# ShuhangGu/DASR

Measured on AMD Instinct MI355X. Metric: SR train images/sec (4x, 128->512), higher is better.
Workload: dtype bf16 MFMA operands, fp32 accumulate / fp32 residual stream

## Files before the change

dasr_amd/_lib.py:

```python
import ctypes as C
import os
import struct

HERE = os.path.dirname(os.path.abspath(__file__))
LIB_PATH = os.path.join(HERE, 'libdasr_hip.so')

c_i32, c_i64, c_f32, c_vp = C.c_int32, C.c_int64, C.c_float, C.c_void_p


class Tensor(C.Structure):
    _fields_ = [('p', c_vp), ('n_stride', c_i64), ('cb_stride', c_i64)]


class ConvParams(C.Structure):
    _fields_ = [('inp', Tensor), ('in_f32', c_i32), ('Hin', c_i32), ('Win', c_i32), ('ups', c_i32), ('cin', c_i32),
                ('w', c_vp), ('w_lo_off', c_i64), ('bias', c_vp),
                ('cout', c_i32), ('Hout', c_i32), ('Wout', c_i32), ('N', c_i32),
                ('kh', c_i32), ('stride', c_i32), ('pad', c_i32), ('prec', c_i32), ('mt', c_i32),
                ('act', c_i32), ('slope', c_f32),
                ('mask', Tensor), ('mask_f32', c_i32),
                ('alpha', c_f32), ('res1', Tensor), ('beta1', c_f32), ('res2', Tensor), ('beta2', c_f32),
                ('out_f32', Tensor), ('out_bf16', Tensor), ('gamma', c_f32), ('xcd_remap', c_i32),
                ('pad_x', c_i32), ('out_stride', c_i32), ('out_oy', c_i32), ('out_ox', c_i32), ('out_W', c_i32), ('slope_ptr', c_vp),
                ('in_stride', c_i32), ('in_oy', c_i32), ('in_ox', c_i32), ('in_W', c_i32), ('in_scale', c_f32), ('out16_f16', c_i32), ('in_wrap', c_i32), ('out16_lo', c_i32), ('res1_lo', c_i32), ('prelu_part', c_vp)]


class WgradPart(C.Structure):
    _fields_ = [('g', Tensor), ('g_f32', c_i32), ('inp', Tensor), ('in_f32', c_i32), ('ups', c_i32), ('n_ctiles', c_i32),
                ('g_planes', c_i32), ('in_planes', c_i32),
                ('Hin', c_i32), ('Win', c_i32), ('Hout', c_i32), ('Wout', c_i32), ('N', c_i32),
                ('kh', c_i32), ('stride', c_i32), ('pad', c_i32), ('want_bias', c_i32),
                ('ws_off', c_i64), ('ws_bias_off', c_i64), ('tap0', c_i32), ('g_scale', c_f32)]


class WgradReducePart(C.Structure):
    _fields_ = [('ws_off', c_i64), ('ws_bias_off', c_i64), ('nsplit', c_i32), ('ntaps', c_i32), ('oc0', c_i32), ('c0', c_i32),
                ('cout', c_i32), ('cin', c_i32), ('n_ctiles', c_i32), ('dst_w_off', c_i64), ('dst_b_off', c_i64),
                ('flip_io', c_i32), ('split_stride', c_i64), ('tap_stride', c_i64), ('bias_stride', c_i64),
                ('tap0', c_i32), ('ntaps_total', c_i32), ('bias_nsplit', c_i32), ('reserved_', c_i32)]


class ResblockParams(C.Structure):
    _fields_ = [('x16', Tensor), ('x32', Tensor), ('w0', c_vp), ('b0', c_vp), ('w1', c_vp), ('b1', c_vp),
                ('y32', Tensor), ('y16', Tensor), ('h', Tensor), ('N', c_i32), ('H', c_i32), ('W', c_i32), ('res_scale', c_f32), ('slope', c_f32)]


class PackSeg(C.Structure):
    _fields_ = [('src_off', c_i64), ('src_cout', c_i32), ('src_cin', c_i32), ('cin_start', c_i32), ('cin_len', c_i32),
                ('src_c0', c_i32), ('transpose', c_i32)]


class PackDesc(C.Structure):
    _fields_ = [('dst_off', c_i64), ('lo_off', c_i64), ('cout', c_i32), ('cin_pad', c_i32), ('ntaps', c_i32), ('mt', c_i32),
                ('nseg', c_i32), ('src_ntaps', c_i32), ('fmt', c_i32), ('tapmap', C.c_int8 * 32), ('tapmask', C.c_uint16 * 16), ('seg', PackSeg * 5)]


class CropDesc(C.Structure):
    _fields_ = [('src', c_vp), ('C', c_i32), ('H', c_i32), ('W', c_i32), ('vH', c_i32), ('vW', c_i32), ('y0', c_i32), ('x0', c_i32), ('flags', c_i32)]


class CropU8Desc(C.Structure):
    _fields_ = [('src', c_vp), ('H', c_i32), ('W', c_i32), ('y0', c_i32), ('x0', c_i32), ('crop', c_i32), ('flags', c_i32), ('sub_y', c_i32), ('sub_x', c_i32)]


class SrnU8Desc(C.Structure):
    _fields_ = [('src', c_vp), ('H', c_i32), ('W', c_i32), ('y0', c_i32), ('x0', c_i32), ('size', c_i32), ('flags', c_i32), ('dst', c_vp)]


class WindowDesc(C.Structure):
    _fields_ = [('y0', c_i32), ('x0', c_i32)]


class Op(C.Structure):
    _fields_ = [('op', c_i32), ('i', c_i32 * 8), ('f', c_f32 * 4), ('l', c_i64 * 4), ('p', c_vp * 4), ('t', Tensor * 5),
                ('conv', ConvParams), ('flops', C.c_double), ('bytes', C.c_double)]

    def get(self, name):
        arr, k, enc = _slot(self.op, name)
        a = getattr(self, arr)
        if enc == '*':
            return list(a) if arr == 'f' else list((c_f32 * 4).from_buffer(a))
        if enc == 'f':
            return struct.unpack('<f', struct.pack('<I', a[k] & 0xffffffff))[0]
        return a[k]

    def set(self, name, value):
        arr, k, enc = _slot(self.op, name)
        a = getattr(self, arr)
        if enc == '*':
            if arr == 'f':
                a[:] = [float(v) for v in value]
            else:
                (c_f32 * 4).from_buffer(a)[:] = [float(v) for v in value]
        elif enc == 'f':
            a[k] = struct.unpack('<I', struct.pack('<f', value))[0]
        elif value is None:
            a[k] = Tensor(None, 0, 0) if arr == 't' else 0
        else:
            a[k] = value


OP_CONV, OP_WGRAD, OP_WGRAD_REDUCE, OP_PACK, OP_DOWNSUM, OP_AXPBY, OP_FILL, OP_L1LOSS, OP_NCHW2B, OP_B2NCHW = range(1, 11)
(OP_INORM_FWD, OP_INORM_BWD, OP_BCE, OP_DWT_FWD, OP_DWT_BWD, OP_LOWPASS, OP_MAXPOOL, OP_MAXPOOL_BWD, OP_L1DIFF, OP_AFFINE4,
 OP_BILINEAR, OP_LOGLOSS, OP_SIGMOID_BWD, OP_PRELU_GRAD, OP_LOWPASS_VALID, OP_ADD_FLAT, OP_SIGMOID_FWD, OP_EVENT_RECORD, OP_STREAM_WAIT,
 OP_SET_STREAM) = range(11, 31)
OP_CVT_F16, OP_DOWNSUM_F16, OP_PIXSHUF, OP_PIXUNSHUF = 31, 32, 33, 34
OP_LPIPS_S2D, OP_MAXPOOL3, OP_MAXPOOL3_BWD, OP_LPIPS_HEAD, OP_RAGAN = 35, 36, 37, 38, 39
OP_BNORM_FWD, OP_BNORM_BWD, OP_BNORM_RUNNING = 40, 41, 42
OP_DDM_SPREAD = 43
OP_INORM_JVP, OP_INORM_SECOND, OP_GRAD_PENALTY, OP_FILL_SCALED = 44, 45, 46, 47
OP_CONV_CHAIN = 48
OP_RDB_CHAIN = 49
OP_BNORM_JVP, OP_BNORM_SECOND = 50, 51
OP_PRELU_FINAL = 52
OP_RESBLOCK = 53
OP_LPIPS_S2D_ANY = 54

OP_ARGS = {
    OP_WGRAD: dict(parts_dev='p0', nparts='i0', nsplit='i1', kh='i2', stride='i3', f32='i4', ws='p1'),
    OP_WGRAD_REDUCE: dict(parts_dev='p0', nparts='i0', ws='p1', grad_flat='p2', scale='f0', inv_prescale='f1', few_splits='i1'),
    OP_PACK: dict(descs_dev='p0', ndesc='i0', total_pieces='l0', piece_prefix_dev='p1', params_flat='p2', packed='p3'),
    OP_DOWNSUM: dict(src='t0', N='i0', C='i1', H='i2', W='i3', mask='t1', mask_f32='i4', slope='f0', dst_f32='t2', dst_bf16='t3'),
    OP_AXPBY: dict(x='t0', a='f0', z='t1', b='f1', N='i0', C='i1', H='i2', W='i3', out_f32='t2', out_bf16='t3', gamma='f2', mask='t4', slope='f3',
                   slope_ptr='p0'),
    OP_FILL: dict(p='p0', n='l0', value='f0'),
    OP_L1LOSS: dict(sr='t0', hr_nchw='p0', weight_map='p1', N='i0', C='i1', H='i2', W='i3', coef='f0', loss_acc='p2', grad='t1', accumulate='i4',
                    grad_scale='f1'),
    OP_NCHW2B: dict(src='p0', N='i0', C='i1', H='i2', W='i3', dst_f32='t0', dst_bf16='t1'),
    OP_B2NCHW: dict(src='t0', N='i0', C='i1', H='i2', W='i3', dst='p0'),
    OP_INORM_FWD: dict(x='t0', N='i0', C='i1', H='i2', W='i3', eps='f0', slope='f1', y='t1', stats='p0'),
    OP_INORM_BWD: dict(a='t0', ga='t1', N='i0', C='i1', H='i2', W='i3', slope='f0', stats='p0', gx='t2'),
    OP_BCE: dict(x='t0', N='i0', C='i1', H='i2', W='i3', gan_type='i4', target='f0', coef='f1', gcoef='f2', loss_acc='p0', score_acc='p1',
                 score_coef='f3', grad='t1'),
    OP_DWT_FWD: dict(x='t0', N='i0', C='i1', H2='i2', W2='i3', norm='i4', ll='t1', hc='t2'),
    OP_DWT_BWD: dict(gll='t0', ghc='t1', N='i0', C='i1', H2='i2', W2='i3', norm='i4', gx='t2', accumulate='i5'),
    OP_LOWPASS: dict(x='t0', x2='t1', w='p0', k='i4', N='i0', C='i1', H='i2', W='i3', mode='i5', a_h='f0', b_h='f1', out_low='t2', out_high='t3',
                     accumulate='i6'),
    OP_MAXPOOL: dict(x='t0', is_f32='i4', N='i0', C='i1', Ho='i2', Wo='i3', y='t1', Win='i6'),
    OP_MAXPOOL_BWD: dict(x='t0', gy='t1', is_f32='i4', N='i0', C='i1', Ho='i2', Wo='i3', gx='t2', relu_mask='i5', Win='i6'),
    OP_L1DIFF: dict(a='t0', b='t1', is_f32='i4', N='i0', C='i1', H='i2', W='i3', coef='f0', gcoef='f1', loss_acc='p0', ga='t2'),
    OP_AFFINE4: dict(x='t0', N='i0', C='i1', H='i2', W='i3', scale4='f*', shift4='l*', y='t1', y_f32='i4', accumulate='i5'),
    OP_BILINEAR: dict(src='p0', N='i0', h='i1', w='i2', factor='i3', dst='p1'),
    OP_LOGLOSS: dict(x='t0', N='i0', H='i1', W='i2', mode='i3', eps='f0', coef='f1', gcoef='f2', loss_acc='p0', score_acc='p1', score_coef='f3',
                     grad='t1', accumulate='i4'),
    OP_SIGMOID_BWD: dict(y='t0', g='t1', N='i0', C='i1', H='i2', W='i3', gz='t2'),
    OP_PRELU_GRAD: dict(y='t0', gx='t1', N='i0', C='i1', H='i2', W='i3', slope='p0', scratch256='p1', dst='p2', scale='f0', f16='i4', inv_prescale='f1'),
    OP_LOWPASS_VALID: dict(x='t0', w='p0', k='i4', N='i0', C='i1', H='i2', W='i3', mode='i5', out='t1', accumulate='i6'),
    OP_ADD_FLAT: dict(y='p0', x='p1', n='l0'),
    OP_SIGMOID_FWD: dict(x='t0', N='i0', C='i1', H='i2', W='i3', y='t1'),
    OP_EVENT_RECORD: dict(event='p0'),
    OP_STREAM_WAIT: dict(event='p0'),
    OP_SET_STREAM: dict(stream='p0'),
    OP_PIXSHUF: dict(src='t0', N='i0', C4='i1', H='i2', W='i3', dst='t1'),
    OP_PIXUNSHUF: dict(gsrc='t0', mask='t1', slope='f0', N='i0', C4='i1', H='i2', W='i3', gdst='t2'),
    OP_CVT_F16: dict(x='t0', N='i0', C='i1', H='i2', W='i3', scale='f0', y='t1', form='i4'),
    OP_DOWNSUM_F16: dict(src='t0', N='i0', C='i1', H='i2', W='i3', mask='t1', slope='f0', out_scale='f1', dst_f32='t2', dst_f16='t3'),
    OP_BNORM_FWD: dict(x='t0', N='i0', C='i1', H='i2', W='i3', group='i4', eps='f0', slope='f1', gamma='p0', beta='p1', y='t1', stats='p2'),
    OP_BNORM_BWD: dict(x='t0', ga='t1', N='i0', C='i1', H='i2', W='i3', group='i4', slope='f0', gamma='p0', beta='p1', stats='p2', gx='t2', dgamma='p3',
                       dbeta='l0', pscale='f1'),
    OP_BNORM_RUNNING: dict(stats='p0', g='i0', C='i1', count='i2', momentum='f0', running_mean='p1', running_var='p2', num_batches_tracked='p3'),
    OP_INORM_JVP: dict(a='t0', t='t1', N='i0', C='i1', H='i2', W='i3', slope='f0', stats='p0', out='t2'),
    OP_INORM_SECOND: dict(a='t0', t='t1', ga='t2', N='i0', C='i1', H='i2', W='i3', slope='f0', stats='p0', out='t3', accumulate='i4'),
    OP_RESBLOCK: dict(p='p0'),
    OP_PRELU_FINAL: dict(partial='p0', nblocks='i0', stride='l0', count='i1', slopes='p1', dsts='p2', scale='f0'),
    OP_BNORM_JVP: dict(x='t0', t='t1', N='i0', C='i1', H='i2', W='i3', group='i4', slope='f0', gamma='p0', beta='p1', stats='p2', out='t2'),
    OP_BNORM_SECOND: dict(x='t0', t='t1', ga='t2', N='i0', C='i1', H='i2', W='i3', group='i4', slope='f0', gamma='p0', beta='p1', stats='p2', out='t3',
                          accumulate='i5', dgamma='p3', pscale='f1'),
    OP_GRAD_PENALTY: dict(g='t0', N='i0', C='i1', H='i2', W='i3', weight='f0', part256='p0', out3='p1', loss_acc='p2', stage='i4',
                          world='i5'),
    OP_FILL_SCALED: dict(x='t0', N='i0', C='i1', H='i2', W='i3', scalar='p0', factor='f0'),
    OP_CONV_CHAIN: dict(dev_layers='p0', host_layers='p1', dev_dep_chunk='p2', nlayers='i0', dev_flags='p3', dev_err='l0'),
    OP_RDB_CHAIN: dict(dev_layers='p0', host_layers='p1', nlayers='i0', dev_flags='p3', dev_err='l0'),
    OP_DDM_SPREAD: dict(d='t0', N='i0', n_h='i1', n_w='i2', H='i3', W='i4', jump='i5', rf='i6', start='f0', out='t1'),
    OP_RAGAN: dict(a='t0', b='t1', N='i0', H='i1', W='i2', stage='i3', n_glob='i4', form='i5', ta='f0', tb='f1', coef='f2', gcoef='f3', eps='l2f',
                   sums='p0', part='p1', loss_acc='p2', score_a='p3', score_b='l0', score_coef='l1f', ga='t2', gb='t3'),
    OP_LPIPS_S2D: dict(x='t0', N='i0', H='i1', W='i2', scale4='f*', shift4='l*', y='t1', mode='i3'),
    OP_MAXPOOL3: dict(x='t0', N='i0', C='i1', H='i2', W='i3', y='t1'),
# ... 184 lines not shown
```

dasr_amd/csrc/conv.hip:

```cpp
#include "common.h"

namespace {

template <int PREC, bool IN_F32, int MT, int KH, int STRIDE, int NT_, int KS = 1>
struct Cfg {
    static constexpr int NT = NT_;
    static constexpr int RPT = STRIDE == 1 ? 1 : 2;
    static constexpr int CPT = STRIDE == 1 ? 32 : 16;
    static constexpr int TH = 4 * NT * RPT;
    static constexpr int TW = CPT;
    static constexpr int IH = (TH - 1) * STRIDE + KH;
    static constexpr int IW = (TW - 1) * STRIDE + KH;
    static constexpr int NTAPS = KH * KH;
    static constexpr int PIXB = KS == 1 ? 48 : 80;
    static constexpr int ACT_BYTES = IH * IW * PIXB;
    static constexpr int W_BYTES = KS * NTAPS * MT * 1024;
    static constexpr int NARR = PREC >= 3 ? 2 : 1;
    static constexpr int LDS_BYTES = NARR * (ACT_BYTES + W_BYTES);
    static constexpr int PPP16 = IN_F32 ? 4 : 2;
    static constexpr int PPP = PPP16 * KS;
    static constexpr int NPIECE = IH * IW * PPP;
    static constexpr int AR = (NPIECE + 255) / 256;
    static constexpr int WPIECE = KS * NTAPS * MT * 64;
    static constexpr int WR = (WPIECE + 255) / 256;
};

constexpr unsigned OOB = 0x80000000u;
constexpr int RSRC_FLAGS = 0x00020000;
constexpr int RSRC_RANGE = 0x7fffffff;

#ifdef DASR_TRACE
__device__ unsigned long long* g_trace = nullptr;
#define TRACE_STAMP(k)                                                                         \
    do {                                                                                       \
        if (g_trace && threadIdx.x == 0) g_trace[(size_t)blockIdx.x * 16 + (k)] = __builtin_readcyclecounter(); \
    } while (0)
#else
#define TRACE_STAMP(k) do {} while (0)
#endif

__device__ __forceinline__ __amdgpu_buffer_rsrc_t make_rsrc(const void* p) {
    return __builtin_amdgcn_make_buffer_rsrc((void*)p, 0, RSRC_RANGE, RSRC_FLAGS);
}

template <int NG>
struct MaskPre {
    u32x4 v[NG][2];
};

template <int MT, int NT>
__device__ __forceinline__ void mask_prefetch(const dasr_conv_params& p, MaskPre<NT * MT>& m, int tid, int mg, int n, int oy0, int ox0) {
    const int lane = tid & 63, wave = tid >> 6, nn = lane & 31, kh2 = lane >> 5;
    const int ostr = p.out_stride > 1 ? p.out_stride : 1, owid = p.out_W > 0 ? p.out_W : p.Wout;
    const __amdgpu_buffer_rsrc_t rmask = make_rsrc((const char*)p.mask.p + (size_t)n * p.mask.n_stride * 2);
    const unsigned mask_cb = (unsigned)p.mask.cb_stride;
#pragma unroll
    for (int gi = 0; gi < NT * MT; ++gi) {
        const int nt = gi / MT, mi = gi - nt * MT;
        const int oy = oy0 + wave * NT + nt, ox = ox0 + nn;
        const unsigned oob = ((oy < p.Hout) & (ox < p.Wout)) ? 0u : OOB;
        const unsigned pixel = (unsigned)((oy * ostr + p.out_oy) * owid + ox * ostr + p.out_ox) * 16u;
#pragma unroll
        for (int pr = 0; pr < 2; ++pr) {
            const int oc = (mg * MT + mi) * 32 + 16 * pr;
            const unsigned mo = (((unsigned)(oc >> 4) * mask_cb + pixel + 8u * kh2) * 2u) | oob;
            m.v[gi][pr] = __builtin_amdgcn_raw_buffer_load_b128(rmask, mo, 0, 0);
        }
    }
}

template <bool SC1>
__device__ __forceinline__ void st128(u32x4 v, __amdgpu_buffer_rsrc_t r, unsigned off) {
    if constexpr (SC1) __builtin_amdgcn_raw_buffer_store_b128(v, r, off, 0, 16);
    else __builtin_amdgcn_raw_buffer_store_b128(v, r, off, 0, 0);
}

template <bool IN_F32, int MT, int NT, int STRIDE, int EPI, int F16OUT = -1, bool PRE = false, bool FSC1 = false, bool BIAS_STAGED = false, bool CONST_SLOPE = false,
          bool PACC = false>
__device__ __forceinline__ void conv_epilogue(const dasr_conv_params& p, f32x16 (&acc)[MT][NT], char* smem, float bias_reg, int tid, int mg, int n,
                                              int oy0, int ox0, const MaskPre<NT * MT>* pre = nullptr) {
    const int lane = tid & 63, wave = tid >> 6, nn = lane & 31, kh2 = lane >> 5;
    (void)lane;
    constexpr bool G = EPI == 0;
    const bool has_bias = G ? p.bias != nullptr : bool(EPI & 1);
    const bool act_lrelu = G ? p.act == 1 : bool(EPI & 2);
    const bool act_sigmoid = G ? p.act == 2 : false;
    const bool has_mask = G ? p.mask.p != nullptr : bool(EPI & 4);
    const bool has_r1 = G ? p.res1.p != nullptr : bool(EPI & 8);
    const bool has_r2 = G ? p.res2.p != nullptr : bool(EPI & 16);
    const bool has_f32 = G ? p.out_f32.p != nullptr : bool(EPI & 32);
    const bool has_bf16 = G ? p.out_bf16.p != nullptr : bool(EPI & 64);
    const bool scaled = G ? true : bool(EPI & 128);
    const bool f16out = F16OUT < 0 ? p.out16_f16 != 0 : F16OUT != 0;
    const bool chan_tail = G ? true : false;
    const int ostr = p.out_stride > 1 ? p.out_stride : 1, owid = p.out_W > 0 ? p.out_W : p.Wout;
    constexpr int MSZ = IN_F32 ? 4 : 2;
    const float slope = (!CONST_SLOPE && p.slope_ptr) ? *p.slope_ptr : p.slope;
    constexpr bool PACC_OK = PACC && EPI == 68 && MT == 2 && !IN_F32 && !FSC1 && !PRE;
    static_assert(!PACC || PACC_OK, "the slope-gradient partials exist for the 64-channel mask-only epilogue of the LDS-DMA kernel");
    constexpr bool pacc_on = PACC_OK;
    float pacc = 0.f;
    const __amdgpu_buffer_rsrc_t rmask = make_rsrc((const char*)p.mask.p + (size_t)n * p.mask.n_stride * MSZ);
    const __amdgpu_buffer_rsrc_t rr1 = make_rsrc((const char*)p.res1.p + (size_t)n * p.res1.n_stride * ((G && p.res1_lo) ? 2 : 4));
    const __amdgpu_buffer_rsrc_t rr2 = make_rsrc((const float*)p.res2.p + (size_t)n * p.res2.n_stride);
    const __amdgpu_buffer_rsrc_t rof = make_rsrc((float*)p.out_f32.p + (size_t)n * p.out_f32.n_stride);
    const __amdgpu_buffer_rsrc_t rob = make_rsrc((bf16_t*)p.out_bf16.p + (size_t)n * p.out_bf16.n_stride);
    const unsigned mask_cb = (unsigned)p.mask.cb_stride, r1_cb = (unsigned)p.res1.cb_stride, r2_cb = (unsigned)p.res2.cb_stride;
    const unsigned of_cb = (unsigned)p.out_f32.cb_stride, ob_cb = (unsigned)p.out_bf16.cb_stride;
    constexpr bool SC1 = FSC1 || (MT == 1 && !IN_F32 && F16OUT == 0);
    const unsigned lo_pl = (G || F16OUT != 0) ? (unsigned)p.out16_lo : 0u;
    f32x4 bia[MT][4];
    if (has_bias) {
        float* bl = (float*)smem;
        if constexpr (!BIAS_STAGED) {
            if (tid < 32 * MT) bl[tid] = bias_reg;
            __syncthreads();
        }
#pragma unroll
        for (int mi = 0; mi < MT; ++mi)
#pragma unroll
            for (int g = 0; g < 4; ++g) bia[mi][g] = *(const f32x4*)(bl + mi * 32 + 8 * g + 4 * kh2);
    }
    TRACE_STAMP(5);
    constexpr int NG = NT * MT;
    constexpr bool WIDE16 = !G && !IN_F32;
    constexpr bool WIDE32 = !G && STRIDE == 1;
    constexpr bool PIPE_EPI = !G && !(MT == 2 && (EPI & 16) && (EPI & 8)) && (EPI & (4 | 8 | 16));
    u32x4 mk[2][4], r1v[2][4], r2v[2][4];
    auto group_addr = [&](int gi, unsigned (&eo)[4], unsigned (&cbv)[4]) {
        const int nt = gi / MT, mi = gi - nt * MT;
        int r, c;
        if constexpr (STRIDE == 1) {
            r = wave * NT + nt;
            c = nn;
        } else {
            r = (wave * NT + nt) * 2 + (nn >> 4);
            c = nn & 15;
        }
        const int oy = oy0 + r, ox = ox0 + c;
        const bool pv = (oy < p.Hout) & (ox < p.Wout);
        const unsigned pixel = (unsigned)((oy * ostr + p.out_oy) * owid + ox * ostr + p.out_ox) * 16u;
#pragma unroll
        for (int g = 0; g < 4; ++g) {
            const int oc = (mg * MT + mi) * 32 + 8 * g + 4 * kh2;
            const bool cv = chan_tail ? (pv & (oc < ((p.cout + 15) & ~15))) : pv;
            cbv[g] = (unsigned)(oc >> 4);
            eo[g] = cv ? pixel + (unsigned)(oc & 15) : OOB;
        }
    };
    auto group_addr32 = [&](int gi, unsigned (&e32)[2]) {
        const int nt = gi / MT;
        const int oy = oy0 + wave * NT + nt;
        const unsigned q4 = 4u * (2u * (unsigned)(nn >> 4) + (unsigned)kh2);
#pragma unroll
        for (int st = 0; st < 2; ++st) {
            const int ox = ox0 + (nn & 15) + 16 * st;
            const bool pv = (oy < p.Hout) & (ox < p.Wout);
            e32[st] = pv ? (unsigned)((oy * ostr + p.out_oy) * owid + ox * ostr + p.out_ox) * 16u + q4 : OOB;
        }
    };
    auto issue_loads = [&](int gi, int slot) {
        unsigned eo[4], cbv[4];
        group_addr(gi, eo, cbv);
        unsigned e32[2];
        if constexpr (WIDE32) group_addr32(gi, e32);
        if (has_mask && !PRE) {
            if constexpr (WIDE16) {
#pragma unroll
                for (int pr = 0; pr < 2; ++pr) {
                    const unsigned mo = eo[2 * pr] != OOB ? (cbv[2 * pr] * mask_cb + eo[2 * pr] + 4u * kh2) * 2u : OOB;
                    mk[slot][2 * pr] = __builtin_amdgcn_raw_buffer_load_b128(rmask, mo, 0, 0);
                }
            } else {
#pragma unroll
                for (int g = 0; g < 4; ++g) {
                    const unsigned mo = eo[g] != OOB ? (cbv[g] * mask_cb + eo[g]) * MSZ : OOB;
                    if constexpr (IN_F32) {
                        mk[slot][g] = __builtin_amdgcn_raw_buffer_load_b128(rmask, mo, 0, 0);
                    } else {
                        const u32x2 t2 = __builtin_amdgcn_raw_buffer_load_b64(rmask, mo, 0, 0);
                        mk[slot][g] = u32x4{t2[0], t2[1], 0u, 0u};
                    }
                }
            }
        }
        if (G && has_r1 && p.res1_lo) {
#pragma unroll
            for (int g = 0; g < 4; ++g) {
                const u32x2 hi = __builtin_amdgcn_raw_buffer_load_b64(rr1, eo[g] != OOB ? (cbv[g] * r1_cb + eo[g]) * 2u : OOB, 0, 0);
                const u32x2 lo = __builtin_amdgcn_raw_buffer_load_b64(rr1, eo[g] != OOB ? ((cbv[g] + (unsigned)p.res1_lo) * r1_cb + eo[g]) * 2u : OOB, 0, 0);
                r1v[slot][g] = u32x4{hi[0], hi[1], lo[0], lo[1]};
            }
        } else if (has_r1) {
#pragma unroll
            for (int g = 0; g < 4; ++g) {
                if constexpr (WIDE32) r1v[slot][g] = __builtin_amdgcn_raw_buffer_load_b128(rr1, e32[g & 1] != OOB ? (cbv[g] * r1_cb + e32[g & 1]) * 4u : OOB, 0, 0);
                else r1v[slot][g] = __builtin_amdgcn_raw_buffer_load_b128(rr1, eo[g] != OOB ? (cbv[g] * r1_cb + eo[g]) * 4u : OOB, 0, 0);
            }
        }
        if (has_r2) {
#pragma unroll
            for (int g = 0; g < 4; ++g) {
                if constexpr (WIDE32) r2v[slot][g] = __builtin_amdgcn_raw_buffer_load_b128(rr2, e32[g & 1] != OOB ? (cbv[g] * r2_cb + e32[g & 1]) * 4u : OOB, 0, 0);
                else r2v[slot][g] = __builtin_amdgcn_raw_buffer_load_b128(rr2, eo[g] != OOB ? (cbv[g] * r2_cb + eo[g]) * 4u : OOB, 0, 0);
            }
        }
    };
    auto rows_swap = [&](u32x4& a, u32x4& b) {
#pragma unroll
        for (int j = 0; j < 4; ++j) {
            const auto r = __builtin_amdgcn_permlane16_swap(a[j], b[j], false, false);
            a[j] = r[0];
            b[j] = r[1];
        }
    };
    if constexpr (PIPE_EPI) issue_loads(0, 0);
#pragma unroll
    for (int gi = 0; gi < NG; ++gi) {
        const int nt = gi / MT, mi = gi - nt * MT;
        const int slot = PIPE_EPI ? (gi & 1) : 0;
        if constexpr (PIPE_EPI) {
            if (gi + 1 < NG) issue_loads(gi + 1, (gi + 1) & 1);
        } else {
            issue_loads(gi, 0);
        }
        {
            unsigned eo[4], cbv[4];
            group_addr(gi, eo, cbv);
            float v[4][4];
#pragma unroll
            for (int g = 0; g < 4; ++g)
#pragma unroll
                for (int j = 0; j < 4; ++j) v[g][j] = acc[mi][nt][4 * g + j];
            if (has_bias) {
#pragma unroll
                for (int g = 0; g < 4; ++g)
#pragma unroll
                    for (int j = 0; j < 4; ++j) v[g][j] += bia[mi][g][j];
            }
            if (act_lrelu && !G && !CONST_SLOPE && p.slope_ptr) {
#pragma unroll
                for (int g = 0; g < 4; ++g)
#pragma unroll
                    for (int j = 0; j < 4; ++j) v[g][j] = v[g][j] > 0.f ? v[g][j] : slope * v[g][j];
            } else if (act_lrelu && !G) {
#pragma unroll
                for (int g = 0; g < 4; ++g)
#pragma unroll
                    for (int j = 0; j < 4; ++j) v[g][j] = fmaxf(v[g][j], slope * v[g][j]);
            } else if (act_lrelu) {
#pragma unroll
                for (int g = 0; g < 4; ++g)
#pragma unroll
                    for (int j = 0; j < 4; ++j) v[g][j] = fmaxf(v[g][j], 0.f) + slope * fminf(v[g][j], 0.f);
            } else if (act_sigmoid) {
#pragma unroll
                for (int g = 0; g < 4; ++g)
#pragma unroll
                    for (int j = 0; j < 4; ++j) v[g][j] = __frcp_rn(1.f + __expf(-v[g][j]));
            }
            if (has_mask) {
                if constexpr (WIDE16) {
#pragma unroll
                    for (int pr = 0; pr < 2; ++pr) {
                        u32x4 w = mk[slot][2 * pr];
                        if constexpr (PRE) w = pre->v[gi][pr];
                        const auto r0 = __builtin_amdgcn_permlane32_swap(w[0], w[2], false, false);
                        const auto r1 = __builtin_amdgcn_permlane32_swap(w[1], w[3], false, false);
                        mk[slot][2 * pr] = u32x4{r0[0], r1[0], 0u, 0u};
                        mk[slot][2 * pr + 1] = u32x4{r0[1], r1[1], 0u, 0u};
                    }
                }
#pragma unroll
                for (int g = 0; g < 4; ++g)
#pragma unroll
                    for (int j = 0; j < 4; ++j) {
                        if constexpr (IN_F32) {
                            v[g][j] *= __uint_as_float(mk[slot][g][j]) > 0.f ? 1.f : slope;
                        } else {
                            const unsigned wd = mk[slot][g][j >> 1];
                            const short hbits = (j & 1) ? (short)(wd >> 16) : (short)(wd & 0xffffu);
                            if constexpr (PACC_OK) {
                                if (pacc_on) {
                                    const unsigned short hb = (unsigned short)hbits;
                                    const float hv = f16out ? (float)__builtin_bit_cast(f16_t, hb) : (float)__builtin_bit_cast(bf16_t, hb);
                                    pacc += hbits > 0 ? 0.f : v[g][j] * hv;
                                }
                            }
                            v[g][j] = hbits > 0 ? v[g][j] : slope * v[g][j];
                        }
                    }
            }
            if (scaled && p.alpha != 1.f) {
#pragma unroll
                for (int g = 0; g < 4; ++g)
#pragma unroll
                    for (int j = 0; j < 4; ++j) v[g][j] *= p.alpha;
            }
            if (G && has_r1 && p.res1_lo) {
#pragma unroll
                for (int g = 0; g < 4; ++g) {
                    const u32x4 w = r1v[slot][g];
#pragma unroll
                    for (int j = 0; j < 4; ++j) {
                        const unsigned short hb = (unsigned short)((j & 1) ? (w[j >> 1] >> 16) : (w[j >> 1] & 0xffffu));
                        const unsigned short lb = (unsigned short)((j & 1) ? (w[2 + (j >> 1)] >> 16) : (w[2 + (j >> 1)] & 0xffffu));
                        const float r = f16out ? (float)__builtin_bit_cast(f16_t, hb) + (float)__builtin_bit_cast(f16_t, lb)
                                               : (float)__builtin_bit_cast(bf16_t, hb) + (float)__builtin_bit_cast(bf16_t, lb);
                        v[g][j] += p.beta1 * r;
                    }
                }
            } else if (has_r1) {
                if constexpr (WIDE32) {
                    rows_swap(r1v[slot][0], r1v[slot][1]);
                    rows_swap(r1v[slot][2], r1v[slot][3]);
                }
#pragma unroll
                for (int g = 0; g < 4; ++g)
#pragma unroll
                    for (int j = 0; j < 4; ++j) v[g][j] += p.beta1 * __uint_as_float(r1v[slot][g][j]);
            }
            if (has_r2) {
                if constexpr (WIDE32) {
                    rows_swap(r2v[slot][0], r2v[slot][1]);
                    rows_swap(r2v[slot][2], r2v[slot][3]);
                }
#pragma unroll
                for (int g = 0; g < 4; ++g)
#pragma unroll
                    for (int j = 0; j < 4; ++j) v[g][j] += p.beta2 * __uint_as_float(r2v[slot][g][j]);
            }
            if (chan_tail && (mg * MT + mi) * 32 + 32 > p.cout) {
#pragma unroll
                for (int g = 0; g < 4; ++g)
#pragma unroll
                    for (int j = 0; j < 4; ++j)
                        if ((mg * MT + mi) * 32 + 8 * g + 4 * kh2 + j >= p.cout) v[g][j] = 0.f;
            }
            if (has_f32 && WIDE32) {
                unsigned e32[2];
                group_addr32(gi, e32);
#pragma unroll
                for (int pr = 0; pr < 2; ++pr) {
                    u32x4 oa = {__float_as_uint(v[2 * pr][0]), __float_as_uint(v[2 * pr][1]), __float_as_uint(v[2 * pr][2]), __float_as_uint(v[2 * pr][3])};
                    u32x4 ob = {__float_as_uint(v[2 * pr + 1][0]), __float_as_uint(v[2 * pr + 1][1]), __float_as_uint(v[2 * pr + 1][2]), __float_as_uint(v[2 * pr + 1][3])};
                    rows_swap(oa, ob);
                    st128<SC1>(oa, rof, e32[0] != OOB ? (cbv[2 * pr] * of_cb + e32[0]) * 4u : OOB);
                    st128<SC1>(ob, rof, e32[1] != OOB ? (cbv[2 * pr] * of_cb + e32[1]) * 4u : OOB);
                }
            } else if (has_f32) {
#pragma unroll
                for (int g = 0; g < 4; ++g) {
                    const u32x4 o = {__float_as_uint(v[g][0]), __float_as_uint(v[g][1]), __float_as_uint(v[g][2]), __float_as_uint(v[g][3])};
                    st128<SC1>(o, rof, eo[g] != OOB ? (cbv[g] * of_cb + eo[g]) * 4u : OOB);
                }
            }
            if (has_bf16 && WIDE16) {
                const bool gm = scaled && p.gamma != 1.f;
#pragma unroll
                for (int pr = 0; pr < 2; ++pr) {
                    bf16x4 oa, ob;
#pragma unroll
                    for (int j = 0; j < 4; ++j) {
                        const float va = gm ? v[2 * pr][j] * p.gamma : v[2 * pr][j], vb = gm ? v[2 * pr + 1][j] * p.gamma : v[2 * pr + 1][j];
                        oa[j] = f16out ? __builtin_bit_cast(bf16_t, (f16_t)va) : (bf16_t)va;
                        ob[j] = f16out ? __builtin_bit_cast(bf16_t, (f16_t)vb) : (bf16_t)vb;
                    }
                    const u32x2 a = __builtin_bit_cast(u32x2, oa), b = __builtin_bit_cast(u32x2, ob);
                    const auto r0 = __builtin_amdgcn_permlane32_swap(a[0], b[0], false, false);
                    const auto r1 = __builtin_amdgcn_permlane32_swap(a[1], b[1], false, false);
                    const u32x4 o = {r0[0], r1[0], r0[1], r1[1]};
                    st128<SC1>(o, rob, eo[2 * pr] != OOB ? (cbv[2 * pr] * ob_cb + eo[2 * pr] + 4u * kh2) * 2u : OOB);
                    if (lo_pl) {
                        bf16x4 la, lb;
#pragma unroll
                        for (int j = 0; j < 4; ++j) {
                            const float va = gm ? v[2 * pr][j] * p.gamma : v[2 * pr][j], vb = gm ? v[2 * pr + 1][j] * p.gamma : v[2 * pr + 1][j];
                            const float ha = f16out ? (float)(f16_t)va : (float)(bf16_t)va, hb = f16out ? (float)(f16_t)vb : (float)(bf16_t)vb;
                            la[j] = f16out ? __builtin_bit_cast(bf16_t, (f16_t)(va - ha)) : (bf16_t)(va - ha);
                            lb[j] = f16out ? __builtin_bit_cast(bf16_t, (f16_t)(vb - hb)) : (bf16_t)(vb - hb);
                        }
                        const u32x2 a2 = __builtin_bit_cast(u32x2, la), b2 = __builtin_bit_cast(u32x2, lb);
                        const auto q0 = __builtin_amdgcn_permlane32_swap(a2[0], b2[0], false, false);
                        const auto q1 = __builtin_amdgcn_permlane32_swap(a2[1], b2[1], false, false);
                        const u32x4 o2 = {q0[0], q1[0], q0[1], q1[1]};
                        st128<SC1>(o2, rob, eo[2 * pr] != OOB ? ((cbv[2 * pr] + lo_pl) * ob_cb + eo[2 * pr] + 4u * kh2) * 2u : OOB);
                    }
                }
            } else if (has_bf16) {
                const bool gm = scaled && p.gamma != 1.f;
#pragma unroll
                for (int g = 0; g < 4; ++g) {
                    bf16x4 ob;
#pragma unroll
                    for (int j = 0; j < 4; ++j) {
                        const float vv = gm ? v[g][j] * p.gamma : v[g][j];
                        ob[j] = f16out ? __builtin_bit_cast(bf16_t, (f16_t)vv) : (bf16_t)vv;
                    }
#ifdef DASR_TRACE
                    if (p.xcd_remap & 2) {
                        const unsigned lin = ((((unsigned)blockIdx.x * 4 + wave) * NT + nt) * 4 + g) * 512u + (unsigned)lane * 8u;
                        __builtin_amdgcn_raw_buffer_store_b64(__builtin_bit_cast(u32x2, ob), make_rsrc(p.out_bf16.p), lin, 0, 0);
                        continue;
                    }
#endif
                    __builtin_amdgcn_raw_buffer_store_b64(__builtin_bit_cast(u32x2, ob), rob, eo[g] != OOB ? (cbv[g] * ob_cb + eo[g]) * 2u : OOB, 0, 0);
                    if (lo_pl) {
                        bf16x4 lb;
#pragma unroll
                        for (int j = 0; j < 4; ++j) {
                            const float vv = gm ? v[g][j] * p.gamma : v[g][j];
                            const float hh = f16out ? (float)(f16_t)vv : (float)(bf16_t)vv;
                            lb[j] = f16out ? __builtin_bit_cast(bf16_t, (f16_t)(vv - hh)) : (bf16_t)(vv - hh);
                        }
                        __builtin_amdgcn_raw_buffer_store_b64(__builtin_bit_cast(u32x2, lb), rob, eo[g] != OOB ? ((cbv[g] + lo_pl) * ob_cb + eo[g]) * 2u : OOB, 0, 0);
                    }
                }
            }
        }
    }
    if constexpr (PACC_OK) {
        if (pacc_on) {
            const float t = wave_sum(pacc);
            __syncthreads();
            if (lane == 0) ((float*)smem)[wave] = t;
            __syncthreads();
            if (tid == 0) {
                float tot = 0.f;
                for (int w = 0; w < (int)(blockDim.x >> 6); ++w) tot += ((const float*)smem)[w];
                p.prelu_part[blockIdx.x] = tot * slope;
            }
        }
    }
}

template <int PREC, bool IN_F32, int MT, int KH, int STRIDE, int NT, int KS, bool DBUF, int MODE, int EPI>
__global__ __launch_bounds__(256, 2) void conv_kernel(const dasr_conv_params p) {
    using C = Cfg<PREC, IN_F32, MT, KH, STRIDE, NT, KS>;
    extern __shared__ __attribute__((aligned(16))) char smem[];
    constexpr int ACT_LO = C::ACT_BYTES, W_HI = C::NARR * C::ACT_BYTES, W_LO = W_HI + C::W_BYTES;
    constexpr int DUMMY = C::LDS_BYTES;

    const int tid = threadIdx.x, lane = tid & 63, wave = tid >> 6;
#ifdef DASR_TRACE
    if (g_trace && threadIdx.x == 0) g_trace[(size_t)blockIdx.x * 16 + 15] = __builtin_amdgcn_s_memrealtime();
#endif
    TRACE_STAMP(0);
    const int cout_tiles = (p.cout + 31) >> 5;
    const int MG = (cout_tiles + MT - 1) / MT;
    const int tiles_x = (p.Wout + C::TW - 1) / C::TW, tiles_y = (p.Hout + C::TH - 1) / C::TH;
    int bid = blockIdx.x;
    {
        const int total = gridDim.x;
        if ((p.xcd_remap & 1) && (total & 7) == 0) bid = (bid & 7) * (total >> 3) + (bid >> 3);
    }
    const int mg = bid % MG;
    bid /= MG;
    const int tx = bid % tiles_x;
    bid /= tiles_x;
    const int ty = bid % tiles_y;
    const int n = bid / tiles_y;
    const int oy0 = ty * C::TH, ox0 = tx * C::TW;
    const int iy0 = oy0 * STRIDE - p.pad, ix0 = ox0 * STRIDE - (p.pad_x >= 0 ? p.pad_x : p.pad);
    const int HL = p.ups ? 2 * p.Hin : p.Hin, WL = p.ups ? 2 * p.Win : p.Win;
    const int nchunks = p.cin / (16 * KS);
    constexpr int ESZ = IN_F32 ? 4 : 2;
    static_assert(PREC != 2 || IN_F32, "prec 2 (f16 operands) converts an f32 input while staging");
    const float in_sc = ((PREC == 2 || PREC == 4) && p.in_scale != 0.f) ? p.in_scale : 1.f;
    float bias_reg = 0.f;
    {
        const int oc = mg * MT * 32 + tid;
        const unsigned bo = ((p.bias != nullptr) & (tid < 32 * MT) & (oc < p.cout)) ? (unsigned)oc * 4u : OOB;
        bias_reg = __uint_as_float(__builtin_amdgcn_raw_buffer_load_b32(make_rsrc(p.bias), bo, 0, 0));
    }

    unsigned goff[C::AR];
    int loff[C::AR];
#pragma unroll
    for (int r = 0; r < C::AR; ++r) {
        const int q = tid + r * 256;
        const int pix = q / C::PPP, piece = q - pix * C::PPP;
        const int iy = pix / C::IW, ix = pix - iy * C::IW;
        const int gy = iy0 + iy, gx = ix0 + ix;
        const bool ok = (q < C::NPIECE) & (gy >= 0) & (gy < HL) & (gx >= 0) & (gx < WL);
        const int sy = p.ups ? (gy >> 1) : gy, sx = p.ups ? (gx >> 1) : gx;
        const int pl = piece / C::PPP16, pp = piece - pl * C::PPP16;
        const int spix = p.in_stride > 1 ? (sy * p.in_stride + p.in_oy) * p.in_W + sx * p.in_stride + p.in_ox : sy * p.Win + sx;
        goff[r] = ok ? (unsigned)((pl * (int)p.in.cb_stride + spix * 16 + pp * (IN_F32 ? 4 : 8)) * ESZ) : OOB;
        loff[r] = q < C::NPIECE ? pix * C::PIXB + piece * (IN_F32 ? 8 : 16) : DUMMY;
    }
    const __amdgpu_buffer_rsrc_t rin = make_rsrc((const char*)p.in.p + (size_t)n * p.in.n_stride * ESZ);
    const unsigned in_chunk_bytes = (unsigned)(p.in.cb_stride * KS * ESZ);
    const __amdgpu_buffer_rsrc_t rw = make_rsrc((const bf16_t*)p.w + (size_t)mg * nchunks * KS * C::NTAPS * MT * 512);
    const unsigned w_chunk_bytes = KS * C::NTAPS * MT * 1024;
    const unsigned w_lo_bytes = (unsigned)(p.w_lo_off * 2);
    unsigned woff[C::WR];
    int wloff[C::WR];
#pragma unroll
    for (int r = 0; r < C::WR; ++r) {
        const int q = tid + r * 256;
        woff[r] = q < C::WPIECE ? (unsigned)q * 16u : OOB;
        wloff[r] = q < C::WPIECE ? q * 16 : DUMMY - W_HI;
    }

    u32x4 areg[C::AR];
    u32x4 wreg[C::WR * C::NARR];
    auto load_chunk = [&](int ck) {
        const unsigned so = (unsigned)ck * in_chunk_bytes;
#pragma unroll
        for (int r = 0; r < C::AR; ++r) areg[r] = __builtin_amdgcn_raw_buffer_load_b128(rin, goff[r], so, 0);
        const unsigned wo = (unsigned)ck * w_chunk_bytes;
#pragma unroll
        for (int r = 0; r < C::WR; ++r) {
            wreg[r] = __builtin_amdgcn_raw_buffer_load_b128(rw, woff[r], wo, 0);
            if constexpr (PREC >= 3) wreg[C::WR + r] = __builtin_amdgcn_raw_buffer_load_b128(rw, woff[r], wo + w_lo_bytes, 0);
        }
    };
    auto store_chunk = [&](char* buf) {
#pragma unroll
        for (int r = 0; r < C::AR; ++r) {
            if constexpr (!IN_F32) {
                *(u32x4*)(buf + loff[r]) = areg[r];
            } else {
                bf16x4 hi, lo;
#pragma unroll
                for (int j = 0; j < 4; ++j) {
                    bf16_t h, l;
                    if constexpr (PREC == 2) {
                        h = __builtin_bit_cast(bf16_t, (f16_t)(__uint_as_float(areg[r][j]) * in_sc));
                        l = h;
                    } else if constexpr (PREC == 4) {
                        split_f16(__uint_as_float(areg[r][j]) * in_sc, h, l);
                    } else {
                        split_bf16(__uint_as_float(areg[r][j]), h, l);
                    }
                    hi[j] = h;
                    lo[j] = l;
                }
                *(bf16x4*)(buf + loff[r]) = hi;
// ... 169 lines not shown

template <int MT, int NW = 4>
struct GCfg {
    static constexpr int NT = 4, NTH = NW * 64, TH = 4 * NW, TW = 32, IH = TH + 2, IW = 34, NPIX = IH * IW;
    static constexpr int AR = (NPIX * 2 + NTH - 1) / NTH;
    static constexpr int ACT_BYTES = AR * NTH * 16;
    static constexpr int WPIECE = 9 * MT * 64;
    static constexpr int WR = (WPIECE + NTH - 1) / NTH;
    static constexpr int W_BYTES = WPIECE * 16;
    static constexpr int BUF_BYTES = ACT_BYTES + W_BYTES;
    static constexpr int LDS_BYTES = 2 * BUF_BYTES;
};

template <int MT, int NW>
__device__ __forceinline__ void glds_dma_piece(int i, int ck, char* buf, __amdgpu_buffer_rsrc_t rin, __amdgpu_buffer_rsrc_t rw, const unsigned* goff,
                                               unsigned in_chunk_bytes, int wave, int tid, int ckp) {
    using C = GCfg<MT, NW>;
    typedef __attribute__((address_space(3))) void* lds_ptr;
    if (i < C::AR) {
        __builtin_amdgcn_raw_ptr_buffer_load_lds(rin, (lds_ptr)(buf + (i * C::NTH + wave * 64) * 16), 16, goff[i], (unsigned)ckp * in_chunk_bytes, 0, 0);
    } else {
        const int r = i - C::AR;
        if (r * C::NTH + wave * 64 < C::WPIECE)
            __builtin_amdgcn_raw_ptr_buffer_load_lds(rw, (lds_ptr)(buf + C::ACT_BYTES + (r * C::NTH + wave * 64) * 16), 16, (unsigned)(tid + r * C::NTH) * 16u,
                                                     (unsigned)ck * (9u * MT * 1024u), 0, 0);
    }
}

template <int MT, int EPI, int NW, int ABL = 0, bool F16 = false, int RING = 0>
__global__ __launch_bounds__(NW * 64, NW == 4 ? 2 : 1) void conv_glds_kernel(const dasr_conv_params p) {
    using C = GCfg<MT, NW>;
    constexpr int NT = C::NT;
    extern __shared__ __attribute__((aligned(16))) char smem[];
    const int tid = threadIdx.x, lane = tid & 63, wave = __builtin_amdgcn_readfirstlane(tid >> 6);
#ifdef DASR_TRACE
    if (g_trace && threadIdx.x == 0) g_trace[(size_t)blockIdx.x * 16 + 15] = __builtin_amdgcn_s_memrealtime();
#endif
    TRACE_STAMP(0);
    int a_cout = p.cout, a_Wout = p.Wout, a_Hout = p.Hout, a_remap = p.xcd_remap, a_ups = p.ups, a_cin = p.cin, a_Hin = p.Hin, a_Win = p.Win;
    const void* a_bias = p.bias;
    const void* a_in = p.in.p;
    const void* a_w = p.w;
    long long a_nstr = p.in.n_stride, a_cbstr = p.in.cb_stride;
    int a_wrap = p.in_wrap;
    asm volatile("" : "+s"(a_cout), "+s"(a_Wout), "+s"(a_Hout), "+s"(a_remap), "+s"(a_cin), "+s"(a_Hin), "+s"(a_Win), "+s"(a_bias), "+s"(a_in), "+s"(a_w),
                 "+s"(a_nstr), "+s"(a_cbstr), "+s"(a_wrap), "+s"(a_ups)
                 : "s"(p.slope), "s"(p.out_stride), "s"(p.out_oy), "s"(p.out_ox), "s"(p.out_W), "s"(p.alpha), "s"(p.gamma), "s"(p.out16_lo), "s"(p.N));
    a_remap |= a_ups << 8;
    const int cout_tiles = (a_cout + 31) >> 5;
    const int MG = (cout_tiles + MT - 1) / MT;
    const int tiles_x = (a_Wout + C::TW - 1) / C::TW, tiles_y = (a_Hout + C::TH - 1) / C::TH;
    int bid = blockIdx.x;
    {
        const int total = (int)((unsigned)a_remap >> 12);
        const int remapped = (bid & 7) * (total >> 3) + (bid >> 3);
        bid = ((a_remap & 1) && (total & 7) == 0) ? remapped : bid;
    }
    const int mg = bid % MG;
    bid /= MG;
    const int tx = bid % tiles_x;
    bid /= tiles_x;
    const int ty = bid % tiles_y;
    const int n = bid / tiles_y;
    const int oy0 = ty * C::TH, ox0 = tx * C::TW;
    const int iy0 = oy0 - 1, ix0 = ox0 - 1;
    const int nchunks = a_cin >> 4;
    const int in_wrap = a_wrap > 0 ? a_wrap : 0x7fffffff;
    constexpr int rot = 0;
    float bias_reg = 0.f;
    {
        const int oc = mg * MT * 32 + tid;
        const unsigned bo = ((a_bias != nullptr) & (tid < 32 * MT) & (oc < a_cout)) ? (unsigned)oc * 4u : OOB;
        bias_reg = __uint_as_float(__builtin_amdgcn_raw_buffer_load_b32(make_rsrc(a_bias), bo, 0, 0));
    }
    unsigned goff[C::AR];
#pragma unroll
    for (int r = 0; r < C::AR; ++r) {
        const int q = tid + r * C::NTH;
        const int pp = q >> 1, h = (q & 1) ^ ((pp >> 3) & 1);
        const int iy = pp / C::IW, ix = pp - iy * C::IW;
        const int gy = iy0 + iy, gx = ix0 + ix;
        const int us = (a_remap >> 8) & 1;
        const bool ok = (pp < C::NPIX) & (gy >= 0) & (gy < (a_Hin << us)) & (gx >= 0) & (gx < (a_Win << us));
        goff[r] = ok ? (unsigned)((((gy >> us) * a_Win + (gx >> us)) * 16 + 8 * h) * 2) : OOB;
    }
    const __amdgpu_buffer_rsrc_t rin = make_rsrc((const bf16_t*)a_in + (size_t)n * a_nstr);
    const unsigned in_chunk_bytes = (unsigned)(a_cbstr * 2);
    const __amdgpu_buffer_rsrc_t rw = make_rsrc((const bf16_t*)a_w + (size_t)mg * nchunks * 9 * MT * 512);
    constexpr int NP = C::AR + C::WR;
#pragma unroll
    for (int i = 0; i < NP; ++i) glds_dma_piece<MT, NW>(i, rot, smem, rin, rw, goff, in_chunk_bytes, wave, tid, rot);
    TRACE_STAMP(1);
    const int nn = lane & 31, kh2 = lane >> 5;
    int baddr[6][3];
#pragma unroll
    for (int rr = 0; rr < 6; ++rr)
#pragma unroll
        for (int kx = 0; kx < 3; ++kx) {
            const int pp = (wave * NT + rr) * C::IW + nn + kx;
            baddr[rr][kx] = ((pp << 1) + (kh2 ^ ((pp >> 3) & 1))) << 4;
        }
    const int aoff = lane * 16;

    f32x16 acc[MT][NT];
    constexpr bool R1_PRE = MT == 2 && EPI != 0 && (EPI & 8);
    if constexpr (R1_PRE) {
        const __amdgpu_buffer_rsrc_t rr1 = make_rsrc((const float*)p.res1.p + (size_t)n * p.res1.n_stride);
        const unsigned r1_cb = (unsigned)p.res1.cb_stride;
        const int nn_ = lane & 31, kh_ = lane >> 5;
#pragma unroll
        for (int nt = 0; nt < NT; ++nt) {
            const int oy = oy0 + wave * NT + nt, ox = ox0 + nn_;
            const bool pv = (oy < a_Hout) & (ox < a_Wout);
            const unsigned pixel = (unsigned)((oy + p.out_oy) * (p.out_W > 0 ? p.out_W : a_Wout) + ox + p.out_ox) * 16u;
#pragma unroll
            for (int mi = 0; mi < MT; ++mi)
#pragma unroll
                for (int g = 0; g < 4; ++g) {
                    const int oc = (mg * MT + mi) * 32 + 8 * g + 4 * kh_;
                    const u32x4 t = __builtin_amdgcn_raw_buffer_load_b128(rr1, pv ? ((unsigned)(oc >> 4) * r1_cb + pixel + (unsigned)(oc & 15)) * 4u : OOB, 0, 0);
#pragma unroll
                    for (int j = 0; j < 4; ++j) acc[mi][nt][4 * g + j] = __uint_as_float(t[j]);
                }
        }
    } else {
#pragma unroll
        for (int mi = 0; mi < MT; ++mi)
#pragma unroll
            for (int nt = 0; nt < NT; ++nt)
#pragma unroll
                for (int j = 0; j < 16; ++j) acc[mi][nt][j] = 0.f;
    }

    __builtin_amdgcn_s_waitcnt(0x0F70);
    __syncthreads();
    if constexpr (R1_PRE) {
        const float c1 = p.beta1 / p.alpha;
#pragma unroll
        for (int mi = 0; mi < MT; ++mi)
#pragma unroll
            for (int nt = 0; nt < NT; ++nt) acc[mi][nt] *= c1;
    }
    TRACE_STAMP(2);

    constexpr bool PRE = EPI == 68 && MT == 1;
    MaskPre<NT * MT> mpre;
    bf16x8 fb[2][6], fa[2][MT];
    for (int ck = 0; ck < nchunks; ++ck) {
        const char* buf = smem + (ck & 1) * C::BUF_BYTES;
        const char* wbuf = buf + C::ACT_BYTES;
        char* nbuf = smem + ((ck + 1) & 1) * C::BUF_BYTES;
        const bool more = ck + 1 < nchunks;
        if constexpr (PRE) {
            if (!more) mask_prefetch<MT, NT>(p, mpre, tid, mg, n, oy0, ox0);
        }
        const int ckn = ck + 1 + rot < nchunks ? ck + 1 + rot : ck + 1 + rot - nchunks;
        const int ckp = ckn >= in_wrap ? ckn - in_wrap : ckn;
        if (ck == 2) TRACE_STAMP(8);
#pragma unroll
        for (int rr = 0; rr < 6; ++rr) fb[0][rr] = *(const bf16x8*)(buf + baddr[rr][0]);
#pragma unroll
        for (int mi = 0; mi < MT; ++mi) fa[0][mi] = *(const bf16x8*)(wbuf + aoff + (0 * MT + mi) * 1024);
#pragma unroll
        for (int s = 0; s < 9; ++s) {
            const int kx = s / 3, ky = s - kx * 3;
            if (s + 1 < 9) {
                const int kx1 = (s + 1) / 3, ky1 = (s + 1) - kx1 * 3;
#pragma unroll
                for (int mi = 0; mi < MT; ++mi) fa[(s + 1) & 1][mi] = *(const bf16x8*)(wbuf + aoff + ((ky1 * 3 + kx1) * MT + mi) * 1024);
                if (ky == 1 && kx < 2) {
#pragma unroll
                    for (int rr = 0; rr < 6; ++rr) fb[(kx + 1) & 1][rr] = *(const bf16x8*)(buf + baddr[rr][kx + 1]);
                }
            }
            if (more && s < 4) {
#pragma unroll
                for (int i = s * NP / 4; i < (s + 1) * NP / 4; ++i) glds_dma_piece<MT, NW>(i, ckn, nbuf, rin, rw, goff, in_chunk_bytes, wave, tid, ckp);
            }
            __builtin_amdgcn_sched_barrier(0);
#pragma unroll
            for (int mi = 0; mi < MT; ++mi)
#pragma unroll
                for (int nt = 0; nt < NT; ++nt)
                    acc[mi][nt] = mfma16<F16>(fa[s & 1][mi], fb[kx & 1][nt + ky], acc[mi][nt]);
            __builtin_amdgcn_sched_barrier(0);
        }
        if (ck == 2) TRACE_STAMP(9);
        __builtin_amdgcn_s_waitcnt(0x0F70);
        if (ck == 2) TRACE_STAMP(10);
        __syncthreads();
        if (ck == 2) TRACE_STAMP(11);
    }
    TRACE_STAMP(4);
    if constexpr (EPI == 68 && MT == 2 && !PRE) {
        if (p.prelu_part) conv_epilogue<false, MT, NT, 1, EPI, F16 ? 1 : 0, false, false, false, false, true>(p, acc, smem, bias_reg, tid, mg, n, oy0, ox0, &mpre);
        else conv_epilogue<false, MT, NT, 1, EPI, F16 ? 1 : 0, PRE>(p, acc, smem, bias_reg, tid, mg, n, oy0, ox0, &mpre);
    } else {
        conv_epilogue<false, MT, NT, 1, R1_PRE ? (EPI & ~8) : EPI, F16 ? 1 : 0, PRE>(p, acc, smem, bias_reg, tid, mg, n, oy0, ox0, &mpre);
    }
    TRACE_STAMP(6);
#ifdef DASR_TRACE
    __builtin_amdgcn_s_waitcnt(0);
#endif
    TRACE_STAMP(7);
#ifdef DASR_TRACE
    if (g_trace && threadIdx.x == 0) g_trace[(size_t)blockIdx.x * 16 + 14] = __builtin_amdgcn_s_memrealtime();
#endif
}

#ifdef DASR_TRACE
#define CH_T() (g_trace && threadIdx.x == 0 ? (unsigned long long)__builtin_readcyclecounter() : 0ull)
#define CH_ACC(type, phase, val)                                                                           \
    do {                                                                                                   \
        if (g_trace && threadIdx.x == 0) g_trace[(size_t)(1 << 20) + (size_t)blockIdx.x * 64 + (type) * 8 + (phase)] += (val); \
    } while (0)
#else
#define CH_T() 0ull
#define CH_ACC(type, phase, val) do {} while (0)
#endif

#ifdef DASR_TRACE
#define CH_WHERE(ticket, xcc)                                                                  \
    do {                                                                                       \
        if (g_trace && threadIdx.x == 0) {                                                     \
            unsigned hw;                                                                       \
            asm volatile("s_getreg_b32 %0, hwreg(HW_REG_HW_ID)" : "=s"(hw));                   \
            g_trace[(size_t)(1 << 20) + (size_t)blockIdx.x * 64 + 56] = hw;                    \
            g_trace[(size_t)(1 << 20) + (size_t)blockIdx.x * 64 + 57] = (unsigned)(ticket);    \
            g_trace[(size_t)(1 << 20) + (size_t)blockIdx.x * 64 + 58] = (unsigned)(xcc);       \
        }                                                                                      \
    } while (0)
#else
#define CH_WHERE(ticket, xcc) do {} while (0)
#endif

struct ChainSync {
    __amdgpu_buffer_rsrc_t rflags;
    int* err;
    unsigned f0;
    int base, ty, tx, tiles_y, tiles_x;

    __device__ __forceinline__ void wait(int layer, int tid) const {
        if (layer > 0) {
            if (tid < 9 && tid != 4) {
                const int y = ty + tid / 3 - 1, x = tx + tid % 3 - 1;
                if ((y >= 0) & (y < tiles_y) & (x >= 0) & (x < tiles_x)) {
                    const unsigned off = (unsigned)(base + y * tiles_x + x) * 4u, target = f0 + (unsigned)layer;
                    int spins = 0;
                    while ((int)(__builtin_amdgcn_raw_buffer_load_b32(rflags, off, 0, 17) - target) < 0) {
                        __builtin_amdgcn_s_sleep(2);
                        ++spins;
                        if (spins > (1 << 21) || ((spins & 1023) == 0 && __builtin_amdgcn_raw_buffer_load_b32(make_rsrc(err), 0, 0, 17) != 0)) {
                            atomicOr(err, 2);
                            break;
                        }
                    }
                }
            }
            __syncthreads();
        }
    }
    __device__ __forceinline__ void publish(int layer, int tid) const {
        __builtin_amdgcn_s_waitcnt(0x0F70);
        __syncthreads();
        if (tid == 0) __builtin_amdgcn_raw_buffer_store_b32(f0 + (unsigned)layer + 1u, rflags, (unsigned)(base + ty * tiles_x + tx) * 4u, 0, 16);
    }
};

template <int MT, int EPI, bool F16>
__device__ __forceinline__ void chain_layer(const dasr_conv_params& p, char* smem, const int tid, const int n, const int oy0, const int ox0,
                                            const unsigned (&goff)[GCfg<1, 4>::AR], const int dep_chunk, const ChainSync& cs, const int layer) {
    using C = GCfg<MT, 4>;
    constexpr int NT = C::NT, NW = 4;
    static_assert(GCfg<1, 4>::AR == GCfg<2, 4>::AR, "the activation pieces do not depend on MT");
    const int lane = tid & 63, wave = __builtin_amdgcn_readfirstlane(tid >> 6);
    const int nchunks = p.cin >> 4;
    const int ttype = MT == 2 ? 2 : (dep_chunk <= 1 ? 0 : 1);
    (void)ttype;
    const unsigned long long t_a = CH_T();
    float bias_reg;
    {
        const unsigned bo = ((p.bias != nullptr) & (tid < 32 * MT)) ? (unsigned)tid * 4u : OOB;
        bias_reg = __uint_as_float(__builtin_amdgcn_raw_buffer_load_b32(make_rsrc(p.bias), bo, 0, 0));
    }
    const __amdgpu_buffer_rsrc_t rin = make_rsrc((const bf16_t*)p.in.p + (size_t)n * p.in.n_stride);
    const unsigned in_chunk_bytes = (unsigned)(p.in.cb_stride * 2);
    const __amdgpu_buffer_rsrc_t rw = make_rsrc(p.w);
    constexpr int NP = C::AR + C::WR;
    if (dep_chunk <= 0) cs.wait(layer, tid);
#pragma unroll
    for (int i = 0; i < NP; ++i) glds_dma_piece<MT, NW>(i, 0, smem, rin, rw, goff, in_chunk_bytes, wave, tid, 0);
    const unsigned long long t_b = CH_T();
    const int nn = lane & 31, kh2 = lane >> 5;
    int baddr[6][3];
#pragma unroll
    for (int rr = 0; rr < 6; ++rr)
#pragma unroll
        for (int kx = 0; kx < 3; ++kx) {
            const int pp = (wave * NT + rr) * C::IW + nn + kx;
            baddr[rr][kx] = ((pp << 1) + (kh2 ^ ((pp >> 3) & 1))) << 4;
        }
    const int aoff = lane * 16;
    f32x16 acc[MT][NT];
    constexpr bool R1_PRE = MT == 2 && (EPI & 8);
    if constexpr (R1_PRE) {
        const __amdgpu_buffer_rsrc_t rr1 = make_rsrc((const float*)p.res1.p + (size_t)n * p.res1.n_stride);
        const unsigned r1_cb = (unsigned)p.res1.cb_stride;
#pragma unroll
        for (int nt = 0; nt < NT; ++nt) {
            const int oy = oy0 + wave * NT + nt, ox = ox0 + nn;
            const bool pv = (oy < p.Hout) & (ox < p.Wout);
            const unsigned pixel = (unsigned)(oy * p.Wout + ox) * 16u;
#pragma unroll
            for (int mi = 0; mi < MT; ++mi)
#pragma unroll
                for (int g = 0; g < 4; ++g) {
                    const int oc = mi * 32 + 8 * g + 4 * kh2;
                    const u32x4 t = __builtin_amdgcn_raw_buffer_load_b128(rr1, pv ? ((unsigned)(oc >> 4) * r1_cb + pixel + (unsigned)(oc & 15)) * 4u : OOB, 0, 0);
#pragma unroll
                    for (int j = 0; j < 4; ++j) acc[mi][nt][4 * g + j] = __uint_as_float(t[j]);
                }
        }
    } else {
#pragma unroll
        for (int mi = 0; mi < MT; ++mi)
#pragma unroll
            for (int nt = 0; nt < NT; ++nt)
#pragma unroll
                for (int j = 0; j < 16; ++j) acc[mi][nt][j] = 0.f;
    }
    __builtin_amdgcn_s_waitcnt(0x0F70);
    __syncthreads();
    if constexpr (R1_PRE) {
        const float c1 = p.beta1 / p.alpha;
#pragma unroll
        for (int mi = 0; mi < MT; ++mi)
#pragma unroll
            for (int nt = 0; nt < NT; ++nt) acc[mi][nt] *= c1;
    }
    constexpr bool PRE = EPI == 68 && MT == 1;
    MaskPre<NT * MT> mpre;
    bf16x8 fb[2][6];
    const unsigned long long t_c = CH_T();
    unsigned long long t_poll = 0;
    (void)t_poll;
    for (int ck = 0; ck < nchunks; ++ck) {
        const char* buf = smem + (ck & 1) * C::BUF_BYTES;
        const char* wbuf = buf + C::ACT_BYTES;
        char* nbuf = smem + ((ck + 1) & 1) * C::BUF_BYTES;
        const bool more = ck + 1 < nchunks;
        if (ck + 1 == dep_chunk) {
            const unsigned long long t0 = CH_T();
            cs.wait(layer, tid);
            t_poll += CH_T() - t0;
        }
        if constexpr (PRE) {
            if (!more) mask_prefetch<MT, NT>(p, mpre, tid, 0, n, oy0, ox0);
        }
        bf16x8 fa[3][MT];
#pragma unroll
        for (int rr = 0; rr < 6; ++rr) fb[0][rr] = *(const bf16x8*)(buf + baddr[rr][0]);
#pragma unroll
        for (int mi = 0; mi < MT; ++mi) fa[0][mi] = *(const bf16x8*)(wbuf + aoff + (0 * MT + mi) * 1024);
#pragma unroll
        for (int s = 0; s < 9; ++s) {
            const int kx = s / 3, ky = s - kx * 3;
            if (s + 1 < 9) {
                const int kx1 = (s + 1) / 3, ky1 = (s + 1) - kx1 * 3;
#pragma unroll
                for (int mi = 0; mi < MT; ++mi) fa[(s + 1) & 1][mi] = *(const bf16x8*)(wbuf + aoff + ((ky1 * 3 + kx1) * MT + mi) * 1024);
                if (ky == 1 && kx < 2) {
#pragma unroll
                    for (int rr = 0; rr < 6; ++rr) fb[(kx + 1) & 1][rr] = *(const bf16x8*)(buf + baddr[rr][kx + 1]);
                }
            }
            if (more && s < 4) {
#pragma unroll
                for (int i = s * NP / 4; i < (s + 1) * NP / 4; ++i) glds_dma_piece<MT, NW>(i, ck + 1, nbuf, rin, rw, goff, in_chunk_bytes, wave, tid, ck + 1);
            }
            __builtin_amdgcn_sched_barrier(0);
#pragma unroll
            for (int mi = 0; mi < MT; ++mi)
#pragma unroll
                for (int nt = 0; nt < NT; ++nt) acc[mi][nt] = mfma16<F16>(fa[s & 1][mi], fb[kx & 1][nt + ky], acc[mi][nt]);
            __builtin_amdgcn_sched_barrier(0);
        }
        __builtin_amdgcn_s_waitcnt(0x0F70);
        __syncthreads();
    }
    const unsigned long long t_d = CH_T();
    conv_epilogue<false, MT, NT, 1, R1_PRE ? (EPI & ~8) : EPI, F16 ? 1 : 0, PRE, true>(p, acc, smem, bias_reg, tid, 0, n, oy0, ox0, &mpre);
    const unsigned long long t_e = CH_T();
    cs.publish(layer, tid);
    const unsigned long long t_f = CH_T();
    CH_ACC(ttype, 0, t_b - t_a);
    CH_ACC(ttype, 1, t_c - t_b);
    CH_ACC(ttype, 2, t_d - t_c);
    CH_ACC(ttype, 3, t_poll);
    CH_ACC(ttype, 4, t_e - t_d);
    CH_ACC(ttype, 5, t_f - t_e);
    CH_ACC(ttype, 6, 1ull);
    CH_ACC(ttype, 7, (unsigned long long)nchunks);
    (void)t_a; (void)t_b; (void)t_c; (void)t_d; (void)t_e; (void)t_f;
}

template <bool F16, bool BWD>
__global__ __launch_bounds__(256, 2) void conv_chain_kernel(const dasr_conv_params* __restrict__ layers, const int* __restrict__ dep_chunk, int nlayers,
                                                           int tiles_y, int tiles_x, unsigned* flags, unsigned* tickets, int* err) {
    using C = GCfg<1, 4>;
    extern __shared__ __attribute__((aligned(16))) char smem[];
    const int tid = threadIdx.x;
    const int T = tiles_y * tiles_x;
    unsigned xcc;
    asm volatile("s_getreg_b32 %0, hwreg(HW_REG_XCC_ID)" : "=s"(xcc));
    const int xcd = (int)(xcc & 7u);
    const int quota = (int)(gridDim.x >> 3);
    int* tk = (int*)smem;
    if (tid == 0) tk[0] = (int)(atomicAdd(tickets + xcd, 1u) % (unsigned)quota);
    __syncthreads();
    const int j = __builtin_amdgcn_readfirstlane(tk[0]);
    __syncthreads();
    const int img = j / T, tile = j - img * T;
    const int n = xcd + 8 * img;
    const int ty = tile / tiles_x, tx = tile - ty * tiles_x;
    CH_WHERE(j, xcc);
    ChainSync cs;
    cs.rflags = make_rsrc(flags);
    cs.err = err;
    cs.base = n * T;
    cs.ty = ty, cs.tx = tx, cs.tiles_y = tiles_y, cs.tiles_x = tiles_x;
    cs.f0 = __builtin_amdgcn_readfirstlane(__builtin_amdgcn_raw_buffer_load_b32(cs.rflags, (unsigned)(cs.base + tile) * 4u, 0, 17));
    const int oy0 = ty * C::TH, ox0 = tx * C::TW;
    const int iy0 = oy0 - 1, ix0 = ox0 - 1;
    const int Hin = layers[0].Hin, Win = layers[0].Win;
    unsigned goff[C::AR];
#pragma unroll
    for (int r = 0; r < C::AR; ++r) {
        const int q = tid + r * C::NTH;
        const int pp = q >> 1, h = (q & 1) ^ ((pp >> 3) & 1);
        const int iy = pp / C::IW, ix = pp - iy * C::IW;
        const int gy = iy0 + iy, gx = ix0 + ix;
        const bool ok = (pp < C::NPIX) & (gy >= 0) & (gy < Hin) & (gx >= 0) & (gx < Win);
        goff[r] = ok ? (unsigned)(((gy * Win + gx) * 16 + 8 * h) * 2) : OOB;
    }
    for (int L = 0; L < nlayers; ++L) {
        const dasr_conv_params& p = layers[L];
        const int dep = dep_chunk[L];
        if constexpr (BWD) {
            if (p.mt == 1) chain_layer<1, 68, F16>(p, smem, tid, n, oy0, ox0, goff, dep, cs, L);
            else if (p.res2.p != nullptr) chain_layer<2, 248, F16>(p, smem, tid, n, oy0, ox0, goff, dep, cs, L);
            else chain_layer<2, 232, F16>(p, smem, tid, n, oy0, ox0, goff, dep, cs, L);
        } else {
            if (p.mt == 1) chain_layer<1, 67, F16>(p, smem, tid, n, oy0, ox0, goff, dep, cs, L);
            else if (p.res2.p != nullptr) chain_layer<2, 249, F16>(p, smem, tid, n, oy0, ox0, goff, dep, cs, L);
            else chain_layer<2, 233, F16>(p, smem, tid, n, oy0, ox0, goff, dep, cs, L);
        }
    }
}

template <int MT, int EPI = 0, int NW = 4, int ABL = 0, bool F16 = false, int RING = 0>
int launch_glds(const dasr_conv_params& p, hipStream_t s) {
    static_assert(ABL == 0 && RING == 0, "one dense-block conv kernel");
    using C = GCfg<MT, NW>;
    static bool attr_set = false;
    auto kfn = conv_glds_kernel<MT, EPI, NW, ABL, F16, RING>;
    if ((p.cin & 15) || p.kh != 3 || p.stride != 1 || p.pad != 1 || p.in_f32 || p.prec != (F16 ? 2 : 1) || (p.pad_x >= 0 && p.pad_x != 1) || p.in_stride > 1)
        return DASR_EINVAL;
    if (p.out_bf16.p && (p.out16_f16 != 0) != F16) return DASR_EINVAL;
    if (p.prelu_part && !(EPI == 68 && MT == 2)) return DASR_EINVAL;
    if (!attr_set) {
        HIP_TRY(hipFuncSetAttribute((const void*)kfn, hipFuncAttributeMaxDynamicSharedMemorySize, C::LDS_BYTES));
        attr_set = true;
    }
    const int cout_tiles = (p.cout + 31) >> 5;
    const int MG = (cout_tiles + MT - 1) / MT;
    const int tiles_x = (p.Wout + C::TW - 1) / C::TW, tiles_y = (p.Hout + C::TH - 1) / C::TH;
    const long long grid = (long long)MG * tiles_x * tiles_y * p.N;
    if (grid <= 0 || grid >= (1LL << 20)) return DASR_EINVAL;
    dasr_conv_params q = p;
    q.xcd_remap = (p.xcd_remap & 0xfff) | (int)((unsigned)grid << 12);
    DASR_LAUNCH_TAG(__PRETTY_FUNCTION__, kfn, dim3((unsigned)grid), dim3(C::NTH), C::LDS_BYTES, s, q);
    return (int)hipGetLastError();
}

template <int PREC, bool IN_F32, int MT, int KH, int STRIDE, int NT, int KS = 1, bool DBUF = false, int MODE = 0, int EPI = 0>
int launch(const dasr_conv_params& p, hipStream_t s) {
    static_assert(KS == 1 && !DBUF && MODE == 0, "one staging form of the register-staged kernel");
    using C = Cfg<PREC, IN_F32, MT, KH, STRIDE, NT, KS>;
    static bool attr_set = false;
    auto kfn = conv_kernel<PREC, IN_F32, MT, KH, STRIDE, NT, KS, DBUF, MODE, EPI>;
    if (p.cin % (16 * KS)) return DASR_EINVAL;
    if (p.prelu_part) return DASR_EINVAL;
    if (!attr_set) {
        HIP_TRY(hipFuncSetAttribute((const void*)kfn, hipFuncAttributeMaxDynamicSharedMemorySize, C::LDS_BYTES + 16));
        attr_set = true;
    }
    const int cout_tiles = (p.cout + 31) >> 5;
    const int MG = (cout_tiles + MT - 1) / MT;
    const int tiles_x = (p.Wout + C::TW - 1) / C::TW, tiles_y = (p.Hout + C::TH - 1) / C::TH;
    const long long grid = (long long)MG * tiles_x * tiles_y * p.N;
    if (grid <= 0 || grid > 0x7fffffffLL) return DASR_EINVAL;
    DASR_LAUNCH_TAG(__PRETTY_FUNCTION__, kfn, dim3((unsigned)grid), dim3(256), C::LDS_BYTES + 16, s, p);
    return (int)hipGetLastError();
}

__global__ void conv_naive_kernel(const dasr_conv_params p, const float* w) {
    const long long total = (long long)p.N * p.cout * p.Hout * p.Wout;
    const long long i = (long long)blockIdx.x * blockDim.x + threadIdx.x;
    if (i >= total) return;
    const int ox = i % p.Wout;
    long long t = i / p.Wout;
    const int oy = t % p.Hout;
    t /= p.Hout;
    const int oc = t % p.cout;
    const int n = t / p.cout;
    const int HL = p.ups ? 2 * p.Hin : p.Hin, WL = p.ups ? 2 * p.Win : p.Win;
    float acc = 0.f;
    for (int c = 0; c < p.cin; ++c)
        for (int ky = 0; ky < p.kh; ++ky)
            for (int kx = 0; kx < p.kh; ++kx) {
                const int gy = oy * p.stride - p.pad + ky, gx = ox * p.stride - (p.pad_x >= 0 ? p.pad_x : p.pad) + kx;
                if (gy < 0 || gy >= HL || gx < 0 || gx >= WL) continue;
                const int sy = p.ups ? gy >> 1 : gy, sx = p.ups ? gx >> 1 : gx;
                const size_t spix = p.in_stride > 1 ? ((size_t)sy * p.in_stride + p.in_oy) * p.in_W + (size_t)sx * p.in_stride + p.in_ox : (size_t)sy * p.Win + sx;
                const size_t o = (size_t)n * p.in.n_stride + (size_t)(c >> 4) * p.in.cb_stride + spix * 16 + (c & 15);
                const float x = p.in_f32 ? ((const float*)p.in.p)[o] : (float)((const bf16_t*)p.in.p)[o];
                acc += x * w[(((size_t)oc * p.cin + c) * p.kh + ky) * p.kh + kx];
            }
    if (p.bias) acc += p.bias[oc];
    const float nslope = p.slope_ptr ? *p.slope_ptr : p.slope;
    if (p.act == 1) acc = acc > 0.f ? acc : acc * nslope;
    if (p.act == 2) acc = 1.f / (1.f + expf(-acc));
    const size_t po = ((size_t)oy * p.Wout + ox) * 16 + (oc & 15);
    if (p.mask.p) {
        const size_t mo = (size_t)n * p.mask.n_stride + (size_t)(oc >> 4) * p.mask.cb_stride + po;
        const float m = p.mask_f32 ? ((const float*)p.mask.p)[mo] : (float)((const bf16_t*)p.mask.p)[mo];
        acc = m > 0.f ? acc : acc * nslope;
    }
    acc *= p.alpha;
    if (p.res1.p) acc += p.beta1 * ((const float*)p.res1.p)[(size_t)n * p.res1.n_stride + (size_t)(oc >> 4) * p.res1.cb_stride + po];
    if (p.res2.p) acc += p.beta2 * ((const float*)p.res2.p)[(size_t)n * p.res2.n_stride + (size_t)(oc >> 4) * p.res2.cb_stride + po];
    if (p.out_f32.p) ((float*)p.out_f32.p)[(size_t)n * p.out_f32.n_stride + (size_t)(oc >> 4) * p.out_f32.cb_stride + po] = acc;
    if (p.out_bf16.p)
        ((bf16_t*)p.out_bf16.p)[(size_t)n * p.out_bf16.n_stride + (size_t)(oc >> 4) * p.out_bf16.cb_stride + po] = (bf16_t)(acc * p.gamma);
}

int classify_epi(const dasr_conv_params& p) {
    if ((p.cout & 31) || p.act == 2 || p.out_stride > 1 || p.res1_lo || (p.out16_lo && !p.out16_f16)) return 0;
    if (p.act == 1 && !p.slope_ptr && !(p.slope >= 0.f && p.slope <= 1.f)) return 0;
    int e = (p.bias ? 1 : 0) | (p.act == 1 ? 2 : 0) | (p.mask.p ? 4 : 0) | (p.res1.p ? 8 : 0) | (p.res2.p ? 16 : 0) | (p.out_f32.p ? 32 : 0) |
            (p.out_bf16.p ? 64 : 0);
    if (p.res1.p || p.alpha != 1.f || p.gamma != 1.f) e |= 128;
    return e;
}

int g_tune_rdb64 = 13;

#include "rdb_is.h"

}

#ifdef DASR_TRACE
extern "C" int dasr_debug_set_trace(void* buf) {
    return (int)hipMemcpyToSymbol(HIP_SYMBOL(g_trace), &buf, sizeof(buf));
}
#endif

extern "C" int dasr_set_tuning(int32_t key, int32_t value) {
    if (key == 2 && (value == 12 || value == 13)) { g_tune_rdb64 = value; return 0; }
    if ((key == 1 && value == 12) || (key == 3 && value == 0) || (key == 4 && value == 1) || (key == 5 && value == 1) || (key == 6 && value == 0)) return 0;
    return DASR_EINVAL;
}

extern "C" int dasr_conv_chain(const dasr_conv_params* dev_layers, const dasr_conv_params* host_layers, const int32_t* dev_dep_chunk, int32_t nlayers,
                               uint32_t* dev_flags, int32_t* dev_err, void* stream) {
    using C = GCfg<2, 4>;
    if (!dev_layers || !host_layers || !dev_dep_chunk || nlayers <= 0 || !dev_flags || !dev_err) return DASR_EINVAL;
    const dasr_conv_params& p0 = host_layers[0];
    const bool f16 = p0.prec == 2;
    const bool bwd = classify_epi(p0) == 68 || classify_epi(p0) == 232 || classify_epi(p0) == 248;
    for (int i = 0; i < nlayers; ++i) {
        const dasr_conv_params& p = host_layers[i];
        if (p.kh != 3 || p.stride != 1 || p.pad != 1 || p.in_f32 || p.prec != p0.prec || (p.cin & 15) || p.cin <= 0 || p.ups || p.in_wrap || p.out16_lo || p.res1_lo) return DASR_EINVAL;
        if (p.Hin != p0.Hin || p.Win != p0.Win || p.Hout != p0.Hin || p.Wout != p0.Win || p.N != p0.N || p.out_stride > 1 || p.in_stride > 1 || p.out_W || p.out_oy || p.out_ox) return DASR_EINVAL;
        if (!(p.mt == 1 || p.mt == 2) || p.cout != 32 * p.mt || !p.w || !p.in.p || p.slope_ptr || p.mask_f32 || p.prelu_part) return DASR_EINVAL;
        if ((p.out16_f16 != 0) != f16 || (p.prec != 1 && p.prec != 2)) return DASR_EINVAL;
        const int epi = classify_epi(p);
        const bool ok = bwd ? (p.mt == 1 ? epi == 68 : (epi == 232 || epi == 248)) : (p.mt == 1 ? epi == 67 : (epi == 233 || epi == 249));
        if (!ok) return DASR_EINVAL;
    }
    const int tiles_x = (p0.Wout + C::TW - 1) / C::TW, tiles_y = (p0.Hout + C::TH - 1) / C::TH;
    const long long ntiles = (long long)tiles_x * tiles_y * p0.N;
    const long long grid = 512;
    if ((p0.N & 7) || ntiles != grid) return DASR_EINVAL;
    {
        static int n_cu = -1;
        if (n_cu < 0) {
            int dev = 0;
            hipDeviceProp_t prop;
            HIP_TRY(hipGetDevice(&dev));
            HIP_TRY(hipGetDeviceProperties(&prop, dev));
            n_cu = prop.multiProcessorCount;
        }
        if (n_cu != 256) return DASR_EINVAL;
    }
    hipStream_t s = as_stream(stream);
    static bool attr_set[4] = {false, false, false, false};
    const int v = (f16 ? 1 : 0) | (bwd ? 2 : 0);
#define DASR_CHAIN_LAUNCH(F16_, BWD_, NAME)                                                                                                              \
    {                                                                                                                                                    \
        auto kfn = conv_chain_kernel<F16_, BWD_>;                                                                                                        \
        if (!attr_set[v]) {                                                                                                                              \
            HIP_TRY(hipFuncSetAttribute((const void*)kfn, hipFuncAttributeMaxDynamicSharedMemorySize, C::LDS_BYTES));                                    \
            attr_set[v] = true;                                                                                                                          \
        }                                                                                                                                                \
        DASR_LAUNCH_TAG(NAME, kfn, dim3((unsigned)grid), dim3(256), C::LDS_BYTES, s, dev_layers, (const int*)dev_dep_chunk, (int)nlayers, tiles_y, tiles_x, \
                        dev_flags, dev_flags + grid, dev_err);                                                                                           \
    }
    if (v == 0) DASR_CHAIN_LAUNCH(false, false, "conv_chain_kernel<false, false>")
    else if (v == 1) DASR_CHAIN_LAUNCH(true, false, "conv_chain_kernel<true, false>")
    else if (v == 2) DASR_CHAIN_LAUNCH(false, true, "conv_chain_kernel<false, true>")
    else DASR_CHAIN_LAUNCH(true, true, "conv_chain_kernel<true, true>")
#undef DASR_CHAIN_LAUNCH
    return (int)hipGetLastError();
}

extern "C" int dasr_rdb_chain(const dasr_conv_params* dev_layers, const dasr_conv_params* host_layers, int32_t nlayers, uint32_t* dev_flags, int32_t* dev_err, void* stream) {
    if (!dev_layers || !host_layers || nlayers <= 0 || nlayers % 5 || !dev_flags || !dev_err) return DASR_EINVAL;
    const dasr_conv_params& p0 = host_layers[0];
    if (p0.prec != 1) return DASR_EINVAL;
    const int e0 = classify_epi(p0);
    const bool bwd = e0 == 68;
    if (!bwd && e0 != 67) return DASR_EINVAL;
    for (int i = 0; i < nlayers; ++i) {
        const dasr_conv_params& p = host_layers[i];
        const dasr_conv_params& pb = host_layers[i - i % 5];
        const int k = i % 5;
        if (p.kh != 3 || p.stride != 1 || p.pad != 1 || p.in_f32 || p.prec != 1 || p.ups || p.in_wrap || p.out16_lo || p.res1_lo || p.out16_f16) return DASR_EINVAL;
        if (p.Hin != p0.Hin || p.Win != p0.Win || p.Hout != p0.Hin || p.Wout != p0.Win || p.N != p0.N || p.out_stride > 1 || p.in_stride > 1 || p.out_W || p.out_oy || p.out_ox) return DASR_EINVAL;
        if (p.cin != 64 + 32 * k || p.mt != (k == 4 ? 2 : 1) || p.cout != 32 * p.mt || !p.w || !p.in.p || p.slope_ptr || p.mask_f32 || p.prelu_part) return DASR_EINVAL;
        if (p.in.p != pb.in.p || p.in.n_stride != pb.in.n_stride || p.in.cb_stride != pb.in.cb_stride) return DASR_EINVAL;
        const int epi = classify_epi(p);
        const bool ok = k < 4 ? epi == (bwd ? 68 : 67) : ((epi & ~(16 | 64)) == (bwd ? 168 : 169) && p.res1.p && p.alpha != 0.f);
        if (!ok) return DASR_EINVAL;
    }
    if (p0.N & 7) return DASR_EINVAL;
    const int tiles_x = (p0.Wout + ISC::TW - 1) / ISC::TW;
    auto geometry = [&](int th, int& q_out, int& tpw_out) -> bool {
        const int T = tiles_x * ((p0.Hout + th - 1) / th);
        if (T <= 0 || T > 32) return false;
        const long long per_xcd = (long long)T * p0.N / 8;
        for (int c = 32 - 32 % T; c >= T; c -= T)
            if (per_xcd % c == 0 && per_xcd / c <= ISC::MAX_TPW) {
                q_out = c, tpw_out = (int)(per_xcd / c);
                return true;
            }
        return false;
    };
    int th = 0, q = 0, tpw = 0, best = 1 << 30;
    for (int cand = 16; cand >= 4; cand >>= 1) {
        int qc = 0, tc = 0;
        if (!geometry(cand, qc, tc)) continue;
        const int cost = tc * (cand == 16 ? 43 : cand == 8 ? 30 : 24);
        if (cost < best) best = cost, th = cand, q = qc, tpw = tc;
    }
    if (!th) return DASR_EINVAL;
    const int grid = 8 * q;
    const int tiles_y = (p0.Hout + th - 1) / th;
    {
        static int n_cu = -1;
        if (n_cu < 0) {
            int dev = 0;
            hipDeviceProp_t prop;
            HIP_TRY(hipGetDevice(&dev));
            HIP_TRY(hipGetDeviceProperties(&prop, dev));
            n_cu = prop.multiProcessorCount;
        }
        if (n_cu != 256) return DASR_EINVAL;
    }
    unsigned* tickets = dev_flags + (long long)tiles_x * ((p0.Hout + 3) / 4) * p0.N;
    const int nrdb = nlayers / 5;
    hipStream_t st = as_stream(stream);
#define IS_GO(NTv, NWv)                                                                                                                                              \
    return bwd ? launch_rdb_is<false, true, NTv, NWv>(dev_layers, nrdb, tiles_y, tiles_x, tpw, dev_flags, tickets, dev_err, st, "rdb_is_kernel<false, true, " #NTv ", " #NWv ">", grid) \
               : launch_rdb_is<false, false, NTv, NWv>(dev_layers, nrdb, tiles_y, tiles_x, tpw, dev_flags, tickets, dev_err, st, "rdb_is_kernel<false, false, " #NTv ", " #NWv ">", grid)
    if (th == 16) { IS_GO(2, 8); }
    if (th == 8) { IS_GO(1, 8); }
    IS_GO(1, 4);
#undef IS_GO
}

extern "C" int dasr_conv(const dasr_conv_params* pp, void* stream) {
    dasr_conv_params p = *pp;
    p.xcd_remap = 1;
    if (p.pad_x == 0 && p.out_stride == 0 && p.kh != 2 && p.kh != 1) p.pad_x = -1;
    hipStream_t s = as_stream(stream);
    if (p.cin <= 0 || (p.cin & 15) || p.cout <= 0 || !p.w || !p.in.p) return DASR_EINVAL;
    if (!(p.mt == 1 || p.mt == 2) || !(p.prec >= 1 && p.prec <= 4)) return DASR_EINVAL;
    if (p.prec == 4 && (!p.in_f32 || p.mt != 1)) return DASR_EINVAL;
    if (p.prec == 2 && !p.in_f32 && (p.kh != 3 || p.stride != 1)) return DASR_EINVAL;
    int kcode = 0;
    if (p.kh == 4) kcode = p.stride == 2 ? 2 : 1;
    else if (p.kh == 2) kcode = 3;
    else if (p.kh == 5) kcode = 4;
    else if (p.kh == 1) kcode = 5;
    else if (p.kh == 3 && p.stride == 2) kcode = 6;
    const int key = (p.prec == 4 ? 3000 : p.prec == 3 ? 1000 : p.prec == 2 ? 2000 : 0) + (p.in_f32 ? 100 : 0) + p.mt * 10 + kcode;
    if (p.kh == 3 && ((p.stride != 1 && p.stride != 2) || (p.pad != 1 && !(p.pad >= 0 && p.pad <= 2 && p.stride == 1 && p.in_f32)))) return DASR_EINVAL;
    if (p.kh == 5 && (p.stride != 1 || p.pad != 2)) return DASR_EINVAL;
    if (p.kh == 1 && (p.stride != 1 || p.pad != 0)) return DASR_EINVAL;
    if (p.kh == 4 && ((p.stride != 1 && p.stride != 2) || p.pad < 0 || p.pad > 3)) return DASR_EINVAL;
    if (p.kh == 2 && (p.stride != 1 || p.pad < 0 || p.pad > 1)) return DASR_EINVAL;
    if (p.kh < 1 || p.kh > 5) return DASR_EINVAL;
    if (p.mask.p && (p.mask_f32 != 0) != (p.in_f32 != 0)) return DASR_EINVAL;
    if (p.ups && !p.in_f32 && p.prec != 2) return DASR_EINVAL;
    if (p.in_wrap < 0 || p.out16_lo < 0 || p.res1_lo < 0) return DASR_EINVAL;
    if (p.in_wrap || p.out16_lo || p.res1_lo) {
        if (p.in_f32 || p.kh != 3 || p.stride != 1 || p.pad != 1 || !(p.prec == 1 || p.prec == 2) || p.ups || p.out_stride > 1) return DASR_EINVAL;
        if (p.in_wrap && (p.cin >> 4) * 2 != p.in_wrap * 3) return DASR_EINVAL;
        if (p.out16_lo && !p.out_bf16.p) return DASR_EINVAL;
        if (p.res1_lo < 0 || (p.res1_lo && !p.res1.p)) return DASR_EINVAL;
    }
    switch (key) {
        case 10:
            switch (classify_epi(p)) {
                case 67: return launch_glds<1, 67>(p, s);
                case 68: return launch_glds<1, 68>(p, s);
                default: return launch_glds<1, 0>(p, s);
            }
        case 20:
            if (g_tune_rdb64 == 12 || (long long)p.N * ((p.Hout + 15) / 16) * ((p.Wout + 31) / 32) * ((p.cout + 63) / 64) > 256) {
                switch (classify_epi(p)) {
                    case 233: return launch_glds<2, 233>(p, s);
                    case 249: return launch_glds<2, 249>(p, s);
                    case 232: return launch_glds<2, 232>(p, s);
                    case 248: return launch_glds<2, 248>(p, s);
                    default: return launch_glds<2, 0>(p, s);
                }
            }
            switch (classify_epi(p)) {
                case 233: return launch_glds<2, 233, 8>(p, s);
                case 249: return launch_glds<2, 249, 8>(p, s);
                case 232: return launch_glds<2, 232, 8>(p, s);
                case 248: return launch_glds<2, 248, 8>(p, s);
                default: return launch_glds<2, 0, 8>(p, s);
            }
        case 110: return launch<1, true, 1, 3, 1, 4>(p, s);
        case 120: return launch<1, true, 2, 3, 1, 4>(p, s);
        case 1110: return launch<3, true, 1, 3, 1, 4>(p, s);
        case 1111: return launch<3, true, 1, 4, 1, 2>(p, s);
        case 1112: return launch<3, true, 1, 4, 2, 1>(p, s);
        case 1113: return launch<3, true, 1, 2, 1, 4>(p, s);
        case 1114: return launch<3, true, 1, 5, 1, 2>(p, s);
        case 1115: return launch<3, true, 1, 1, 1, 4>(p, s);
        case 1116: return launch<3, true, 1, 3, 2, 1>(p, s);
        case 2010:
            switch (classify_epi(p)) {
                case 67: return launch_glds<1, 67, 4, 0, true>(p, s);
                case 68: return launch_glds<1, 68, 4, 0, true>(p, s);
                case 64: return launch_glds<1, 64, 4, 0, true>(p, s);
                default: return launch_glds<1, 0, 4, 0, true>(p, s);
            }
        case 2020:
            if (p.res1.p) {
                const bool four = g_tune_rdb64 == 12 || (long long)p.N * ((p.Hout + 15) / 16) * ((p.Wout + 31) / 32) * ((p.cout + 63) / 64) > 256;
                switch (classify_epi(p)) {
                    case 233: return four ? launch_glds<2, 233, 4, 0, true>(p, s) : launch_glds<2, 233, 8, 0, true>(p, s);
                    case 249: return four ? launch_glds<2, 249, 4, 0, true>(p, s) : launch_glds<2, 249, 8, 0, true>(p, s);
                    case 232: return four ? launch_glds<2, 232, 4, 0, true>(p, s) : launch_glds<2, 232, 8, 0, true>(p, s);
                    case 248: return four ? launch_glds<2, 248, 4, 0, true>(p, s) : launch_glds<2, 248, 8, 0, true>(p, s);
                    default: return launch_glds<2, 0, 4, 0, true>(p, s);
                }
            }
            switch (classify_epi(p)) {
                case 67: return launch_glds<2, 67, 4, 0, true>(p, s);
                case 68: return launch_glds<2, 68, 4, 0, true>(p, s);
                case 64: return launch_glds<2, 64, 4, 0, true>(p, s);
                default: return launch_glds<2, 0, 4, 0, true>(p, s);
            }
        case 3110: return launch<4, true, 1, 3, 1, 4>(p, s);
        case 3111: return launch<4, true, 1, 4, 1, 2>(p, s);
        case 3112: return launch<4, true, 1, 4, 2, 1>(p, s);
        case 3113: return launch<4, true, 1, 2, 1, 4>(p, s);
        case 3114: return launch<4, true, 1, 5, 1, 2>(p, s);
        case 3115: return launch<4, true, 1, 1, 1, 4>(p, s);
        case 3116: return launch<4, true, 1, 3, 2, 1>(p, s);
        case 2110: return launch<2, true, 1, 3, 1, 4>(p, s);
        case 2120: return launch<2, true, 2, 3, 1, 4>(p, s);
        case 2111: return launch<2, true, 1, 4, 1, 2>(p, s);
        case 2112: return launch<2, true, 1, 4, 2, 1>(p, s);
        case 2113: return launch<2, true, 1, 2, 1, 4>(p, s);
        case 2123: return launch<2, true, 2, 2, 1, 4>(p, s);
        case 2114: return launch<2, true, 1, 5, 1, 2>(p, s);
        case 2115: return launch<2, true, 1, 1, 1, 4>(p, s);
        case 2116: return launch<2, true, 1, 3, 2, 1>(p, s);
        default: return DASR_EINVAL;
    }
}

extern "C" int dasr_conv_naive(const dasr_conv_params* pp, const float* w_ref, void* stream) {
    const dasr_conv_params& p = *pp;
    const long long total = (long long)p.N * p.cout * p.Hout * p.Wout;
    if (total <= 0) return DASR_EINVAL;
    DASR_LAUNCH(conv_naive_kernel, dim3((unsigned)((total + 255) / 256)), dim3(256), 0, as_stream(stream), p, w_ref);
    return (int)hipGetLastError();
}
```

dasr_amd/csrc/rdb_is.h:

```cpp
struct ISC {
    static constexpr int TW = 32, IW = 34;
    static constexpr int WGRAN = 18432, NSLOT = 4;
    static constexpr int LDS_BYTES = 163840;
    static constexpr int X_OFF = LDS_BYTES - 8192;
    static constexpr int BIAS_OFF = X_OFF;
    static constexpr int POLL_OFF = X_OFF + 2560;
    static constexpr int MAX_TPW = 8;
    static constexpr int F0_OFF = POLL_OFF + MAX_TPW * 64;
    static constexpr int DEC_OFF = F0_OFF + 64;
    static constexpr int TRC_OFF = DEC_OFF + 64;
    static constexpr int NSTEP = 34;
    static constexpr int PUB_DELAY = 1;
};
template <int NT_, int NW_ = 8>
struct ISCfg : ISC {
    static constexpr int NW = NW_, NTH = 64 * NW_;
    static constexpr int NT = NT_, TH = NW * NT, IH = TH + 2, NPIX = IH * IW;
    static constexpr int APIECE = NPIX * 2;
    static constexpr int AR = (APIECE + NTH - 1) / NTH;
    static constexpr int ACT_SLOT = (APIECE * 16 + 1023) / 1024 * 1024;
    static constexpr int W_OFF = NSLOT * ACT_SLOT;
    static constexpr int NWG = 4;
    static constexpr int WDIST = 3;
    static_assert(W_OFF + NWG * WGRAN <= X_OFF && WDIST < NWG && WDIST >= 2 && WDIST <= 5, "LDS budget / ring depth");
// ... 315 lines not shown
            const bool has_next = rn < nrdb;
            const int L0n = has_next ? 5 * rn : L0;
            const void* wp0 = layers[L0].w;
            const void* wp1 = layers[L0 + 1].w;
            const void* wp2 = layers[L0 + 2].w;
            const void* wp3 = layers[L0 + 3].w;
            const void* wp4 = layers[L0 + 4].w;
            const void* wpn0 = layers[L0n].w;
            const void* wpn1 = layers[L0n + 1].w;
            const void* wpn2 = layers[L0n + 2].w;
            auto wptr = [&](int u, bool next) -> const void* {
                return next ? (u == 0 ? wpn0 : u == 1 ? wpn1 : wpn2) : (u == 0 ? wp0 : u == 1 ? wp1 : u == 2 ? wp2 : u == 3 ? wp3 : wp4);
            };

            {
                const unsigned long long t0 = IS_T();
                is_wait_vm(__builtin_amdgcn_readfirstlane(issued - mark_x));
                __builtin_amdgcn_s_barrier();
                IS_ACC(4, IS_T() - t0);
            }
            const dasr_conv_params& p5 = layers[L0 + 4];
            const bool r1pre = p5.out_bf16.p != nullptr;
            if (r1pre) {
                const __amdgpu_buffer_rsrc_t rr1 = make_rsrc((const float*)p5.res1.p + (size_t)cur.n * p5.res1.n_stride);
                const unsigned r1_cb = (unsigned)p5.res1.cb_stride;
#pragma unroll
                for (int nt = 0; nt < NT; ++nt) {
                    const int oy = cur.oy0 + wave * NT + nt, ox = cur.ox0 + nn;
                    const bool pv = (oy < p5.Hout) & (ox < p5.Wout);
                    const unsigned pixel = (unsigned)(oy * p5.Wout + ox) * 16u;
#pragma unroll
                    for (int mi = 0; mi < 2; ++mi)
#pragma unroll
                        for (int gq = 0; gq < 4; ++gq) {
                            const int oc = mi * 32 + 8 * gq + 4 * kh2;
                            const u32x4 t = __builtin_amdgcn_raw_buffer_load_b128(rr1, pv ? ((unsigned)(oc >> 4) * r1_cb + pixel + (unsigned)(oc & 15)) * 4u : OOB, 0, 0);
#pragma unroll
                            for (int e = 0; e < 4; ++e) A5[mi][nt][4 * gq + e] = __uint_as_float(t[e]);
                        }
                }
            } else {
#pragma unroll
                for (int mi = 0; mi < 2; ++mi)
#pragma unroll
                    for (int nt = 0; nt < NT; ++nt)
#pragma unroll
                        for (int e = 0; e < 16; ++e) A5[mi][nt][e] = 0.f;
            }
#pragma unroll
            for (int nt = 0; nt < NT; ++nt)
#pragma unroll
                for (int e = 0; e < 16; ++e) A0[0][nt][e] = 0.f, A1[0][nt][e] = 0.f, A2[0][nt][e] = 0.f, A3[0][nt][e] = 0.f;

            bool arr_issued = false;
            int mark_act = 0;
            bool next_x_issued = false, next_rdy = false;
            const unsigned f0n = (unsigned)__builtin_amdgcn_readfirstlane(xi[sn]);

            auto request_group = [&](int c0) {
                issued += is_dma_act<C>(rin, smem + (c0 & 3) * C::ACT_SLOT, cur.goff, (unsigned)c0 * icb, wave, tid);
                issued += is_dma_act<C>(rin, smem + ((c0 + 1) & 3) * C::ACT_SLOT, cur.goff, (unsigned)(c0 + 1) * icb, wave, tid);
                arr_issued = true;
                mark_act = issued;
            };
            auto request_next_x = [&](const ISGeo<C>& nxt) {
                const dasr_conv_params& pn = layers[L0n];
                const __amdgpu_buffer_rsrc_t rinn = make_rsrc((const bf16_t*)pn.in.p + (size_t)nxt.n * pn.in.n_stride);
                const unsigned icbn = (unsigned)(pn.in.cb_stride * 2);
#pragma unroll
                for (int c = 0; c < 4; ++c) issued += is_dma_act<C>(rinn, smem + c * C::ACT_SLOT, nxt.goff, (unsigned)c * icbn, wave, tid);
                mark_x = issued;
                next_x_issued = true;
            };

            auto do_step = [&](auto tc) {
                constexpr int TT = decltype(tc)::value;
                constexpr ISStep d = IS_PROG[TT];
                constexpr int GK = is_group_of_step(TT);
                constexpr bool MUST = GK >= 1 && GK <= 4 && TT + 1 == IS_WIN1[GK];
                const char* abuf = smem + (d.c & 3) * C::ACT_SLOT;
                const char* wbuf = smem + C::W_OFF + (g % C::NWG) * C::WGRAN;
                char* wnext = smem + C::W_OFF + ((g + C::WDIST) % C::NWG) * C::WGRAN;
                if constexpr (GK != 0 && TT == IS_WIN0[GK > 0 ? GK : 1]) arr_issued = false;
                bool act_now = false, poll_now = false;
                unsigned target = 0;
                int pslot = 0;
                auto decided = [&]() -> bool {
                    const unsigned* dw = (const unsigned*)(smem + C::DEC_OFF) + ((g - 1) & 1) * 2;
                    return __builtin_amdgcn_readfirstlane(dw[0]) == target && __builtin_amdgcn_readfirstlane(dw[1]) == (unsigned)pslot;
                };
                bool need = false;
                if constexpr (GK >= 1 && GK <= 4) {
                    target = cur.f0 + (unsigned)(L0 + GK), pslot = cur.slot;
                    if (!arr_issued) {
                        if (decided()) act_now = true;
                        else need = true, poll_now = !pub_on && !poll_pend;
                    }
                } else if constexpr (GK == 5) {
                    if (has_next && rn > 0 && !next_rdy) {
                        target = f0n + (unsigned)L0n, pslot = sn;
                        if (decided()) next_rdy = true;
                        else need = true, poll_now = !poll_pend;
                    }
                }
                constexpr int EU_AFTER = is_epi_after(TT);
                auto prefetch_w = [&]() {
                    if (g + C::WDIST < total_steps) {
                        constexpr int T3 = (TT + C::WDIST) % C::NSTEP;
                        constexpr ISStep e = IS_PROG[T3];
                        constexpr bool NX = TT + C::WDIST >= C::NSTEP;
                        if constexpr (e.kind == 5) {
                            issued += is_dma_w<C::NTH>(make_rsrc(wptr(4, NX)), wnext, (unsigned)e.c * 18432u, 1152, wave, tid);
                        } else {
                            issued += is_dma_w<C::NTH>(make_rsrc(wptr(e.u0, NX)), wnext, (unsigned)e.c * 9216u, 576, wave, tid);
                            if constexpr (e.kind == 2) issued += is_dma_w<C::NTH>(make_rsrc(wptr(e.u1, NX)), wnext + 9216, (unsigned)e.c * 9216u, 576, wave, tid);
                        }
                    }
                };
                auto mid = [&](int s) {
                    if (s == 0) {
                        if (poll_now && wave == 0) {
                            if constexpr (GK == 5) {
                                const ISGeo<C> nq = geo_of(sn);
                                if (lane < 9) is_dma_poll(rflags, smem + C::POLL_OFF + sn * 64, nq.nbo);
                            } else {
                                if (lane < 9) is_dma_poll(rflags, smem + C::POLL_OFF + cur.slot * 64, cur.nbo);
                            }
                            ++issued;
                            poll_mark = issued;
                            poll_pend = true;
                        }
                        if constexpr (EU_AFTER < 0) prefetch_w();
                    }
                    if (s == 2) {
                        if constexpr (GK >= 1 && GK <= 4) {
                            if (act_now) request_group(4 + 2 * (GK - 1));
                        }
                    }
                };
                const unsigned long long t0 = IS_T();
                if constexpr (d.kind == 1) {
                    if constexpr (d.u0 == 0) is_body<NT, 1, 1024, 0, F16>(A0[0], A0[0], abuf, wbuf, baddr, aoff, mid);
                    else if constexpr (d.u0 == 1) is_body<NT, 1, 1024, 0, F16>(A1[0], A1[0], abuf, wbuf, baddr, aoff, mid);
                    else if constexpr (d.u0 == 2) is_body<NT, 1, 1024, 0, F16>(A2[0], A2[0], abuf, wbuf, baddr, aoff, mid);
                    else is_body<NT, 1, 1024, 0, F16>(A3[0], A3[0], abuf, wbuf, baddr, aoff, mid);
                } else if constexpr (d.kind == 2) {
                    if constexpr (d.u0 == 1) is_body<NT, 2, 1024, 9216, F16>(A1[0], A2[0], abuf, wbuf, baddr, aoff, mid);
                    else is_body<NT, 2, 1024, 9216, F16>(A2[0], A3[0], abuf, wbuf, baddr, aoff, mid);
                    static_assert(d.kind != 2 || (d.u0 == 1 && d.u1 == 2) || (d.u0 == 2 && d.u1 == 3), "pairs of the program");
                } else {
                    is_body<NT, 2, 2048, 1024, F16>(A5[0], A5[1], abuf, wbuf, baddr, aoff, mid);
                }
                MaskPre<NT> mpre;
                if constexpr (BWD && EU_AFTER >= 0 && EU_AFTER < 4) mask_prefetch<1, NT>(layers[L0 + EU_AFTER], mpre, tid, 0, cur.n, cur.oy0, cur.ox0);
                const unsigned long long t1 = IS_T();
                int nwait = issued - mk[C::WDIST - 2];
                bool do_pub = false;
                if (pub_on && g >= pub_due) do_pub = true, nwait = min(nwait, issued - pub_mark);
                if constexpr (MUST) {
                    if (arr_issued) nwait = min(nwait, issued - mark_act);
                }
                is_wait_vm(__builtin_amdgcn_readfirstlane(nwait));
                const unsigned long long t1b = IS_T();
                if (poll_pend && wave == 0) {
                    unsigned ib;
                    asm volatile("s_getreg_b32 %0, hwreg(HW_REG_IB_STS)" : "=s"(ib));
                    const int out = (int)((ib & 15u) | (((ib >> 22) & 3u) << 4));
                    if (out <= issued - poll_mark) {
                        poll_pend = false;
                        if (need) {
                            const unsigned v = ((const unsigned*)(smem + C::POLL_OFF))[pslot * 16 + (lane < 9 ? lane : 0)];
                            const bool rdy = __builtin_amdgcn_ballot_w64((int)(v - target) < 0) == 0ull;
                            if (lane < 2) ((unsigned*)(smem + C::DEC_OFF))[(g & 1) * 2 + lane] = lane == 0 ? (rdy ? target : target - 1u) : (unsigned)pslot;
                            __builtin_amdgcn_s_waitcnt(0xC07F);
                        }
                    }
                }
                __builtin_amdgcn_s_barrier();
                if (do_pub) flag_store();
#pragma unroll
                for (int k = 7; k > 0; --k) mk[k] = mk[k - 1];
                mk[0] = issued;
                const unsigned long long t2 = IS_T();
                IS_ACC(d.kind == 1 ? 0 : 1, t1 - t0);
                IS_ACC(2, t2 - t1);
                IS_ACC(d.kind == 1 ? 12 : 13, t1b - t1);
                IS_ACC(d.kind == 1 ? 14 : 15, t2 - t1b);
                IS_ACC(d.kind == 1 ? 8 : 9, 1ull);
                if constexpr (MUST) {
                    if (!arr_issued) {
                        block_until(cur, target);
                        request_group(4 + 2 * (GK - 1));
                        const unsigned long long t3 = IS_T();
                        __builtin_amdgcn_s_waitcnt(0x0F70);
                        __builtin_amdgcn_s_barrier();
                        IS_ACC(3, IS_T() - t3);
                    }
                }
                constexpr int EU = is_epi_after(TT);
                if constexpr (EU == 0) {
                    const unsigned long long t3 = IS_T();
                    const float c1 = r1pre ? p5.beta1 / p5.alpha : 1.f;
#pragma unroll
                    for (int mi = 0; mi < 2; ++mi)
#pragma unroll
                        for (int nt = 0; nt < NT; ++nt) {
                            A5[mi][nt] *= c1;
                            asm volatile("" : "+v"(A5[mi][nt]));
                        }
                    IS_ACC(7, IS_T() - t3);
                }
                if constexpr (EU >= 0) {
                    const unsigned long long t4 = IS_T();
                    const dasr_conv_params& p = layers[L0 + EU];
                    char* bl = smem + C::BIAS_OFF + par * 1280 + EU * 256;
                    if constexpr (EU == 4) {
                        if (has_next) {
                            if (rn > 0 && !next_rdy) {
                                const unsigned* dw = (const unsigned*)(smem + C::DEC_OFF) + (g & 1) * 2;
                                next_rdy = __builtin_amdgcn_readfirstlane(dw[0]) == f0n + (unsigned)L0n && __builtin_amdgcn_readfirstlane(dw[1]) == (unsigned)sn;
                            }
                        }
                        const bool two = p.res2.p != nullptr, sh = p.out_bf16.p != nullptr;
                        constexpr int E0 = BWD ? 160 : 161;
                        if (two && sh) conv_epilogue<false, 2, NT, 1, E0 + 80, F16 ? 1 : 0, false, true, true, true>(p, A5, bl, 0.f, tid, 0, cur.n, cur.oy0, cur.ox0);
                        else if (sh) conv_epilogue<false, 2, NT, 1, E0 + 64, F16 ? 1 : 0, false, true, true, true>(p, A5, bl, 0.f, tid, 0, cur.n, cur.oy0, cur.ox0);
                        else if (two) conv_epilogue<false, 2, NT, 1, E0 + 8 + 16, F16 ? 1 : 0, false, true, true, true>(p, A5, bl, 0.f, tid, 0, cur.n, cur.oy0, cur.ox0);
                        else conv_epilogue<false, 2, NT, 1, E0 + 8, F16 ? 1 : 0, false, true, true, true>(p, A5, bl, 0.f, tid, 0, cur.n, cur.oy0, cur.ox0);
                    } else {
                        auto epi14 = [&](f32x16 (&A)[1][NT]) {
                            if constexpr (BWD) conv_epilogue<false, 1, NT, 1, 68, F16 ? 1 : 0, true, true, true, true>(p, A, bl, 0.f, tid, 0, cur.n, cur.oy0, cur.ox0, &mpre);
                            else conv_epilogue<false, 1, NT, 1, 67, F16 ? 1 : 0, false, true, true, true>(p, A, bl, 0.f, tid, 0, cur.n, cur.oy0, cur.ox0);
                        };
                        if constexpr (EU == 0) epi14(A0);
                        else if constexpr (EU == 1) epi14(A1);
                        else if constexpr (EU == 2) epi14(A2);
                        else epi14(A3);
                    }
                    flush_pub();
                    pub_on = true, pub_mark = issued, pub_due = g + C::PUB_DELAY;
                    pub_off = cur.selfo, pub_val = cur.f0 + (unsigned)(L0 + EU + 1);
                    prefetch_w();
                    if constexpr (EU == 4) {
                        if (has_next && (rn == 0 || next_rdy)) request_next_x(geo_of(sn));
                        if constexpr (!BWD) {
                            if (has_next) {
#pragma unroll
                                for (int l = 0; l < 5; l += NW) {
                                    if (l + wave < 5) {
                                        const dasr_conv_params& pb = layers[L0n + l + wave];
                                        is_dma_bias(make_rsrc(pb.bias), smem + C::BIAS_OFF + (par ^ 1) * 1280 + (l + wave) * 256, (pb.bias != nullptr && lane < 32 * pb.mt) ? (unsigned)lane * 4u : OOB);
                                        ++issued;
                                    }
                                }
                            }
                        }
                    }
                    mk[0] = issued;
                    IS_ACC(EU == 4 ? 6 : 5, IS_T() - t4);
                }
                ++g;
            };
            auto run = [&](auto self, auto tc) -> void {
                constexpr int TT = decltype(tc)::value;
                if constexpr (TT < C::NSTEP) {
                    do_step(tc);
                    self(self, ISInt<TT + 1>{});
                }
            };
            run(run, ISInt<0>{});
            IS_ACC(10, 1ull);
            {
                const ISGeo<C> nxt = geo_of(sn);
                if (has_next && !next_x_issued) {
                    block_until(nxt, nxt.f0 + (unsigned)L0n);
                    request_next_x(nxt);
                }
                cur = nxt;
            }
        }
    }
    flush_pub();
    __builtin_amdgcn_s_waitcnt(0x0F70);
#ifdef DASR_TRACE
    if (g_trace && tid < 16) g_trace[(size_t)(1 << 20) + (size_t)blockIdx.x * 64 + tid] = ((unsigned long long*)(smem + C::TRC_OFF))[tid];
#endif
}

template <bool F16, bool BWD, int NT, int NW>
int launch_rdb_is(const dasr_conv_params* dev_layers, int nrdb, int tiles_y, int tiles_x, int tpw, unsigned* flags, unsigned* tickets, int* err, hipStream_t s, const char* name, int grid) {
    static bool attr_set = false;
    auto kfn = rdb_is_kernel<F16, BWD, NT, NW>;
    if (!attr_set) {
        HIP_TRY(hipFuncSetAttribute((const void*)kfn, hipFuncAttributeMaxDynamicSharedMemorySize, ISC::LDS_BYTES));
        attr_set = true;
    }
    DASR_LAUNCH_TAG(name, kfn, dim3((unsigned)grid), dim3(64 * NW), ISC::LDS_BYTES, s, dev_layers, nrdb, tiles_y, tiles_x, tpw, flags, tickets, err);
    return (int)hipGetLastError();
}
```

dasr_amd/dist.py:

```python
import os

import torch
import torch.distributed as dist


RANK_CONSISTENT_ENV = ('DASR_HR_PREC', 'DASR_RDB_PREC', 'DASR_VGG_PREC', 'DASR_VGG_BWD_PREC', 'DASR_VGG_NOGRAD_PREC', 'DASR_D_PREC', 'DASR_DSN_BWD16', 'DASR_DSN_FWD16', 'DASR_DSN_PRELU_FUSED',
                       'DASR_STREAMS', 'DASR_ENQ', 'DASR_CHAIN', 'DASR_CHAIN_FORM', 'DASR_CHAIN_SPLIT', 'DASR_TUNE', 'DASR_HIP_LIB', 'DASR_RCCL_NATIVE', 'DASR_DP_BACKEND', 'DASR_ALLOW_NONFINITE')


SHARED_DEVICE = False


def env_fingerprint():
    import hashlib
    items = [(k, os.environ.get(k, '')) for k in RANK_CONSISTENT_ENV]
    return hashlib.sha1(repr(items).encode()).hexdigest(), items


class DataParallelGroup:
    def __init__(self, backend=None, force=False):
        self.world = int(os.environ.get('WORLD_SIZE', '1'))
        self.rank = int(os.environ.get('RANK', '0'))
        self.local_rank = int(os.environ.get('LOCAL_RANK', '0'))
        self.backend = backend or os.environ.get('DASR_DP_BACKEND') or ('nccl' if torch.cuda.is_available() else 'gloo')
        self.force = bool(force)
        ndev = torch.cuda.device_count() if torch.cuda.is_available() else 0
        if self.backend == 'nccl' and ndev and self.local_rank >= ndev:
            raise RuntimeError('LOCAL_RANK %d but only %d visible device(s): one process per GPU (RCCL cannot share a device between ranks; '
                               'DASR_DP_BACKEND=gloo does, for tests)' % (self.local_rank, ndev))
        self.device_index = self.local_rank % ndev if ndev else 0
        self.shared_device = False
        if (self.world > 1 or force) and not dist.is_initialized():
            os.environ.setdefault('MASTER_ADDR', '127.0.0.1')
            os.environ.setdefault('MASTER_PORT', '29500')
            if self.backend == 'nccl':
                torch.cuda.set_device(self.device_index)
            dist.init_process_group(self.backend, rank=self.rank, world_size=self.world)
        self.comm_stream = torch.cuda.Stream() if (self.backend == 'nccl' and torch.cuda.is_available()) else None
        self.pending = []
        self.native = None
        if self.world > 1:
            self.check_env_agreement()
            self._detect_shared_device(ndev)
        if self.backend == 'nccl' and self.active and os.environ.get('DASR_RCCL_NATIVE', '0') == '1':
            self._init_native()

    def check_env_agreement(self):
        digest, items = env_fingerprint()
        got = [None] * self.world
        dist.all_gather_object(got, (self.rank, digest, items))
        if len(set(g[1] for g in got)) > 1:
            ref = dict(got[0][2])
            diff = sorted(set(k for g in got for k, v in g[2] if ref.get(k) != v))
            raise RuntimeError('data-parallel ranks disagree on %s: %s' % (', '.join(diff), '; '.join('rank %d: %s' % (g[0], {k: v for k, v in g[2] if k in diff}) for g in got)))

    def _detect_shared_device(self, ndev):
        global SHARED_DEVICE
        if not ndev:
            return
        import socket
        got = [None] * self.world
        dist.all_gather_object(got, (socket.gethostname(), self.device_index))
        self.shared_device = len(set(got)) < len(got)
        if self.shared_device:
            SHARED_DEVICE = True

    def _init_native(self):
        import ctypes as C
        from . import _lib
        L = _lib.lib()
        ident = [None]
        if self.rank == 0:
            buf = C.create_string_buffer(128)
            _lib.check(L.dasr_rccl_unique_id(buf), 'dasr_rccl_unique_id')
            ident = [buf.raw]
        if self.world > 1:
            dist.broadcast_object_list(ident, src=0)
        comm = C.c_void_p()
        _lib.check(L.dasr_rccl_init(ident[0], self.rank, self.world, C.byref(comm)), 'dasr_rccl_init')
        self.native = comm

    @property
    def active(self):
        return self.world > 1 or self.force

    def all_reduce_here(self, flat_slice):
        if self.active and flat_slice.numel():
            if self.native is not None:
                from . import _lib
                _lib.check(_lib.lib().dasr_allreduce(self.native, flat_slice.data_ptr(), flat_slice.numel(), torch.cuda.current_stream().cuda_stream),
                           'dasr_allreduce')
            else:
                dist.all_reduce(flat_slice, op=dist.ReduceOp.SUM)

    @property
    def grad_scale(self):
        return 1.0 / self.world

    def reduce_async(self, flat_slice):
        if not self.active or flat_slice.numel() == 0:
            return
        if self.comm_stream is not None:
            ev = torch.cuda.Event()
            ev.record(torch.cuda.current_stream())
            with torch.cuda.stream(self.comm_stream):
                self.comm_stream.wait_event(ev)
                self.all_reduce_here(flat_slice)
            self.pending.append(flat_slice)
        else:
            dist.all_reduce(flat_slice, op=dist.ReduceOp.SUM)

    def wait(self):
        if self.comm_stream is not None and self.pending:
            torch.cuda.current_stream().wait_stream(self.comm_stream)
            self.pending = []

    def allreduce_mean(self, flat):
        self.reduce_async(flat)
        self.wait()

    def barrier(self):
        if self.active:
            dist.barrier()

    def sync_error_words(self, words):
        if not self.active or not words:
            return
        dev = 'cuda' if self.backend == 'nccl' else 'cpu'
        t = torch.stack([w.reshape(-1)[0].to(dev) for w in words]).to(torch.int32)
        dist.all_reduce(t, op=dist.ReduceOp.MAX)
        for i, w in enumerate(words):
            w.reshape(-1)[0:1].copy_(t[i:i + 1])

    def max_over_ranks(self, value):
        if not self.active:
            return value
        dev = 'cuda' if self.backend == 'nccl' else 'cpu'
        t = torch.tensor([value], dtype=torch.float64, device=dev)
        dist.all_reduce(t, op=dist.ReduceOp.MAX)
        return float(t.item())

    def broadcast_params(self, flat):
        if self.active:
            dist.broadcast(flat, src=0)


def shard_minibatch(batch, rank, world):
    out = {}
    for k, v in batch.items():
        if torch.is_tensor(v):
            n = v.shape[0]
            assert n % world == 0, 'global batch %d not divisible by world size %d' % (n, world)
            per = n // world
            out[k] = v[rank * per:(rank + 1) * per]
        else:
            out[k] = v
    return out
```

dasr_amd/engine.py:

```python
import ctypes as C
from collections import OrderedDict

import torch

from . import _lib
from ._lib import Tensor, ConvParams, WgradPart, WgradReducePart, PackDesc, Op, make_op

SLOPE = 0.2

BUCKETS = {1: 'G forward: trunk fea_conv .. LR_conv (DSN: whole generator)', 2: 'G HR tail forward', 3: 'G HR tail backward (data + weight gradients)',
           4: 'G trunk data gradient (DSN: generator backward)', 5: 'G trunk weight gradients (deferred phase + reduce)', 6: 'perceptual net forward, gradient images',
           7: 'perceptual net forward, target images (one pass)', 8: 'perceptual net data gradient', 9: 'discriminator forward',
           10: 'discriminator backward (data + weight gradients)', 11: 'G other backward (LR_conv, fea_conv)', 0: 'losses / filters / layout / optimiser'}


def _stream():
    return C.c_void_p(torch.cuda.current_stream().cuda_stream)


def ceil_div(a, b):
    return (a + b - 1) // b


class BTensor:
# ... 116 lines not shown
        return r

    def finalize(self):
        dev = self.params.device
        self.buf = torch.zeros(self.size, dtype=torch.bfloat16, device=dev)
        arr = (PackDesc * len(self.descs))(*self.descs)
        self.desc_dev = torch.frombuffer(bytearray(bytes(arr)), dtype=torch.uint8).to(dev)
        self.prefix_dev = torch.tensor(self.prefix, dtype=torch.int64, device=dev)

    def ptr(self, ref):
        return self.buf.data_ptr() + 2 * ref.off

    def op(self):
        return make_op(_lib.OP_PACK, descs_dev=self.desc_dev.data_ptr(), ndesc=len(self.descs), total_pieces=self.prefix[-1],
                       piece_prefix_dev=self.prefix_dev.data_ptr(), params_flat=self.params.flat.data_ptr(), packed=self.buf.data_ptr())

    def run(self):
        ops = (Op * 1)(self.op())
        _lib.check(_lib.lib().dasr_run_ops(C.cast(ops, C.c_void_p), 1, _stream()), 'pack')


_GEN = 0
_CONV_FIELDS = frozenset(n for n, _ in ConvParams._fields_)


def patch(op, **args):
    global _GEN
    for name, value in args.items():
        if op.op == _lib.OP_CONV and name != 'tag':
            if name not in _CONV_FIELDS:
                raise TypeError('dasr_conv_params has no field %r' % name)
            setattr(op.conv, name, value)
        else:
            op.set(name, value)
    _GEN += 1


def set_reduce_scale(lists, scale):
    scale = C.c_float(scale).value
    changed = False
    for ol in lists:
        for o in ol.ops:
            if o.op == _lib.OP_WGRAD_REDUCE:
                name = 'scale'
            elif (o.op == _lib.OP_BNORM_BWD and o.get('dgamma')) or o.op == _lib.OP_BNORM_SECOND:
                name = 'pscale'
            else:
                continue
            if o.get(name) != scale:
                patch(o, **{name: scale})
                changed = True
    return changed


class OpList:
    def __init__(self):
        self.ops = []
        self.keep = []
        self._arr, self._gen = None, -1

    def add(self, o):
        self.ops.append(o)
        self._arr = None

    def extend(self, other):
        self.ops.extend(other.ops)
        self.keep.extend(other.keep)
        self._arr = None

    def slice(self, lo=0, hi=None):
        ol = OpList()
        ol.ops = self.ops[lo:hi]
        return ol

    def pop(self, idx):
        self._arr = None
        return self.ops.pop(idx)

    def tag(self, bucket, start=0, end=None):
        for o in self.ops[start:end]:
            if o.get('tag') == 0:
                patch(o, tag=bucket)
        return self

    def set(self, idx, name, value):
        self.ops[idx].set(name, value)
        if self._arr is not None:
            self._arr[idx].set(name, value)

    def _image(self):
        if self._arr is None or self._gen != _GEN:
            self._arr, self._gen = (Op * len(self.ops))(*self.ops), _GEN
        return self._arr

    def safe_cuts(self, chunk):
        key = ('cuts', chunk, len(self.ops))
        if getattr(self, '_cuts_key', None) != key:
            cuts, redirected, last = [0], False, 0
            for i, o in enumerate(self.ops):
                if o.op == _lib.OP_SET_STREAM:
                    redirected = bool(o.get('stream'))
                if i + 1 - last >= chunk and not redirected:
                    cuts.append(i + 1)
                    last = i + 1
            if cuts[-1] != len(self.ops):
                cuts.append(len(self.ops))
            self._cuts, self._cuts_key = cuts, key
        return self._cuts

    def run(self, lo=0, hi=None):
        if not self.ops:
            return
        hi = len(self.ops) if hi is None else min(hi, len(self.ops))
        if hi <= lo:
            return
        L = _lib.lib()
        rc = L.dasr_run_ops(C.c_void_p(C.addressof(self._image()) + lo * C.sizeof(Op)), hi - lo, _stream())
        if rc != 0:
            k = L.dasr_last_failed_op() + lo
            raise _lib.DasrHipError('dasr_run_ops: op #%d (kind %d) failed with code %d' % (k, self.ops[k].op if 0 <= k < len(self.ops) else -1, rc))


def run_interleaved(lists, streams, chunk=None):
    chunk = chunk or 48
    cuts = [l.safe_cuts(chunk) for l in lists]
    for k in range(max(len(c) for c in cuts) - 1):
        for l, st, c in zip(lists, streams, cuts):
            if k + 1 < len(c):
                with torch.cuda.stream(st):
                    l.run(c[k], c[k + 1])


def run_parallel(lists, streams):
    import os
    lists = [l for l in lists]
    if len(lists) == 1 or os.environ.get('DASR_ENQ', 'mt') == 'chunk' or torch.cuda.is_current_stream_capturing():
        return run_interleaved(lists, streams)
    n = len(lists)
    ptrs = (C.c_void_p * n)(*[C.addressof(l._image()) for l in lists])
    cnts = (C.c_int32 * n)(*[len(l.ops) for l in lists])
    sts = (C.c_void_p * n)(*[st.cuda_stream for st in streams])
    L = _lib.lib()
    rc = L.dasr_run_ops_mt(ptrs, cnts, sts, n)
    if rc != 0:
        k = L.dasr_last_failed_op()
        li, oi = (k >> 24) & 0x7f, k & 0xffffff
        kind = lists[li].ops[oi].op if (0 <= li < n and 0 <= oi < len(lists[li].ops)) else -1
        raise _lib.DasrHipError('dasr_run_ops_mt: list %d op #%d (kind %d) failed with code %d' % (li, oi, kind, rc))


def conv_op(pack, ref, inp, in_f32, cin, Hin, Win, Hout, Wout, N, bias=None, kh=3, stride=1, pad=1, ups=0, act=0, slope=SLOPE,
            mask=None, mask_f32=0, alpha=1.0, res1=None, beta1=0.0, res2=None, beta2=0.0, out_f32=None, out_bf16=None, gamma=1.0,
            pad_x=-1, out_stride=1, out_oy=0, out_ox=0, out_W=0, slope_ptr=None, in_stride=1, in_oy=0, in_ox=0, in_W=0, flops=None, in_scale=0.0, out16_f16=0,
            in_wrap=0, out16_lo=0, res1_lo=0):
    assert cin == ref.cin_pad, (cin, ref.cin_pad)
    o = Op()
    o.op = _lib.OP_CONV
    o.flops = float(flops) if flops is not None else 2.0 * N * Hout * Wout * kh * kh * (cin // 3 if in_wrap else cin) * ref.cout
    p = o.conv
    p.inp, p.in_f32, p.Hin, p.Win, p.ups, p.cin = inp, int(in_f32), Hin, Win, ups, cin
    p.w, p.w_lo_off, p.bias = pack.ptr(ref), ref.lo_off, bias
    p.cout, p.Hout, p.Wout, p.N = ref.cout, Hout, Wout, N
    p.kh, p.stride, p.pad, p.prec, p.mt = kh, stride, pad, ref.prec, ref.mt
    p.act, p.slope = act, slope
    p.mask, p.mask_f32 = (mask if mask is not None else NULL_T), mask_f32
    p.alpha = alpha
    p.res1, p.beta1 = (res1 if res1 is not None else NULL_T), beta1
    p.res2, p.beta2 = (res2 if res2 is not None else NULL_T), beta2
    p.out_f32 = out_f32 if out_f32 is not None else NULL_T
    p.out_bf16 = out_bf16 if out_bf16 is not None else NULL_T
    p.gamma = gamma
    p.pad_x, p.out_stride, p.out_oy, p.out_ox, p.out_W = pad_x, out_stride, out_oy, out_ox, out_W
    p.slope_ptr = slope_ptr
    p.in_stride, p.in_oy, p.in_ox, p.in_W = in_stride, in_oy, in_ox, in_W
    p.in_scale = in_scale if (ref.prec in (2, 4) and in_f32) else 0.0
    p.out16_f16 = int(out16_f16)
    p.res1_lo = int(res1_lo)
    p.in_wrap, p.out16_lo = int(in_wrap), int(out16_lo)
    return o


class ConvChain:

    def __init__(self, ops, dep_chunks, n_images, n_tiles, device, flags=None, err=None, form='layer'):
        assert len(ops) == len(dep_chunks) and ops
        assert form in ('layer', 'is')
        self.form = form
        n = len(ops)
        self.host = (_lib.ConvParams * n)(*[o.conv for o in ops])
        raw = torch.frombuffer(bytearray(bytes(self.host)), dtype=torch.uint8)
        self.dev = raw.to(device)
        self.dep = torch.tensor([int(d) for d in dep_chunks], dtype=torch.int32, device=device)
        self.flags = flags if flags is not None else torch.zeros(n_images * n_tiles + 8, dtype=torch.int32, device=device)
        self.err = err if err is not None else torch.zeros(1, dtype=torch.int32, device=device)
        self.n = n
        self.flops = sum(o.flops for o in ops)

    def op(self):
        chain = dict(dev_layers=self.dev.data_ptr(), host_layers=C.cast(self.host, C.c_void_p).value, dev_flags=self.flags.data_ptr(),
                     dev_err=self.err.data_ptr(), nlayers=self.n)
        if self.form == 'is':
            return make_op(_lib.OP_RDB_CHAIN, flops=self.flops, **chain)
        return make_op(_lib.OP_CONV_CHAIN, flops=self.flops, dev_dep_chunk=self.dep.data_ptr(), **chain)

    def check(self):
        e = int(self.err.item())
        if e:
            raise RuntimeError('conv chain: device error word %d (bit 1: a neighbour wait gave up)' % e)


class _WgradEmit:

    def __init__(self):
        self.parts = []
        self.f16, self.g_scale = False, 0.0
        self.flops = 0.0
        self.ppu = 0

    def emit(self, ops, workspace, device, grad_ptr, **finalize_kw):
        self.finalize(workspace, device, **finalize_kw)
        pair = self.ops(grad_ptr)
        for o in pair:
            ops.add(o)
        ops.keep.append(self)
        return pair


class WgradGroup(_WgradEmit):

    def __init__(self, kh, stride):
        super().__init__()
        self.kh, self.stride = kh, stride

    def add_conv(self, g, g_f32, g_planes_total, inp, in_f32, in_planes_total, cout, cin, Hin, Win, Hout, Wout, N,
                 dst_w_off, dst_b_off, pad=None, ups=0, f16=False, g_scale=0.0, split=None, more_pairs=()):
        assert not f16 or (g_f32 and in_f32)
        assert split is None or f16
        self.f16 = bool(f16) or self.f16
        if f16 and g_scale:
            self.g_scale = float(g_scale)
        ntaps = self.kh * self.kh
        tpp = ntaps if ntaps <= 16 else 10
        self.tpp = tpp
        self.flops += 2.0 * N * Hout * Wout * ntaps * cin * cout
        pad = (self.kh - 1) // 2 if pad is None else pad
        cin_pad = ceil_div(cin, 16) * 16
        variants = ([(g, inp)] if split is None else [(g, inp), (g, split[1]), (split[0], inp)]) + list(more_pairs)
        for oc0 in range(0, cout, 32):
            for c0 in range(0, cin_pad, 64):
                for tap0 in range(0, ntaps, tpp):
                    rp = WgradReducePart()
                    first = dst_b_off is not None and c0 == 0 and tap0 == 0
                    wps = []
                    for vi, (gv, xv) in enumerate(variants):
                        wp = WgradPart()
                        wp.g, wp.g_f32 = gv(oc0), int(g_f32)
                        wp.inp, wp.in_f32 = xv(c0), int(in_f32)
                        wp.ups = ups
                        wp.n_ctiles = min(2, ceil_div(cin_pad - c0, 32))
                        wp.g_planes = min(2, g_planes_total - oc0 // 16)
                        wp.in_planes = min(4, in_planes_total - c0 // 16)
                        wp.Hin, wp.Win, wp.Hout, wp.Wout, wp.N = Hin, Win, Hout, Wout, N
                        wp.kh, wp.stride, wp.pad, wp.tap0 = self.kh, self.stride, pad, tap0
                        wp.want_bias = 1 if (first and vi == 0) else 0
                        wp.g_scale = float(g_scale) if f16 else 0.0
                        wps.append(wp)
                    rp.ntaps, rp.oc0, rp.c0, rp.cout, rp.cin, rp.n_ctiles = min(tpp, ntaps - tap0), oc0, c0, cout, cin, wps[0].n_ctiles
                    rp.tap0, rp.ntaps_total = tap0, ntaps
                    rp.dst_w_off = dst_w_off
                    rp.dst_b_off = dst_b_off if first else -1
                    for wp in wps:
                        self.parts.append((wp, rp if wp is wps[0] else None, len(wps) if wp is wps[0] else 0))

    def finalize(self, workspace, device, target_wgs=768):
        wp0 = self.parts[0][0]
        ph = 2 if self.stride == 2 else (8 if self.kh in (3, 1) else 4)
        ntiles = wp0.N * ceil_div(wp0.Hout, ph) * ceil_div(wp0.Wout, 16)
        nparts = len(self.parts)
        self.nsplit = max(1, min(ntiles, target_wgs // nparts))
        if self.nsplit >= 16:
            self.nsplit -= self.nsplit % 8
        off = 0
        reds = []
        for wp, rp, nvar in self.parts:
            wp.ws_off = off
            if rp is not None:
                rp.ws_off = off
                rp.nsplit = self.nsplit * nvar
                rp.bias_nsplit = self.nsplit if nvar > 1 else 0
                rp.split_stride, rp.tap_stride, rp.bias_stride = self.tpp * 2048, 2048, 32
                reds.append(rp)
            off += self.nsplit * self.tpp * 2048
        for wp, rp, nvar in self.parts:
            wp.ws_bias_off = off
            if rp is not None:
                rp.ws_bias_off = off
            off += self.nsplit * 32
        self.ws_floats = off
        self.workspace = workspace
        workspace.reserve(off)
        wa = (WgradPart * nparts)(*[p[0] for p in self.parts])
        ra = (WgradReducePart * len(reds))(*reds)
        self.n_red = len(reds)
        self.w_dev = torch.frombuffer(bytearray(bytes(wa)), dtype=torch.uint8).to(device)
        self.r_dev = torch.frombuffer(bytearray(bytes(ra)), dtype=torch.uint8).to(device)

    def ops(self, grad_ptr, scale=1.0):
        f32s = set((p[0].g_f32, p[0].in_f32) for p in self.parts)
        assert f32s in ({(0, 0)}, {(1, 1)}), 'a wgrad group must be all-bf16 or all-f32'
        a = make_op(_lib.OP_WGRAD, flops=float(self.flops), parts_dev=self.w_dev.data_ptr(), nparts=len(self.parts), nsplit=self.nsplit,
                    kh=self.kh, stride=self.stride, f32=self.parts[0][0].g_f32 | (2 if self.f16 else 0))
        gs = self.g_scale
        b = make_op(_lib.OP_WGRAD_REDUCE, parts_dev=self.r_dev.data_ptr(), nparts=self.n_red, grad_flat=grad_ptr, scale=scale,
                    few_splits=1 if (self.tpp <= 16 and all(rp is None or rp.nsplit <= 4 for _, rp, _ in self.parts)) else 0,
                    inv_prescale=1.0 / gs if gs else 0.0)
        self.workspace.register(a, b)
        return [a, b]


class WgradGroup3(_WgradEmit):

    kh, stride = 3, 1

    def add_block(self, g_view, g_planes, in_view, in_planes, n_ctiles, Hin, Win, Hout, Wout, N, tiles, want_bias, f32=False, ups=0):
        assert 1 <= len(tiles) <= 3 and g_planes <= 6
        wp = WgradPart()
        wp.g, wp.g_f32, wp.inp, wp.in_f32 = g_view, int(f32), in_view, int(f32)
        wp.ups, wp.n_ctiles, wp.g_planes, wp.in_planes = ups, n_ctiles, g_planes, in_planes
        wp.Hin, wp.Win, wp.Hout, wp.Wout, wp.N = Hin, Win, Hout, Wout, N
        wp.kh, wp.stride, wp.pad, wp.want_bias = 3, 1, 1, int(bool(want_bias))
        self.parts.append((wp, [(i, t) for i, t in enumerate(tiles) if t is not None]))
# ... 128 lines not shown
```

dasr_amd/rrdbnet.py:

```python
import os
from collections import OrderedDict

import torch

from . import _lib
from .engine import (BTensor, ParamStore, PackRegistry, OpList, WgradGroup, WgradGroup3, Workspace, conv_op, ceil_div, SLOPE, ConvChain, GradScale,
                     set_reduce_scale)
from ._lib import Op, Tensor, make_op

GC = 32
_SUBPIXEL_ROWS = {0: ((0,), (1, 2)), 1: ((0, 1), (2,))}


def rrdbnet_param_spec(in_nc, out_nc, nf, nb, upsample_mode='upconv'):
    spec = [('model.0.weight', (nf, in_nc, 3, 3)), ('model.0.bias', (nf,))]
    for i in range(nb):
        for r in (1, 2, 3):
            for j in range(1, 6):
                cin = nf + (j - 1) * GC
                cout = GC if j < 5 else nf
                p = 'model.1.sub.%d.RDB%d.conv%d.0.' % (i, r, j)
                spec += [(p + 'weight', (cout, cin, 3, 3)), (p + 'bias', (cout,))]
    spec += [('model.1.sub.%d.weight' % nb, (nf, nf, 3, 3)), ('model.1.sub.%d.bias' % nb, (nf,))]
    ups = ((3, nf), (6, nf)) if upsample_mode == 'upconv' else ((2, 4 * nf), (5, 4 * nf))
    for idx, co in ups + ((8, nf), (10, out_nc)):
        spec += [('model.%d.weight' % idx, (co, nf, 3, 3)), ('model.%d.bias' % idx, (co,))]
    return spec


class RRDBNetHIP:
    act_slope = SLOPE

    def __init__(self, in_nc=3, out_nc=3, nf=64, nb=23, upscale=4, device='cuda', rdb_prec=None, stream_prec=3, upsample_mode='upconv'):
        assert upscale == 4 and nf % 32 == 0 and in_nc <= 16 and out_nc <= 16
        if upsample_mode not in ('upconv', 'pixelshuffle'):
            raise NotImplementedError('upsample mode [{:s}] is not found'.format(str(upsample_mode)))
        self.in_nc, self.out_nc, self.nf, self.nb, self.upsample_mode = in_nc, out_nc, nf, nb, upsample_mode
        self.device = torch.device(device)
        self.params = ParamStore(rrdbnet_param_spec(in_nc, out_nc, nf, nb, upsample_mode), self.device)
        if rdb_prec is None:
            rdb_prec = int(os.environ.get('DASR_RDB_PREC', '1'))
        if rdb_prec not in (1, 2):
            raise ValueError('rdb_prec / DASR_RDB_PREC must be 1 (bf16) or 2 (f16 storage)')
        self.rdb_prec, self.stream_prec = rdb_prec, stream_prec
        self.rdb_f16 = rdb_prec == 2
        self.chain = os.environ.get('DASR_CHAIN', '1') == '1' and not self.rdb_f16
        self.chain_form = os.environ.get('DASR_CHAIN_FORM', 'auto')
        assert self.chain_form in ('auto', 'is', 'layer')
        self.chain_err = torch.zeros(1, dtype=torch.int32, device=self.device)
        self.hr_prec = int(os.environ.get('DASR_HR_PREC', '2')) if stream_prec == 3 else stream_prec
        if self.hr_prec not in (2, 3):
            raise ValueError('DASR_HR_PREC must be 2 (f16 storage) or 3 (split-bf16 on f32 tensors)')
        self.hr_f16s = self.hr_prec == 2
        self.ps = upsample_mode == 'pixelshuffle'
        if self.ps and not self.hr_f16s:
            raise NotImplementedError('the PixelShuffle upsampler is built on the f16-storage HR tail (unset DASR_HR_PREC)')
        self.pack = PackRegistry(self.params)
        self._register_packs()
        self.pack.finalize()
        self.plans = {}

    def _seg_fwd(self, key, cout, cin):
        return (self.params.off(key), cout, cin, 0, cin, 0, 0)

    def _register_packs(self):
        self._register_stream_packs()
        self._register_trunk_packs()

    def _register_stream_packs(self):
        nf, P, sp = self.nf, self.params, self.stream_prec
        hp = self.hr_prec
        hmt = 1
        self.pk = {}
        self.pk['fea'] = self.pack.add(nf, 16, 9, 1, sp, [(P.off('model.0.weight'), nf, self.in_nc, 0, self.in_nc, 0, 0)])
        lr = 'model.1.sub.%d.weight' % self.nb
        for name, key, cout in (('lr', lr, nf), ('up1', 'model.3.weight', nf), ('up2', 'model.6.weight', nf),
                                ('hr0', 'model.8.weight', nf), ('hr1', 'model.10.weight', self.out_nc)):
            if self.ps and name in ('up1', 'up2'):
                continue
            pr = sp if name == 'lr' else hp
            if self.hr_f16s and name != 'lr':
                continue
            self.pk[name] = self.pack.add(cout, nf, 9, hmt if (pr == 2 and cout % 64 == 0) else 1, pr, [self._seg_fwd(key, cout, nf)])
            cin_b = ceil_div(cout, 16) * 16
            self.pk[name + '_b'] = self.pack.add(nf, cin_b, 9, hmt if pr == 2 else 1, pr, [(P.off(key), cout, nf, 0, cout, 0, 1)])
        if self.hr_f16s:
            mtH = 2 if nf % 64 == 0 else 1
            ups = (('up1', 'model.2.weight', 4 * nf), ('up2', 'model.5.weight', 4 * nf)) if self.ps else (('up1', 'model.3.weight', nf), ('up2', 'model.6.weight', nf))
            for name, key, co in ups + (('hr0', 'model.8.weight', nf),):
                self.pk[name] = self.pack.add(co, nf, 9, mtH, 2, [self._seg_fwd(key, co, nf)])
                self.pk[name + '_b'] = self.pack.add(nf, co, 9, mtH, 2, [(P.off(key), co, nf, 0, co, 0, 1)])
            self.pk['hr1'] = self.pack.add(self.out_nc, nf, 9, 1, 2, [self._seg_fwd('model.10.weight', self.out_nc, nf)])
            self.pk['hr1_b'] = self.pack.add(nf, 16, 9, mtH, 2, [(P.off('model.10.weight'), self.out_nc, nf, 0, self.out_nc, 0, 1)])
        self.subpixel = not self.hr_f16s
        rows = _SUBPIXEL_ROWS
        for name, key in (() if self.hr_f16s else (('up1', 'model.3.weight'), ('up2', 'model.6.weight'))):
            for py in (0, 1):
                for px in (0, 1):
                    fw = [sum(1 << (ky * 3 + kx) for ky in rows[py][a] for kx in rows[px][b]) for a in (0, 1) for b in (0, 1)]
                    bw = [sum(1 << (ky * 3 + kx) for ky in rows[py][1 - a] for kx in rows[px][1 - b]) for a in (0, 1) for b in (0, 1)]
                    self.pk[(name, py, px)] = self.pack.add(nf, nf, 4, hmt, hp, [self._seg_fwd(key, nf, nf)], tapmap=[0, 0, 0, 0], src_ntaps=9, tapmasks=fw)
                    self.pk[(name + '_b', py, px)] = self.pack.add(nf, nf, 4, hmt, hp, [(P.off(key), nf, nf, 0, nf, 0, 1)], tapmap=[0, 0, 0, 0], src_ntaps=9,
                                                                   tapmasks=bw)

    def _register_trunk_packs(self):
        nf, P = self.nf, self.params
        mt_nf = 2 if (nf >= 64 and self.rdb_prec in (1, 2)) else 1
        for i in range(self.nb):
            for r in (1, 2, 3):
                pre = 'model.1.sub.%d.RDB%d.conv' % (i, r)
                for j in range(1, 6):
                    cin = nf + (j - 1) * GC
                    cout = GC if j < 5 else nf
                    self.pk[(i, r, j)] = self.pack.add(cout, cin, 9, mt_nf if j == 5 else 1, self.rdb_prec,
                                                       [self._seg_fwd('%s%d.0.weight' % (pre, j), cout, cin)])
                for k in range(4, -1, -1):
                    segs = []
                    for j in range(5, k, -1):
                        cout_j = GC if j < 5 else nf
                        cin_j = nf + (j - 1) * GC
                        start = 0 if j == 5 else nf + (4 - j) * GC
                        src_c0 = 0 if k == 0 else nf + (k - 1) * GC
                        segs.append((P.off('%s%d.0.weight' % (pre, j)), cout_j, cin_j, start, cout_j, src_c0, 1))
                    cin_b = nf + (4 - k) * GC
                    cout_b = nf if k == 0 else GC
                    self.pk[(i, r, 'b', k)] = self.pack.add(cout_b, cin_b, 9, mt_nf if k == 0 else 1, self.rdb_prec, segs)

    def repack(self):
        self.pack.run()

    def chain_ok(self, N, h, w):
        return self.chain_split(N, h, w) > 0

    def chain_split(self, N, h, w):
        return self.chain_choice(N, h, w)[1]

    @staticmethod
    def is_geometry(N, T):
        if N % 8 or T <= 0 or T > 32:
            return None
        per_xcd = N * T // 8
        for q in range(32 - 32 % T, T - 1, -T):
            if per_xcd % q == 0 and per_xcd // q <= 8:
                return q, per_xcd // q
        return None

    @staticmethod
    def is_launch(N, h, w):
        best, cost = None, None
        for th, c in ((16, 43), (8, 30), (4, 24)):
            g = RRDBNetHIP.is_geometry(N, ceil_div(h, th) * ceil_div(w, 32))
            if g is not None and (cost is None or g[1] * c < cost):
                best, cost = (th,) + g, g[1] * c
        return best

    def chain_choice(self, N, h, w):
        T = ceil_div(h, 16) * ceil_div(w, 32)
        ntiles = N * T
        if not self.chain:
            return None, 0, 'chained launches are off (DASR_CHAIN=0 or f16 dense blocks)'
        if getattr(self, 'debug_taps', ()):
            return None, 0, 'debug taps between the layers'
        from . import dist as _dist
        if _dist.SHARED_DEVICE:
            return None, 0, 'another rank of this job shares the device'
        if not hasattr(self, '_cus'):
            self._cus = torch.cuda.get_device_properties(self.device).multi_processor_count if self.device.type == 'cuda' else 0
        if self._cus != 256:
            return None, 0, 'the device does not expose 256 CUs (partitioned, or no GPU)'
        why = []
        if self.chain_form in ('auto', 'layer'):
            k = ntiles // 512
            kmax = int(os.environ.get('DASR_CHAIN_SPLIT', '4'))
            if k >= 1 and k <= kmax and ntiles == 512 * k and N % k == 0 and (N // k) % 8 == 0:
                return 'layer', k, ''
            why.append('layer form: %d tiles are not 512 k (k <= %d) with N / k a multiple of 8' % (ntiles, kmax))
        if self.chain_form in ('auto', 'is'):
            if RRDBNetHIP.is_launch(N, h, w) is not None and self.nf == 64:
                return 'is', 1, ''
            why.append('input-stationary form: needs nf 64, N %% 8 == 0 and q <= 32 workgroups per XCD with q a multiple of the %d tiles per image, q dividing the %s tiles per XCD, '
                       'at most 8 tiles per workgroup' % (T, ('%d' % (ntiles // 8)) if N % 8 == 0 else 'N x tiles / 8'))
        return None, 0, '; '.join(why)

    def plan(self, N, h, w, replica=0, store=None, n0=0):
        key = (N, h, w, replica, id(store) if store is not None else 0, n0)
        if key not in self.plans:
            self.plans[key] = self._make_plan(N, h, w, replica, store=store, n0=n0)
        return self.plans[key]

    def _make_plan(self, *args, **kw):
        return _Plan(self, *args, **kw)

    defer_wgrad = True

    def trunk_store(self, N, h, w):
        key = (N, h, w)
        st = self.__dict__.setdefault('_stores', {})
        if key not in st:
            st[key] = TrunkStore(self, N, h, w)
        return st[key]

    def state_dict(self):
        return self.params.state_dict()

    def load_state_dict(self, sd, strict=True):
        self.params.load_state_dict(sd, strict)
        self.repack()

    INFER_CACHE = 2

    def forward(self, x):
        N, _, h, w = x.shape
        key = (N, h, w)
        cache = self.__dict__.setdefault('infer_plans', OrderedDict())
        p = cache.pop(key, None)
        if p is None:
            while len(cache) >= self.INFER_CACHE:
                cache.popitem(last=False)
            p = self._make_plan(N, h, w, inference=True)
        cache[key] = p
        p.set_input(x)
        p.fwd.run()
        return p.read_output()


def _sub_batch_conv(o, n0, n, N):
    import ctypes as C
    q = Op()
    C.memmove(C.addressof(q), C.addressof(o), C.sizeof(Op))
    c = q.conv
    assert c.N == N and not c.res1_lo and not c.in_wrap and not c.out16_lo
    for name, esz in (('inp', 4 if c.in_f32 else 2), ('mask', 4 if c.mask_f32 else 2), ('res1', 4), ('res2', 4), ('out_f32', 4), ('out_bf16', 2)):
        t = getattr(c, name)
        if t.p:
            t.p = t.p + n0 * t.n_stride * esz
    c.N = n
    q.flops = o.flops * n / N
    return q


def rdb_wgrad_parts(grp, nf, pre, P, Gs, S, h, w, N):
    gt = []
    for j in (5, 4, 3, 2, 1):
        cout_j = nf if j == 5 else GC
        for oc0 in range(0, cout_j, 32):
            gt.append(dict(j=j, oc0=oc0, cout=cout_j, cin=nf + (j - 1) * GC))
    n = 0
    for c0 in range(0, nf + 4 * GC, 64):
        need = [t for t in gt if t['cin'] > c0]
        blk_ch = min(64, nf + 4 * GC - c0)
        for k0 in range(0, len(need), 3):
            sub = need[k0:k0 + 3]
            tiles = []
            for t in sub:
                wkey = '%s%d.0.' % (pre, t['j'])
                tiles.append(dict(dst_w_off=P.off(wkey + 'weight'), dst_b_off=P.off(wkey + 'bias') if c0 == 0 else None,
                                  cout=t['cout'], cin=t['cin'], oc0=t['oc0'], c0=c0,
                                  n_ctiles=min(2, ceil_div(min(t['cin'] - c0, 64), 32))))
            grp.add_block(Gs.view(32 * k0), 2 * len(sub), S.view(c0), blk_ch // 16, ceil_div(blk_ch, 32),
                          h, w, h, w, N, tiles, want_bias=(c0 == 0))
            n += 1
    return n, 2.0 * N * h * w * 9 * sum((nf + (j - 1) * GC) * (GC if j < 5 else nf) for j in range(1, 6))


class TrunkStore(GradScale):

    def __init__(self, net, N, h, w):
        self.net, self.N, self.h, self.w = net, N, h, w
        dev, nf, nb = net.device, net.nf, net.nb
        sc = nf + 4 * GC
        mk = lambda: torch.zeros((N, ceil_div(sc, 16), h, w, 16), dtype=torch.float16 if net.rdb_f16 else torch.bfloat16, device=dev)
        super().__init__(net.rdb_f16, headroom=0.04)
        self.slab_t = [mk() for _ in range(3 * nb)]
        self.gslab_t = [mk() for _ in range(3 * nb)]
        self.sc = sc
        self.ws = Workspace(dev)
        self._build_phase()
        self.ws.finalize()

    def slab(self, ridx, n0=0, N=None):
        N = self.N if N is None else N
        return BTensor.wrap(self.slab_t[ridx][n0:n0 + N], self.sc, False)

    def gslab(self, ridx, n0=0, N=None):
        N = self.N if N is None else N
        return BTensor.wrap(self.gslab_t[ridx][n0:n0 + N], self.sc, False)

    def _build_phase(self):
        net, N, h, w = self.net, self.N, self.h, self.w
        nf, nb, P = net.nf, net.nb, net.params
        target = 256
        gmax = 4
        self.phase = OpList()
        self.groups = []
        hi_rrdb = nb
        ppr = None
        while hi_rrdb > 0:
            if ppr is None:
                tmp = WgradGroup3()
                ppu, _ = rdb_wgrad_parts(tmp, nf, 'model.1.sub.0.RDB1.conv', P, self.gslab(0), self.slab(0), h, w, N)
                ppr = 3 * ppu
            G = 1
            while G * 2 <= hi_rrdb and G * 2 <= gmax and G * 2 * ppr <= target:
                G *= 2
            lo_rrdb = hi_rrdb - G
            grp = WgradGroup3()
            for i in range(hi_rrdb - 1, lo_rrdb - 1, -1):
                for r in (3, 2, 1):
                    ridx = 3 * i + (r - 1)
                    _, fl = rdb_wgrad_parts(grp, nf, 'model.1.sub.%d.RDB%d.conv' % (i, r), P, self.gslab(ridx), self.slab(ridx), h, w, N)
                    grp.flops += fl
            if net.rdb_f16:
                grp.f16, grp.g_scale = True, self.gscale
            first = len(self.phase.ops)
            reduce_op = grp.emit(self.phase, self.ws, net.device, P.grad.data_ptr(), target_wgs=target, ppu=ppu)[1]
            if net.rdb_f16:
                self.register_reduce(reduce_op)
            lo = P.off('model.1.sub.%d.RDB1.conv1.0.weight' % lo_rrdb)
            hi = P.off('model.1.sub.%d.RDB1.conv1.0.weight' % hi_rrdb) if hi_rrdb < nb else P.off('model.1.sub.%d.weight' % nb)
            self.groups.append((first, len(self.phase.ops), lo, hi))
            hi_rrdb = lo_rrdb
        self.phase.tag(5)

    def set_grad_scale(self, scale):
        return set_reduce_scale([self.phase], scale)


class _Plan:

    def __init__(self, net, N, h, w, replica=0, inference=False, store=None, n0=0):
        self.net, self.N, self.h, self.w = net, N, h, w
        dev, nf, nb = net.device, net.nf, net.nb
        self.inference = inference
        self.replica = replica
        self.defer = not inference
        self.shared_store = store is not None
        self.store = store if store is not None else (TrunkStore(net, N, h, w) if self.defer else None)
        self.n0 = n0
        self.grad = net.params.grad if (replica == 0 or inference) else torch.zeros_like(net.params.grad)
        import math
        self.gscale = float(2.0 ** max(0, int(math.floor(math.log2(max(1, N * 3 * 16 * h * w)))) - 3))
        P, pack, pk = net.params, net.pack, net.pk
        H2, W2, H4, W4 = 2 * h, 2 * w, 4 * h, 4 * w
        sc = nf + 4 * GC
        B = lambda C_, H, W, f32: BTensor(N, C_, H, W, f32, dev)
        self.x_nchw = torch.zeros((N, net.in_nc, h, w), dtype=torch.float32, device=dev)
        self.sr_nchw = torch.zeros((N, net.out_nc, H4, W4), dtype=torch.float32, device=dev)
        self.x_in = B(16, h, w, True)
        self.fea = B(nf, h, w, True)
        if inference:
            ab = [BTensor(N, sc, h, w, False, dev, f16=net.rdb_f16) for _ in range(2)]
            self.slabs = [ab[i & 1] for i in range(3 * nb)]
        else:
            self.slabs = [self.store.slab(r, n0, N) for r in range(3 * nb)]
        self.stream = [B(nf, h, w, True) for _ in range(4)]
        self.t0 = B(nf, h, w, True)
        hs = net.hr_f16s
        Bh = (lambda C_, H, W: BTensor(N, C_, H, W, False, dev, f16=True)) if hs else (lambda C_, H, W: B(C_, H, W, True))
        self.t0h = Bh(nf, h, w) if hs else None
        self.u1 = Bh(nf, H2, W2)
        self.u2 = Bh(nf, H4, W4)
        if net.ps:
            self.ps1, self.ps2 = Bh(4 * nf, h, w), Bh(4 * nf, H2, W2)
            if not inference:
                self.g_ps1, self.g_ps2 = Bh(4 * nf, h, w), Bh(4 * nf, H2, W2)
        self.h0 = Bh(nf, H4, W4)
        self.sr = B(16, H4, W4, True)
        if inference:
            self._build_forward()
            return
        self.g_sr = B(16, H4, W4, True)
        self.g_sr16 = Bh(16, H4, W4) if hs else None
        self.g4a = Bh(nf, H4, W4)
        self.g4b = Bh(nf, H4, W4)
        self.g2a = Bh(nf, H2, W2)
        self.g2b = Bh(nf, H2, W2)
        self.g_t0 = B(nf, h, w, True)
        self.gstream = [B(nf, h, w, True) for _ in range(4)]
        self.n_gslab = 3 * nb
        self.gslab = [self.store.gslab(3 * nb - 1 - k, n0, N) for k in range(3 * nb)]
        self.g_fea = B(nf, h, w, True)
        self.ws = Workspace(dev)
        self._build_forward()
        self._build_backward()
        self.ws.finalize()

    def take_f16_loss_gradient(self):
        if self.g_sr16 is None or getattr(self, '_loss16_taken', False) or hasattr(self, 'whole_step'):
            return None
        o = self.bwd.ops[0]
        assert o.op == _lib.OP_CVT_F16 and o.get('y').p == self.g_sr16.view().p
        self.bwd.pop(0)
        self.tail_end -= 1
        self._marks = [(idx - 1, lo, hi) for idx, lo, hi in self._marks]
        self._segments = None
        self._loss16_taken = True
        return self.g_sr16.view(), self.gscale

    def check_chain(self):
        if getattr(self, 'chain', None) is not None:
            try:
                self.chain.check()
            except RuntimeError as e:
                raise RuntimeError(str(e) + '.  The chained trunk launches (dasr_conv_chain) need the GPU to themselves -- another process sharing the '
                                   'device breaks their workgroup placement; DASR_CHAIN=0 restores one launch per conv.')

    def set_input(self, x):
        self.x_nchw.copy_(x)

    def read_output(self):
        if self._out_ops is not None:
            self._out_ops.run()
        return self.sr_nchw

    def _add_output_op(self, fwd, o):
        if self.inference:
            fwd.add(o)
            self._out_ops = None
        else:
            self._out_ops = OpList()
            self._out_ops.add(o)

    def _build_forward(self):
        net, N, h, w = self.net, self.N, self.h, self.w
        nf, nb, P, pack, pk = net.nf, net.nb, net.params, net.pack, net.pk
        H2, W2, H4, W4 = 2 * h, 2 * w, 4 * h, 4 * w
        ops = OpList()
        ops.add(make_op(_lib.OP_NCHW2B, src=self.x_nchw.data_ptr(), N=N, C=net.in_nc, H=h, W=w, dst_f32=self.x_in.view()))
        f16 = int(net.rdb_f16)
        ops.add(conv_op(pack, pk['fea'], self.x_in.view(), True, 16, h, w, h, w, N, bias=P.ptr('model.0.bias'),
                        out_f32=self.fea.view(), out_bf16=self.slabs[0].view(0), out16_f16=f16))
        X = self.fea
        free = list(self.stream)
        self.rdb_in = []
        tiles = ceil_div(h, 16) * ceil_div(w, 32)
        form, nsub, why = (None, 0, 'inference plan') if self.inference else net.chain_choice(N, h, w)
        if nsub and (self.shared_store or self.replica > 0 or getattr(net, 'concurrent_replicas', 1) > 1):
            form, nsub, why = None, 0, 'the plan is one of several concurrent sub-batch replicas'
        self.chain_form, self.chain_why = form, why
        if not self.inference:
            import logging
            logging.getLogger('base').info('RRDBNet trunk at %d x %d x %d: %s' % (N, h, w, ('%d chained launch(es) per direction, %s form' % (nsub, form)) if nsub else ('one launch per conv (%s)' % why)))
        chain = [] if nsub else None
        trunk_ops = ops if chain is None else OpList()
        main_ops, ops = ops, trunk_ops
        for i in range(nb):
            Xrrdb = X
            for r in (1, 2, 3):
                ridx = 3 * i + (r - 1)
                S = self.slabs[ridx]
                pre = 'model.1.sub.%d.RDB%d.conv' % (i, r)
                for j in range(1, 5):
                    cin = nf + (j - 1) * GC
                    ops.add(conv_op(pack, pk[(i, r, j)], S.view(0), False, cin, h, w, h, w, N, bias=P.ptr('%s%d.0.bias' % (pre, j)),
                                    act=1, out_bf16=S.view(cin), out16_f16=f16))
                last = (ridx == 3 * nb - 1)
                Y = next(b for b in free if b is not X and b is not Xrrdb)
                nxt = None if last else self.slabs[ridx + 1].view(0)
                if r < 3:
                    ops.add(conv_op(pack, pk[(i, r, 5)], S.view(0), False, nf + 4 * GC, h, w, h, w, N, bias=P.ptr(pre + '5.0.bias'),
                                    alpha=0.2, res1=X.view(), beta1=1.0, out_f32=Y.view(), out_bf16=nxt, out16_f16=f16))
                else:
                    ops.add(conv_op(pack, pk[(i, r, 5)], S.view(0), False, nf + 4 * GC, h, w, h, w, N, bias=P.ptr(pre + '5.0.bias'),
                                    alpha=0.04, res1=X.view(), beta1=0.2, res2=Xrrdb.view(), beta2=1.0, out_f32=Y.view(), out_bf16=nxt, out16_f16=f16))
                X = Y
            if i in getattr(net, 'debug_taps', ()):
                self.taps = getattr(self, 'taps', {})
                self.taps[i] = BTensor(N, nf, h, w, True, net.device)
                ops.add(make_op(_lib.OP_AXPBY, x=X.view(), a=1.0, N=N, C=nf, H=h, W=w, out_f32=self.taps[i].view(), gamma=1.0))
        ops = main_ops
        self.chain = None
        if chain is not None:
            body = [o for o in trunk_ops.ops if o.op == _lib.OP_CONV]
            assert len(body) == len(trunk_ops.ops) == 15 * nb
            deps = [0 if k % 5 == 0 else (o.conv.cin // 16) - GC // 16 for k, o in enumerate(body)]
            per = N // nsub
            self.chains = []
            if self.chain_form == 'is':
                ch = ConvChain(body, deps, N, ceil_div(h, 4) * ceil_div(w, 32), net.device, err=net.chain_err, form='is')
                self.chains.append(ch)
                ops.add(ch.op())
                ops.keep.append(ch)
            else:
                for sb in range(nsub):
                    sub = body[:-1] if nsub == 1 else [_sub_batch_conv(o, sb * per, per, N) for o in body[:-1]]
                    ch = ConvChain(sub, deps[:-1], per, tiles, net.device, err=net.chain_err)
                    self.chains.append(ch)
                    ops.add(ch.op())
                    ops.keep.append(ch)
                ops.add(body[-1])
            self.chain = self.chains[0]
        self._build_tail_forward(ops, X)

    def _build_tail_forward(self, ops, X):
        net, N, h, w = self.net, self.N, self.h, self.w
        nf, nb, P, pack, pk = net.nf, net.nb, net.params, net.pack, net.pk
        H2, W2, H4, W4 = 2 * h, 2 * w, 4 * h, 4 * w
        sl = net.act_slope
        self.x_last = X
        lrb = 'model.1.sub.%d.bias' % nb
        if net.hr_f16s:
            ops.add(conv_op(pack, pk['lr'], X.view(), True, nf, h, w, h, w, N, bias=P.ptr(lrb), res1=self.fea.view(), beta1=1.0,
                            out_f32=self.t0.view(), out_bf16=self.t0h.view(), out16_f16=1))
            ops.tag(1)
            if net.ps:
                for name, bkey, src, pre, dst, hi, wi in (('up1', 'model.2.bias', self.t0h, self.ps1, self.u1, h, w), ('up2', 'model.5.bias', self.u1, self.ps2, self.u2, H2, W2)):
                    ops.add(conv_op(pack, pk[name], src.view(), False, nf, hi, wi, hi, wi, N, bias=P.ptr(bkey), act=1, slope=sl, out_bf16=pre.view(), out16_f16=1))
                    ops.add(make_op(_lib.OP_PIXSHUF, src=pre.view(), N=N, C4=4 * nf, H=hi, W=wi, dst=dst.view()))
            for name, bkey, src, dst, hi, wi in (() if net.ps else (('up1', 'model.3.bias', self.t0h, self.u1, h, w), ('up2', 'model.6.bias', self.u1, self.u2, H2, W2))):
                ops.add(conv_op(pack, pk[name], src.view(), False, nf, hi, wi, 2 * hi, 2 * wi, N, bias=P.ptr(bkey), ups=1, act=1, out_bf16=dst.view(),
                                out16_f16=1))
            ops.add(conv_op(pack, pk['hr0'], self.u2.view(), False, nf, H4, W4, H4, W4, N, bias=P.ptr('model.8.bias'), act=1, slope=sl, out_bf16=self.h0.view(),
                            out16_f16=1))
            ops.add(conv_op(pack, pk['hr1'], self.h0.view(), False, nf, H4, W4, H4, W4, N, bias=P.ptr('model.10.bias'), out_f32=self.sr.view()))
            self._add_output_op(ops, make_op(_lib.OP_B2NCHW, src=self.sr.view(), N=N, C=net.out_nc, H=H4, W=W4, dst=self.sr_nchw.data_ptr()))
            self.fwd = ops.tag(2)
            return
        ops.add(conv_op(pack, pk['lr'], X.view(), True, nf, h, w, h, w, N, bias=P.ptr(lrb), res1=self.fea.view(), beta1=1.0,
                        out_f32=self.t0.view()))
        ops.tag(1)
        for name, bkey, src, dst, hi, wi in (('up1', 'model.3.bias', self.t0, self.u1, h, w), ('up2', 'model.6.bias', self.u1, self.u2, H2, W2)):
            if not net.subpixel:
                ops.add(conv_op(pack, pk[name], src.view(), True, nf, hi, wi, 2 * hi, 2 * wi, N, bias=P.ptr(bkey), ups=1, act=1, out_f32=dst.view()))
                continue
            for py in (0, 1):
                for px in (0, 1):
                    ops.add(conv_op(pack, pk[(name, py, px)], src.view(), True, nf, hi, wi, hi, wi, N, bias=P.ptr(bkey), kh=2, stride=1, pad=1 - py,
                                    pad_x=1 - px, act=1, out_f32=dst.view(), out_stride=2, out_oy=py, out_ox=px, out_W=2 * wi,
                                    flops=2.0 * N * hi * wi * 9 * nf * nf))
        ops.add(conv_op(pack, pk['hr0'], self.u2.view(), True, nf, H4, W4, H4, W4, N, bias=P.ptr('model.8.bias'), act=1,
                        out_f32=self.h0.view()))
        ops.add(conv_op(pack, pk['hr1'], self.h0.view(), True, nf, H4, W4, H4, W4, N, bias=P.ptr('model.10.bias'),
                        out_f32=self.sr.view()))
        self._add_output_op(ops, make_op(_lib.OP_B2NCHW, src=self.sr.view(), N=N, C=net.out_nc, H=H4, W=W4, dst=self.sr_nchw.data_ptr()))
        self.fwd = ops.tag(2)

    def _wg(self, ops, conv_key, g, g_f32, inp, in_f32, cout, cin, Hin, Win, Hout, Wout, ups=0, groups=None, f16=False):
        P = self.net.params
        grp = WgradGroup(3, 1)
        grp.add_conv(g.view, g_f32, g.planes, inp.view, in_f32, inp.planes, cout, cin, Hin, Win, Hout, Wout, self.N,
                     P.off(conv_key + 'weight'), P.off(conv_key + 'bias'), ups=ups, f16=f16, g_scale=self.gscale)
        grp.emit(ops, self.ws, self.net.device, self.grad.data_ptr())

    def _subpixel_dgrad(self, ops, name, g_hi, g_lo, hl, wl, mask):
        net, pack, pk, N = self.net, self.net.pack, self.net.pk, self.N
        first = True
        for py in (0, 1):
            for px in (0, 1):
                ops.add(conv_op(pack, pk[(name, py, px)], g_hi.view(), True, net.nf, hl, wl, hl, wl, N, kh=2, stride=1, pad=py, pad_x=px,
                                mask=mask.view() if mask is not None else None, mask_f32=1, slope=SLOPE,
                                res1=None if first else g_lo.view(), beta1=0.0 if first else 1.0, out_f32=g_lo.view(),
                                in_stride=2, in_oy=py, in_ox=px, in_W=2 * wl, flops=2.0 * N * hl * wl * 9 * net.nf * net.nf, in_scale=self.gscale))
                first = False

    def _event(self):
        ev = _lib.lib().dasr_event_create()
        if not ev:
            raise _lib.DasrHipError('hipEventCreate failed')
        self._events = getattr(self, '_events', [])
        self._events.append(ev)
        return ev

    def _build_backward(self):
        net, N, h, w = self.net, self.N, self.h, self.w
        nf, nb, P, pack, pk = net.nf, net.nb, net.params, net.pack, net.pk
        H2, W2, H4, W4 = 2 * h, 2 * w, 4 * h, 4 * w
        ops = OpList()
        g_h0, g_u2, g_up2 = self.g4a, self.g4b, self.g4a
        f16 = net.hr_prec == 2
        gs = self.gscale
        if net.hr_f16s:
            self._build_backward_tail_f16(ops)
        else:
            self._build_backward_tail_f32(ops, f16, gs)
        ops.tag(3)
        self.tail_end = len(ops.ops)
        self._build_backward_trunk(ops)

    def _wg3_target(self, nparts):
        return 256 // max(1, getattr(self.net, 'concurrent_replicas', 1))

    def _wg3(self, ops, conv_key, g, inp, cout, cin, Hin, Win, Hout, Wout, ups=0, f16=True, g_scale=None):
        P, N = self.net.params, self.N
        grp = WgradGroup3()
        octs = list(range(0, cout, 32))
        for c0 in range(0, cin, 64):
            blk = min(64, cin - c0)
            for k0 in range(0, len(octs), 3):
                sub = octs[k0:k0 + 3]
                tiles = [dict(dst_w_off=P.off(conv_key + 'weight'), dst_b_off=P.off(conv_key + 'bias') if c0 == 0 else None, cout=cout, cin=cin,
                              oc0=oc0, c0=c0, n_ctiles=min(2, ceil_div(blk, 32))) for oc0 in sub]
                grp.add_block(g.view(sub[0]), min(2 * len(sub), g.planes - sub[0] // 16), inp.view(c0), ceil_div(blk, 16), ceil_div(blk, 32),
                              Hin, Win, Hout, Wout, N, tiles, want_bias=(c0 == 0), ups=ups)
        if f16:
            grp.f16, grp.g_scale = True, self.gscale if g_scale is None else g_scale
        grp.flops = 2.0 * N * Hout * Wout * 9 * cin * cout
        grp.emit(ops, self.ws, self.net.device, self.grad.data_ptr(), target_wgs=self._wg3_target(len(grp.parts)))

    def _build_backward_tail_f16(self, ops):
        net, N, h, w = self.net, self.N, self.h, self.w
        nf, pack, pk, gs = net.nf, net.pack, net.pk, self.gscale
        H2, W2, H4, W4 = 2 * h, 2 * w, 4 * h, 4 * w
        g_h0, g_u2, g_up2, g_u1, g_up1 = self.g4a, self.g4b, self.g4a, self.g2a, self.g2b
        sl = net.act_slope

        def downsum(src, hl, wl, mask, dst_f32, dst_f16, out_scale):
            ops.add(make_op(_lib.OP_DOWNSUM_F16, src=src.view(), N=N, C=nf, H=hl, W=wl, mask=mask and mask.view(), slope=sl, out_scale=out_scale,
                            dst_f32=dst_f32 and dst_f32.view(), dst_f16=dst_f16 and dst_f16.view()))

        ops.add(make_op(_lib.OP_CVT_F16, x=self.g_sr.view(), N=N, C=net.out_nc, H=H4, W=W4, scale=gs, y=self.g_sr16.view()))
        self._wg3(ops, 'model.10.', self.g_sr16, self.h0, net.out_nc, nf, H4, W4, H4, W4)
        ops.add(conv_op(pack, pk['hr1_b'], self.g_sr16.view(), False, 16, H4, W4, H4, W4, N, mask=self.h0.view(), mask_f32=0, slope=sl, out_bf16=g_h0.view(),
                        out16_f16=1))
        self._wg3(ops, 'model.8.', g_h0, self.u2, nf, nf, H4, W4, H4, W4)
        ops.add(conv_op(pack, pk['hr0_b'], g_h0.view(), False, nf, H4, W4, H4, W4, N, mask=self.u2.view(), mask_f32=0, slope=sl, out_bf16=g_u2.view(), out16_f16=1))
        if net.ps:
            for key, name, g_hi, pre, g_pre, src, g_lo, hl, wl, last in (('model.5.', 'up2', g_u2, None, self.g_ps2, self.u1, g_u1, H2, W2, False),
                                                                          ('model.2.', 'up1', g_u1, self.ps1, self.g_ps1, self.t0h, None, h, w, True)):
                ops.add(make_op(_lib.OP_PIXUNSHUF, gsrc=g_hi.view(), mask=pre and pre.view(), slope=sl, N=N, C4=4 * nf, H=hl, W=wl, gdst=g_pre.view()))
                self._wg3(ops, key, g_pre, src, 4 * nf, nf, hl, wl, hl, wl)
                if last:
                    ops.add(conv_op(pack, pk[name + '_b'], g_pre.view(), False, 4 * nf, hl, wl, hl, wl, N, alpha=1.0 / gs, out_f32=self.g_t0.view()))
                else:
                    ops.add(conv_op(pack, pk[name + '_b'], g_pre.view(), False, 4 * nf, hl, wl, hl, wl, N, out_bf16=g_lo.view(), out16_f16=1))
            return
        self._wg3(ops, 'model.6.', g_u2, self.u1, nf, nf, H2, W2, H4, W4, ups=1)
        ops.add(conv_op(pack, pk['up2_b'], g_u2.view(), False, nf, H4, W4, H4, W4, N, out_bf16=g_up2.view(), out16_f16=1))
        downsum(g_up2, H2, W2, self.u1, None, g_u1, 1.0)
        self._wg3(ops, 'model.3.', g_u1, self.t0h, nf, nf, h, w, H2, W2, ups=1)
        ops.add(conv_op(pack, pk['up1_b'], g_u1.view(), False, nf, H2, W2, H2, W2, N, out_bf16=g_up1.view(), out16_f16=1))
        downsum(g_up1, h, w, None, self.g_t0, None, 1.0 / gs)

    def _build_backward_tail_f32(self, ops, f16, gs):
        net, N, h, w = self.net, self.N, self.h, self.w
        nf, nb, P, pack, pk = net.nf, net.nb, net.params, net.pack, net.pk
        H2, W2, H4, W4 = 2 * h, 2 * w, 4 * h, 4 * w
        g_h0, g_u2, g_up2 = self.g4a, self.g4b, self.g4a
        self._wg(ops, 'model.10.', self.g_sr, True, self.h0, True, net.out_nc, nf, H4, W4, H4, W4, f16=f16)
        ops.add(conv_op(pack, pk['hr1_b'], self.g_sr.view(), True, 16, H4, W4, H4, W4, N, mask=self.h0.view(), mask_f32=1,
                        out_f32=g_h0.view(), in_scale=gs))
        self._wg(ops, 'model.8.', g_h0, True, self.u2, True, nf, nf, H4, W4, H4, W4, f16=f16)
        ops.add(conv_op(pack, pk['hr0_b'], g_h0.view(), True, nf, H4, W4, H4, W4, N, mask=self.u2.view(), mask_f32=1,
                        out_f32=g_u2.view(), in_scale=gs))
        self._wg(ops, 'model.6.', g_u2, True, self.u1, True, nf, nf, H2, W2, H4, W4, ups=1, f16=f16)
        g_u1 = self.g2a
        if net.subpixel:
            self._subpixel_dgrad(ops, 'up2_b', g_u2, g_u1, H2, W2, mask=self.u1)
        else:
            ops.add(conv_op(pack, pk['up2_b'], g_u2.view(), True, nf, H4, W4, H4, W4, N, out_f32=g_up2.view(), in_scale=gs))
            ops.add(make_op(_lib.OP_DOWNSUM, src=g_up2.view(), N=N, C=nf, H=H2, W=W2, mask=self.u1.view(), mask_f32=1, slope=SLOPE, dst_f32=g_u1.view()))
        self._wg(ops, 'model.3.', g_u1, True, self.t0, True, nf, nf, h, w, H2, W2, ups=1, f16=f16)
        if net.subpixel:
            self._subpixel_dgrad(ops, 'up1_b', g_u1, self.g_t0, h, w, mask=None)
        else:
            g_up1 = self.g2b
            ops.add(conv_op(pack, pk['up1_b'], g_u1.view(), True, nf, H2, W2, H2, W2, N, out_f32=g_up1.view(), in_scale=gs))
            ops.add(make_op(_lib.OP_DOWNSUM, src=g_up1.view(), N=N, C=nf, H=h, W=w, slope=SLOPE, dst_f32=self.g_t0.view()))

    def _build_backward_trunk(self, ops):
        net, N, h, w = self.net, self.N, self.h, self.w
        nf, nb, P, pack, pk = net.nf, net.nb, net.params, net.pack, net.pk
        lrk = 'model.1.sub.%d.' % nb
        self._wg(ops, lrk, self.g_t0, True, self.x_last, True, nf, nf, h, w, h, w)
        ops.tag(11)
        self._marks = [(len(ops.ops), P.off(lrk + 'weight'), P.total)]
        free = list(self.gstream)
        G = free[0]
        gs_cur = 0
        f16 = int(net.rdb_f16)
        gsc = self.store.gscale
        ops.add(conv_op(pack, pk['lr_b'], self.g_t0.view(), True, nf, h, w, h, w, N, out_f32=G.view(),
                        out_bf16=self.gslab[gs_cur].view(0), gamma=0.04 * gsc, out16_f16=f16))
        if f16:
            self.store.register_scaled(ops.ops[-1], False, base_gamma=0.04)
        use_chain = self.chain is not None and not f16
        main_ops = ops
        if use_chain:
            ops = OpList()
        for i in range(nb - 1, -1, -1):
            Grr = G
            Gout = None
            for r in (3, 2, 1):
                ridx = 3 * i + (r - 1)
                S, Gs = self.slabs[ridx], self.gslab[gs_cur]
                for k in range(4, 0, -1):
                    cin_b = nf + (4 - k) * GC
                    ops.add(conv_op(pack, pk[(i, r, 'b', k)], Gs.view(0), False, cin_b, h, w, h, w, N,
                                    mask=S.view(nf + (k - 1) * GC), mask_f32=0, out_bf16=Gs.view(cin_b), out16_f16=f16))
                Gin = next(b for b in free if b is not Grr and b is not Gout)
                first = (ridx == 0)
                nxt = None if first else self.gslab[gs_cur + 1].view(0)
                if r == 3:
                    ops.add(conv_op(pack, pk[(i, r, 'b', 0)], Gs.view(0), False, nf + 4 * GC, h, w, h, w, N,
                                    res1=Grr.view(), beta1=0.2, out_f32=Gin.view(), out_bf16=nxt, gamma=0.2 * gsc, alpha=1.0 / gsc, out16_f16=f16))
                elif r == 2:
                    ops.add(conv_op(pack, pk[(i, r, 'b', 0)], Gs.view(0), False, nf + 4 * GC, h, w, h, w, N,
                                    res1=Gout.view(), beta1=1.0, out_f32=Gin.view(), out_bf16=nxt, gamma=0.2 * gsc, alpha=1.0 / gsc, out16_f16=f16))
                else:
                    ops.add(conv_op(pack, pk[(i, r, 'b', 0)], Gs.view(0), False, nf + 4 * GC, h, w, h, w, N,
                                    res1=Gout.view(), beta1=1.0, res2=Grr.view(), beta2=1.0, out_f32=Gin.view(), out_bf16=nxt, gamma=0.04 * gsc, alpha=1.0 / gsc,
                                    out16_f16=f16))
                if f16:
                    self.store.register_scaled(ops.ops[-1], True, base_gamma=0.04 if r == 1 else 0.2)
                Gout = Gin
                gs_cur += 1
            G = Gout
        if use_chain:
            body = list(ops.ops)
            assert len(body) == 15 * nb and all(o.op == _lib.OP_CONV for o in body)
            deps = [0 if k % 5 == 0 else (o.conv.cin // 16) - GC // 16 for k, o in enumerate(body)]
            tiles = ceil_div(h, 16) * ceil_div(w, 32)
            nsub = len(self.chains)
            per = N // nsub
            ops = main_ops
            self.chains_b = []
            if self.chain_form == 'is':
                ch = ConvChain(body, deps, N, ceil_div(h, 4) * ceil_div(w, 32), net.device, err=self.chain.err, form='is')
                self.chains_b.append(ch)
                ops.add(ch.op())
                ops.keep.append(ch)
            else:
                for sb in range(nsub):
                    sub = body[:-1] if nsub == 1 else [_sub_batch_conv(o, sb * per, per, N) for o in body[:-1]]
                    ch = ConvChain(sub, deps[:-1], per, tiles, net.device, err=self.chain.err)
                    self.chains_b.append(ch)
                    ops.add(ch.op())
                    ops.keep.append(ch)
                ops.add(body[-1])
            self.chain_b = self.chains_b[0]
        ops.tag(4)
        rrdb0 = P.off('model.1.sub.0.RDB1.conv1.0.weight')
        if not self.shared_store:
            st = self.store
            for first_op, end_op, lo, hi in st.groups:
                ops.extend(st.phase.slice(first_op, end_op))
                self._marks.append((len(ops.ops), lo, hi))
            ops.keep.append(st)
        ops.add(make_op(_lib.OP_AXPBY, x=G.view(), a=1.0, z=self.g_t0.view(), b=1.0, N=N, C=nf, H=h, W=w, out_f32=self.g_fea.view(), gamma=1.0))
        self._wg(ops, 'model.0.', self.g_fea, True, self.x_in, True, nf, net.in_nc, h, w, h, w)
        self._marks.append((len(ops.ops), 0, rrdb0))
        ops.tag(11)
        self.bwd = ops
        self._segments = None

    def set_grad_scale(self, scale):
        return set_reduce_scale([self.bwd], scale)

    def run_backward_dp(self, dp, g):
        segs = self.bwd_segments()
        has_chain = [any(o.op in (_lib.OP_CONV_CHAIN, _lib.OP_RDB_CHAIN) for o in seg.ops) for seg, _ in segs]
        last_chain = max([k for k, c in enumerate(has_chain) if c], default=-1)
        held = []
        for k, (seg, (lo, hi)) in enumerate(segs):
            seg.run()
            held.append((lo, hi))
            if k < last_chain:
                continue
            for a, b in held:
                dp.reduce_async(g[a:b])
            held = []
        dp.wait()

    def bwd_segments(self):
        if self._segments is None:
            segs, prev_idx = [], 0
            for idx, lo, hi in self._marks:
                segs.append((self.bwd.slice(prev_idx, idx), (lo, hi)))
                prev_idx = idx
            self._segments = segs
        return self._segments
```

include/dasr_hip.h:

```cpp
#ifndef DASR_HIP_H
#define DASR_HIP_H
#include <stdint.h>

#ifdef __cplusplus
extern "C" {
#endif

#define DASR_ABI_VERSION 22
#define DASR_EINVAL (-22)
#define DASR_ECAPTURE (-16)

typedef struct {
    void*   p;
    int64_t n_stride;
    int64_t cb_stride;
} dasr_tensor;

typedef struct {
    dasr_tensor in;  int32_t in_f32;  int32_t Hin, Win;  int32_t ups;  int32_t cin;
    const void* w;   int64_t w_lo_off;
    const float* bias;
    int32_t cout, Hout, Wout, N;
    int32_t kh, stride, pad;
    int32_t prec;
    int32_t mt;
    int32_t act;  float slope;
    dasr_tensor mask;  int32_t mask_f32;
    float alpha;  dasr_tensor res1;  float beta1;  dasr_tensor res2;  float beta2;
    dasr_tensor out_f32;  dasr_tensor out_bf16;  float gamma;
    int32_t xcd_remap;
    int32_t pad_x, out_stride, out_oy, out_ox, out_W;
    const float* slope_ptr;
    int32_t in_stride, in_oy, in_ox, in_W;
    float in_scale;
    int32_t out16_f16;
    int32_t in_wrap, out16_lo, res1_lo;
    float* prelu_part;
} dasr_conv_params;

int dasr_conv(const dasr_conv_params* p, void* stream);
int dasr_conv_chain(const dasr_conv_params* dev_layers, const dasr_conv_params* host_layers, const int32_t* dev_dep_chunk, int32_t nlayers,
                    uint32_t* dev_flags, int32_t* dev_err, void* stream);
int dasr_rdb_chain(const dasr_conv_params* dev_layers, const dasr_conv_params* host_layers, int32_t nlayers, uint32_t* dev_flags, int32_t* dev_err,
                   void* stream);
typedef struct {
    dasr_tensor x16;  dasr_tensor x32;
    const void* w0;  const float* b0;
    const void* w1;  const float* b1;
    dasr_tensor y32;  dasr_tensor y16;
    dasr_tensor h;
    int32_t N, H, W;
    float res_scale, slope;
} dasr_resblock_params;
int dasr_resblock(const dasr_resblock_params* p, void* stream);

int dasr_set_tuning(int32_t key, int32_t value);

typedef struct {
    dasr_tensor g;   int32_t g_f32;
    dasr_tensor in;  int32_t in_f32;
    int32_t ups;
    int32_t n_ctiles;
    int32_t g_planes, in_planes;
    int32_t Hin, Win, Hout, Wout, N;
    int32_t kh, stride, pad;
    int32_t want_bias;
    int64_t ws_off;
    int64_t ws_bias_off;
    int32_t tap0;
    float g_scale;
} dasr_wgrad_part;

int dasr_wgrad(const dasr_wgrad_part* parts_dev, int32_t nparts, int32_t nsplit, int32_t kh, int32_t stride, int32_t f32,
               float* ws, void* stream);
int dasr_wgrad_set_mode(int32_t use_tr);

typedef struct {
    int64_t ws_off;  int64_t ws_bias_off;  int32_t nsplit;  int32_t ntaps;
    int32_t oc0, c0;
    int32_t cout, cin, n_ctiles;
    int64_t dst_w_off;  int64_t dst_b_off;
    int32_t flip_io;
    int64_t split_stride, tap_stride, bias_stride;
    int32_t tap0, ntaps_total;
    int32_t bias_nsplit, reserved_;
} dasr_wgrad_reduce_part;

int dasr_wgrad_reduce(const dasr_wgrad_reduce_part* parts_dev, int32_t nparts, const float* ws, float* grad_flat,
                      float scale, int32_t few_splits, void* stream);

typedef struct {
    int64_t src_off;
    int32_t src_cout, src_cin;
    int32_t cin_start, cin_len;
    int32_t src_c0;
    int32_t transpose;
} dasr_pack_seg;

typedef struct {
    int64_t dst_off;
    int64_t lo_off;
    int32_t cout, cin_pad, ntaps, mt, nseg;
    int32_t src_ntaps;
    int32_t fmt;
    int8_t  tapmap[32];
    uint16_t tapmask[16];
    dasr_pack_seg seg[5];
} dasr_pack_desc;

int dasr_pack_weights(const dasr_pack_desc* descs_dev, int32_t ndesc, int64_t total_pieces, const int64_t* piece_prefix_dev,
                      const float* params_flat, void* packed, void* stream);

int dasr_nchw_to_blocked(const float* src, int32_t N, int32_t C, int32_t H, int32_t W, dasr_tensor dst_f32,
                         dasr_tensor dst_bf16, void* stream);
int dasr_blocked_to_nchw(dasr_tensor src, int32_t N, int32_t C, int32_t H, int32_t W, float* dst, void* stream);

int dasr_l1_loss(dasr_tensor sr, const float* hr_nchw, const float* weight_map, int32_t N, int32_t C, int32_t H, int32_t W,
                 float coef, float* loss_acc, dasr_tensor grad, int32_t accumulate, float grad_scale, void* stream);

int dasr_downsum2x(dasr_tensor src, int32_t N, int32_t C, int32_t H, int32_t W, dasr_tensor mask, int32_t mask_f32,
                   float slope, dasr_tensor dst_f32, dasr_tensor dst_bf16, void* stream);

int dasr_cvt_f16(dasr_tensor x, int32_t N, int32_t C, int32_t H, int32_t W, float scale, dasr_tensor y, void* stream);
int dasr_cvt_split16(dasr_tensor x, int32_t N, int32_t C, int32_t H, int32_t W, float scale, dasr_tensor y, int32_t f16, void* stream);
int dasr_f16_residual(dasr_tensor x, int32_t N, int32_t C, int32_t H, int32_t W, float scale, dasr_tensor y, void* stream);
int dasr_downsum2x_f16(dasr_tensor src, int32_t N, int32_t C, int32_t H, int32_t W, dasr_tensor mask , float slope,
                       float out_scale, dasr_tensor dst_f32, dasr_tensor dst_f16, void* stream);

int dasr_pixel_shuffle_f16(dasr_tensor src, int32_t N, int32_t C4, int32_t H, int32_t W, dasr_tensor dst, void* stream);
int dasr_pixel_unshuffle_f16(dasr_tensor gsrc, dasr_tensor mask , float slope, int32_t N, int32_t C4, int32_t H,
                             int32_t W, dasr_tensor gdst, void* stream);

int dasr_axpby(dasr_tensor x, float a, dasr_tensor z, float b, int32_t N, int32_t C, int32_t H, int32_t W,
               dasr_tensor out_f32, dasr_tensor out_bf16, float gamma, dasr_tensor mask , float slope,
               const float* slope_ptr, void* stream);

int dasr_adam(float* p, const float* g, float* m, float* v, int64_t n, float lr, float beta1, float beta2, float eps,
              float weight_decay, int32_t step, int32_t* nonfinite_flag, const int32_t* gate_flag, void* stream);

int dasr_fill_f32(float* p, int64_t n, float value, void* stream);
int dasr_add_flat(float* y, const float* x, int64_t n, void* stream);


int dasr_inorm_lrelu_fwd(dasr_tensor x, int32_t N, int32_t C, int32_t H, int32_t W, float eps, float slope, dasr_tensor y,
                         float* stats, void* stream);
int dasr_inorm_lrelu_bwd(dasr_tensor a, dasr_tensor ga, int32_t N, int32_t C, int32_t H, int32_t W, float slope,
                         const float* stats, dasr_tensor gx, void* stream);
int dasr_inorm_lrelu_jvp(dasr_tensor a, dasr_tensor t, int32_t N, int32_t C, int32_t H, int32_t W, float slope, const float* stats, dasr_tensor out, void* stream);
int dasr_inorm_second(dasr_tensor a, dasr_tensor t, dasr_tensor ga, int32_t N, int32_t C, int32_t H, int32_t W, float slope, const float* stats,
                      dasr_tensor out, int32_t accumulate, void* stream);
int dasr_grad_penalty(dasr_tensor g, int32_t N, int32_t C, int32_t H, int32_t W, float weight, float* part256, float* out3, float* loss_acc, int32_t stage,
                      int32_t world, void* stream);
int dasr_fill_scaled(dasr_tensor x, int32_t N, int32_t C, int32_t H, int32_t W, const float* scalar, float factor, void* stream);
int dasr_bnorm_lrelu_fwd(dasr_tensor x, int32_t N, int32_t C, int32_t H, int32_t W, int32_t group, float eps, float slope, const float* gamma,
                         const float* beta, dasr_tensor y, float* stats, void* stream);
int dasr_bnorm_lrelu_bwd(dasr_tensor x, dasr_tensor ga, int32_t N, int32_t C, int32_t H, int32_t W, int32_t group, float slope, const float* gamma,
                         const float* beta, const float* stats, dasr_tensor gx, float* dgamma, float* dbeta, float pscale, void* stream);
int dasr_bnorm_lrelu_jvp(dasr_tensor x, dasr_tensor t, int32_t N, int32_t C, int32_t H, int32_t W, int32_t group, float slope, const float* gamma,
                         const float* beta, const float* stats, dasr_tensor out, void* stream);
int dasr_bnorm_second(dasr_tensor x, dasr_tensor t, dasr_tensor ga, int32_t N, int32_t C, int32_t H, int32_t W, int32_t group, float slope,
                      const float* gamma, const float* beta, const float* stats, dasr_tensor out, int32_t accumulate, float* dgamma, float pscale,
                      void* stream);
int dasr_bnorm_running(const float* stats, int32_t g, int32_t C, int32_t count, float momentum, float* running_mean, float* running_var,
                       float* num_batches_tracked, void* stream);
int dasr_bce_logits(dasr_tensor x, int32_t N, int32_t C, int32_t H, int32_t W, float target, float coef, float gcoef,
                    float* loss_acc, float* score_acc, float score_coef, dasr_tensor grad, void* stream);
int dasr_gan_loss(dasr_tensor x, int32_t N, int32_t C, int32_t H, int32_t W, int32_t gan_type, float target, float coef, float gcoef,
                  float* loss_acc, float* score_acc, float score_coef, dasr_tensor grad, void* stream);
int dasr_ragan(dasr_tensor a, dasr_tensor b, int32_t N, int32_t H, int32_t W, int32_t stage, int32_t n_glob, int32_t form, float ta, float tb,
               float coef, float gcoef, float eps, float* sums, float* part, float* loss_acc, float* score_a, float* score_b, float score_coef,
               dasr_tensor ga, dasr_tensor gb, void* stream);
int dasr_dwt_fwd(dasr_tensor x, int32_t N, int32_t C, int32_t H2, int32_t W2, int32_t norm, dasr_tensor ll, dasr_tensor hc, void* stream);
int dasr_dwt_bwd(dasr_tensor gll, dasr_tensor ghc, int32_t N, int32_t C, int32_t H2, int32_t W2, int32_t norm, dasr_tensor gx,
                 int32_t accumulate, void* stream);
int dasr_lowpass(dasr_tensor x, dasr_tensor x2, const float* w, int32_t k, int32_t N, int32_t C, int32_t H, int32_t W,
                 int32_t mode, float a_h, float b_h, dasr_tensor out_low, dasr_tensor out_high, int32_t accumulate, void* stream);
int dasr_maxpool2(dasr_tensor x, int32_t is_f32, int32_t N, int32_t C, int32_t Ho, int32_t Wo, dasr_tensor y, int32_t Win, void* stream);
int dasr_maxpool2_bwd(dasr_tensor x, dasr_tensor gy, int32_t is_f32, int32_t N, int32_t C, int32_t Ho, int32_t Wo, dasr_tensor gx,
                      int32_t relu_mask, int32_t Win, void* stream);
int dasr_l1_diff(dasr_tensor a, dasr_tensor b, int32_t is_f32, int32_t N, int32_t C, int32_t H, int32_t W, float coef, float gcoef,
                 float* loss_acc, dasr_tensor ga, void* stream);
int dasr_affine4(dasr_tensor x, int32_t N, int32_t C, int32_t H, int32_t W, const float* scale4, const float* shift4, dasr_tensor y,
                 int32_t y_f32, int32_t accumulate, void* stream);
int dasr_bilinear_up(const float* src, int32_t N, int32_t h, int32_t w, int32_t factor, float* dst, void* stream);

int dasr_lpips_s2d(dasr_tensor x, int32_t N, int32_t H, int32_t W, const float* scale4, const float* shift4, dasr_tensor y, int32_t mode,
                   void* stream);
int dasr_lpips_s2d_any(dasr_tensor x, int32_t N, int32_t H, int32_t W, const float* scale4, const float* shift4, dasr_tensor y, void* stream);
int dasr_maxpool3s2(dasr_tensor x, int32_t N, int32_t C, int32_t H, int32_t W, dasr_tensor y, void* stream);
int dasr_maxpool3s2_bwd(dasr_tensor x, dasr_tensor gy, int32_t N, int32_t C, int32_t H, int32_t W, dasr_tensor gx, int32_t relu_mask,
// ... 139 lines not shown
```

Measured before the change: 556.0.

## Pack LeakyReLU sign bits in forward to replace bf16 mask reads in backward

```diff
diff --git a/dasr_amd/_lib.py b/dasr_amd/_lib.py
--- a/dasr_amd/_lib.py
+++ b/dasr_amd/_lib.py
@@ -22,7 +22,8 @@
                 ('alpha', c_f32), ('res1', Tensor), ('beta1', c_f32), ('res2', Tensor), ('beta2', c_f32),
                 ('out_f32', Tensor), ('out_bf16', Tensor), ('gamma', c_f32), ('xcd_remap', c_i32),
                 ('pad_x', c_i32), ('out_stride', c_i32), ('out_oy', c_i32), ('out_ox', c_i32), ('out_W', c_i32), ('slope_ptr', c_vp),
-                ('in_stride', c_i32), ('in_oy', c_i32), ('in_ox', c_i32), ('in_W', c_i32), ('in_scale', c_f32), ('out16_f16', c_i32), ('in_wrap', c_i32), ('out16_lo', c_i32), ('res1_lo', c_i32), ('prelu_part', c_vp)]
+                ('in_stride', c_i32), ('in_oy', c_i32), ('in_ox', c_i32), ('in_W', c_i32), ('in_scale', c_f32), ('out16_f16', c_i32), ('in_wrap', c_i32), ('out16_lo', c_i32), ('res1_lo', c_i32), ('prelu_part', c_vp),
+                ('sign_out', c_vp), ('mask_bits', c_vp), ('reserved_', c_i64 * 2)]
 
 
 class WgradPart(C.Structure):
diff --git a/dasr_amd/csrc/conv.hip b/dasr_amd/csrc/conv.hip
--- a/dasr_amd/csrc/conv.hip
+++ b/dasr_amd/csrc/conv.hip
@@ -49,9 +49,19 @@
 };
 
 template <int MT, int NT>
-__device__ __forceinline__ void mask_prefetch(const dasr_conv_params& p, MaskPre<NT * MT>& m, int tid, int mg, int n, int oy0, int ox0) {
+__device__ __forceinline__ void mask_prefetch(const dasr_conv_params& p, MaskPre<NT * MT>& m, int tid, int mg, int n, int oy0, int ox0, const int32_t* bits) {
     const int lane = tid & 63, wave = tid >> 6, nn = lane & 31, kh2 = lane >> 5;
     const int ostr = p.out_stride > 1 ? p.out_stride : 1, owid = p.out_W > 0 ? p.out_W : p.Wout;
+    if (MT == 1 && bits != nullptr) {
+        const __amdgpu_buffer_rsrc_t rbits = make_rsrc(bits + (size_t)n * 4 * p.Hout * p.Wout);
+#pragma unroll
+        for (int gi = 0; gi < NT * MT; ++gi) {
+            const int oy = oy0 + wave * NT + gi, ox = ox0 + nn;
+            const unsigned bo = ((oy < p.Hout) & (ox < p.Wout)) ? (unsigned)(oy * p.Wout + ox) * 4u : OOB;
+            m.v[gi][0][0] = __builtin_amdgcn_raw_buffer_load_b32(rbits, bo, 0, 0);
+        }
+        return;
+    }
     const __amdgpu_buffer_rsrc_t rmask = make_rsrc((const char*)p.mask.p + (size_t)n * p.mask.n_stride * 2);
     const unsigned mask_cb = (unsigned)p.mask.cb_stride;
 #pragma unroll
@@ -69,6 +79,13 @@
     }
 }
 
+typedef short s16x2_t __attribute__((ext_vector_type(2)));
+__device__ __forceinline__ unsigned pos16x2(unsigned d) {
+    const s16x2_t x = __builtin_bit_cast(s16x2_t, d);
+    const s16x2_t zero = {0, 0}, one = {1, 1};
+    return __builtin_bit_cast(unsigned, __builtin_elementwise_min(__builtin_elementwise_max(x, zero), one));
+}
+
 template <bool SC1>
 __device__ __forceinline__ void st128(u32x4 v, __amdgpu_buffer_rsrc_t r, unsigned off) {
     if constexpr (SC1) __builtin_amdgcn_raw_buffer_store_b128(v, r, off, 0, 16);
@@ -78,7 +95,7 @@
 template <bool IN_F32, int MT, int NT, int STRIDE, int EPI, int F16OUT = -1, bool PRE = false, bool FSC1 = false, bool BIAS_STAGED = false, bool CONST_SLOPE = false,
           bool PACC = false>
 __device__ __forceinline__ void conv_epilogue(const dasr_conv_params& p, f32x16 (&acc)[MT][NT], char* smem, float bias_reg, int tid, int mg, int n,
-                                              int oy0, int ox0, const MaskPre<NT * MT>* pre = nullptr) {
+                                              int oy0, int ox0, const MaskPre<NT * MT>* pre = nullptr, const int32_t* plane = nullptr) {
     const int lane = tid & 63, wave = tid >> 6, nn = lane & 31, kh2 = lane >> 5;
     (void)lane;
     constexpr bool G = EPI == 0;
@@ -123,6 +140,11 @@
     }
     TRACE_STAMP(5);
     constexpr int NG = NT * MT;
+    constexpr bool SIGN_OK = EPI == 67 && MT == 1 && !IN_F32 && F16OUT >= 0;
+    static_assert(!SIGN_OK || NT == 1 || NT % 2 == 0, "the sign words of a wave's rows are stored by its two half-waves");
+    const __amdgpu_buffer_rsrc_t rsg = make_rsrc((SIGN_OK ? plane : nullptr) + (size_t)n * 4 * p.Hout * p.Wout);
+    const unsigned sign_oob = (SIGN_OK && plane != nullptr) ? 0u : OOB;
+    unsigned sign_even = 0u, sign_even_off = OOB;
     constexpr bool WIDE16 = !G && !IN_F32;
     constexpr bool WIDE32 = !G && STRIDE == 1;
     constexpr bool PIPE_EPI = !G && !(MT == 2 && (EPI & 16) && (EPI & 8)) && (EPI & (4 | 8 | 16));
@@ -259,7 +281,18 @@
 #pragma unroll
                     for (int j = 0; j < 4; ++j) v[g][j] = __frcp_rn(1.f + __expf(-v[g][j]));
             }
-            if (has_mask) {
+            bool mask_done = false;
+            if constexpr (PRE && MT == 1) {
+                if (has_mask && plane != nullptr) {
+                    const unsigned ws = pre->v[gi][0][0] >> (4 * kh2);
+#pragma unroll
+                    for (int g = 0; g < 4; ++g)
+#pragma unroll
+                        for (int j = 0; j < 4; ++j) v[g][j] = (ws & (1u << (8 * g + j))) ? v[g][j] : slope * v[g][j];
+                    mask_done = true;
+                }
+            }
+            if (has_mask && !mask_done) {
                 if constexpr (WIDE16) {
 #pragma unroll
                     for (int pr = 0; pr < 2; ++pr) {
@@ -357,6 +390,7 @@
             }
             if (has_bf16 && WIDE16) {
                 const bool gm = scaled && p.gamma != 1.f;
+                unsigned sgn = 0u;
 #pragma unroll
                 for (int pr = 0; pr < 2; ++pr) {
                     bf16x4 oa, ob;
@@ -367,6 +401,10 @@
                         ob[j] = f16out ? __builtin_bit_cast(bf16_t, (f16_t)vb) : (bf16_t)vb;
                     }
                     const u32x2 a = __builtin_bit_cast(u32x2, oa), b = __builtin_bit_cast(u32x2, ob);
+                    if constexpr (SIGN_OK) {
+                        const unsigned t = pos16x2(a[0]) | (pos16x2(a[1]) << 2) | (pos16x2(b[0]) << 8) | (pos16x2(b[1]) << 10);
+                        sgn |= ((t | (t >> 15)) & 0x0f0fu) << (16 * pr);
+                    }
                     const auto r0 = __builtin_amdgcn_permlane32_swap(a[0], b[0], false, false);
                     const auto r1 = __builtin_amdgcn_permlane32_swap(a[1], b[1], false, false);
                     const u32x4 o = {r0[0], r1[0], r0[1], r1[1]};
@@ -385,6 +423,20 @@
                         const auto q1 = __builtin_amdgcn_permlane32_swap(a2[1], b2[1], false, false);
                         const u32x4 o2 = {q0[0], q1[0], q0[1], q1[1]};
                         st128<SC1>(o2, rob, eo[2 * pr] != OOB ? ((cbv[2 * pr] + lo_pl) * ob_cb + eo[2 * pr] + 4u * kh2) * 2u : OOB);
+                    }
+                }
+                if constexpr (SIGN_OK) {
+                    const unsigned mine = sgn << (4 * kh2);
+                    const auto sw = __builtin_amdgcn_permlane32_swap(mine, mine, false, false);
+                    const unsigned word = sw[0] | sw[1];
+                    const unsigned off = (eo[0] != OOB ? (eo[0] >> 4) * 4u : OOB) | sign_oob;
+                    if constexpr (NT == 1) {
+                        __builtin_amdgcn_raw_buffer_store_b32(word, rsg, kh2 == 0 ? off : OOB, 0, 0);
+                    } else if ((gi & 1) == 0) {
+                        sign_even = word;
+                        sign_even_off = off;
+                    } else {
+                        __builtin_amdgcn_raw_buffer_store_b32(kh2 ? word : sign_even, rsg, kh2 ? off : sign_even_off, 0, 0);
                     }
                 }
             } else if (has_bf16) {
@@ -860,7 +912,7 @@
         char* nbuf = smem + ((ck + 1) & 1) * C::BUF_BYTES;
         const bool more = ck + 1 < nchunks;
         if constexpr (PRE) {
-            if (!more) mask_prefetch<MT, NT>(p, mpre, tid, mg, n, oy0, ox0);
+            if (!more) mask_prefetch<MT, NT>(p, mpre, tid, mg, n, oy0, ox0, p.mask_bits);
         }
         const int ckn = ck + 1 + rot < nchunks ? ck + 1 + rot : ck + 1 + rot - nchunks;
         const int ckp = ckn >= in_wrap ? ckn - in_wrap : ckn;
@@ -904,7 +956,7 @@
         if (p.prelu_part) conv_epilogue<false, MT, NT, 1, EPI, F16 ? 1 : 0, false, false, false, false, true>(p, acc, smem, bias_reg, tid, mg, n, oy0, ox0, &mpre);
         else conv_epilogue<false, MT, NT, 1, EPI, F16 ? 1 : 0, PRE>(p, acc, smem, bias_reg, tid, mg, n, oy0, ox0, &mpre);
     } else {
-        conv_epilogue<false, MT, NT, 1, R1_PRE ? (EPI & ~8) : EPI, F16 ? 1 : 0, PRE>(p, acc, smem, bias_reg, tid, mg, n, oy0, ox0, &mpre);
+        conv_epilogue<false, MT, NT, 1, R1_PRE ? (EPI & ~8) : EPI, F16 ? 1 : 0, PRE>(p, acc, smem, bias_reg, tid, mg, n, oy0, ox0, &mpre, PRE ? p.mask_bits : p.sign_out);
     }
     TRACE_STAMP(6);
 #ifdef DASR_TRACE
@@ -994,6 +1046,8 @@
     const __amdgpu_buffer_rsrc_t rin = make_rsrc((const bf16_t*)p.in.p + (size_t)n * p.in.n_stride);
     const unsigned in_chunk_bytes = (unsigned)(p.in.cb_stride * 2);
     const __amdgpu_buffer_rsrc_t rw = make_rsrc(p.w);
+    const int32_t* plane = MT == 1 ? ((EPI & 4) ? p.mask_bits : (const int32_t*)p.sign_out) : nullptr;
+    asm volatile("" : "+s"(plane));
     constexpr int NP = C::AR + C::WR;
     if (dep_chunk <= 0) cs.wait(layer, tid);
 #pragma unroll
@@ -1063,7 +1117,7 @@
             t_poll += CH_T() - t0;
         }
         if constexpr (PRE) {
-            if (!more) mask_prefetch<MT, NT>(p, mpre, tid, 0, n, oy0, ox0);
+            if (!more) mask_prefetch<MT, NT>(p, mpre, tid, 0, n, oy0, ox0, plane);
         }
         bf16x8 fa[3][MT];
 #pragma unroll
@@ -1097,7 +1151,7 @@
         __syncthreads();
     }
     const unsigned long long t_d = CH_T();
-    conv_epilogue<false, MT, NT, 1, R1_PRE ? (EPI & ~8) : EPI, F16 ? 1 : 0, PRE, true>(p, acc, smem, bias_reg, tid, 0, n, oy0, ox0, &mpre);
+    conv_epilogue<false, MT, NT, 1, R1_PRE ? (EPI & ~8) : EPI, F16 ? 1 : 0, PRE, true>(p, acc, smem, bias_reg, tid, 0, n, oy0, ox0, &mpre, plane);
     const unsigned long long t_e = CH_T();
     cs.publish(layer, tid);
     const unsigned long long t_f = CH_T();
@@ -1256,10 +1310,19 @@
 int classify_epi(const dasr_conv_params& p) {
     if ((p.cout & 31) || p.act == 2 || p.out_stride > 1 || p.res1_lo || (p.out16_lo && !p.out16_f16)) return 0;
     if (p.act == 1 && !p.slope_ptr && !(p.slope >= 0.f && p.slope <= 1.f)) return 0;
-    int e = (p.bias ? 1 : 0) | (p.act == 1 ? 2 : 0) | (p.mask.p ? 4 : 0) | (p.res1.p ? 8 : 0) | (p.res2.p ? 16 : 0) | (p.out_f32.p ? 32 : 0) |
+    int e = (p.bias ? 1 : 0) | (p.act == 1 ? 2 : 0) | ((p.mask.p || p.mask_bits) ? 4 : 0) | (p.res1.p ? 8 : 0) | (p.res2.p ? 16 : 0) | (p.out_f32.p ? 32 : 0) |
             (p.out_bf16.p ? 64 : 0);
     if (p.res1.p || p.alpha != 1.f || p.gamma != 1.f) e |= 128;
     return e;
+}
+
+bool sign_fields_ok(const dasr_conv_params& p) {
+    if (!p.sign_out && !p.mask_bits) return true;
+    if (p.mask_bits && p.mask.p) return false;
+    if (p.in_f32 || p.mt != 1 || p.cout != 32 || p.kh != 3 || p.stride != 1 || p.pad != 1) return false;
+    if (p.out_stride > 1 || p.out_W || p.out_oy || p.out_ox) return false;
+    const int epi = classify_epi(p);
+    return (!p.sign_out || epi == 67) && (!p.mask_bits || epi == 68);
 }
 
 int g_tune_rdb64 = 13;
@@ -1293,6 +1356,7 @@
         if (p.Hin != p0.Hin || p.Win != p0.Win || p.Hout != p0.Hin || p.Wout != p0.Win || p.N != p0.N || p.out_stride > 1 || p.in_stride > 1 || p.out_W || p.out_oy || p.out_ox) return DASR_EINVAL;
         if (!(p.mt == 1 || p.mt == 2) || p.cout != 32 * p.mt || !p.w || !p.in.p || p.slope_ptr || p.mask_f32 || p.prelu_part) return DASR_EINVAL;
         if ((p.out16_f16 != 0) != f16 || (p.prec != 1 && p.prec != 2)) return DASR_EINVAL;
+        if (!sign_fields_ok(p)) return DASR_EINVAL;
         const int epi = classify_epi(p);
         const bool ok = bwd ? (p.mt == 1 ? epi == 68 : (epi == 232 || epi == 248)) : (p.mt == 1 ? epi == 67 : (epi == 233 || epi == 249));
         if (!ok) return DASR_EINVAL;
@@ -1348,6 +1412,7 @@
         if (p.Hin != p0.Hin || p.Win != p0.Win || p.Hout != p0.Hin || p.Wout != p0.Win || p.N != p0.N || p.out_stride > 1 || p.in_stride > 1 || p.out_W || p.out_oy || p.out_ox) return DASR_EINVAL;
         if (p.cin != 64 + 32 * k || p.mt != (k == 4 ? 2 : 1) || p.cout != 32 * p.mt || !p.w || !p.in.p || p.slope_ptr || p.mask_f32 || p.prelu_part) return DASR_EINVAL;
         if (p.in.p != pb.in.p || p.in.n_stride != pb.in.n_stride || p.in.cb_stride != pb.in.cb_stride) return DASR_EINVAL;
+        if (!sign_fields_ok(p)) return DASR_EINVAL;
         const int epi = classify_epi(p);
         const bool ok = k < 4 ? epi == (bwd ? 68 : 67) : ((epi & ~(16 | 64)) == (bwd ? 168 : 169) && p.res1.p && p.alpha != 0.f);
         if (!ok) return DASR_EINVAL;
@@ -1423,6 +1488,7 @@
     if (p.mask.p && (p.mask_f32 != 0) != (p.in_f32 != 0)) return DASR_EINVAL;
     if (p.ups && !p.in_f32 && p.prec != 2) return DASR_EINVAL;
     if (p.in_wrap < 0 || p.out16_lo < 0 || p.res1_lo < 0) return DASR_EINVAL;
+    if (!sign_fields_ok(p)) return DASR_EINVAL;
     if (p.in_wrap || p.out16_lo || p.res1_lo) {
         if (p.in_f32 || p.kh != 3 || p.stride != 1 || p.pad != 1 || !(p.prec == 1 || p.prec == 2) || p.ups || p.out_stride > 1) return DASR_EINVAL;
         if (p.in_wrap && (p.cin >> 4) * 2 != p.in_wrap * 3) return DASR_EINVAL;
@@ -1509,7 +1575,7 @@
 extern "C" int dasr_conv_naive(const dasr_conv_params* pp, const float* w_ref, void* stream) {
     const dasr_conv_params& p = *pp;
     const long long total = (long long)p.N * p.cout * p.Hout * p.Wout;
-    if (total <= 0) return DASR_EINVAL;
+    if (total <= 0 || p.sign_out || p.mask_bits) return DASR_EINVAL;
     DASR_LAUNCH(conv_naive_kernel, dim3((unsigned)((total + 255) / 256)), dim3(256), 0, as_stream(stream), p, w_ref);
     return (int)hipGetLastError();
 }
diff --git a/dasr_amd/csrc/rdb_is.h b/dasr_amd/csrc/rdb_is.h
--- a/dasr_amd/csrc/rdb_is.h
+++ b/dasr_amd/csrc/rdb_is.h
@@ -491,7 +491,7 @@
                     is_body<NT, 2, 2048, 1024, F16>(A5[0], A5[1], abuf, wbuf, baddr, aoff, mid);
                 }
                 MaskPre<NT> mpre;
-                if constexpr (BWD && EU_AFTER >= 0 && EU_AFTER < 4) mask_prefetch<1, NT>(layers[L0 + EU_AFTER], mpre, tid, 0, cur.n, cur.oy0, cur.ox0);
+                if constexpr (BWD && EU_AFTER >= 0 && EU_AFTER < 4) mask_prefetch<1, NT>(layers[L0 + EU_AFTER], mpre, tid, 0, cur.n, cur.oy0, cur.ox0, layers[L0 + EU_AFTER].mask_bits);
                 const unsigned long long t1 = IS_T();
                 int nwait = issued - mk[C::WDIST - 2];
                 bool do_pub = false;
@@ -568,8 +568,8 @@
                         else conv_epilogue<false, 2, NT, 1, E0 + 8, F16 ? 1 : 0, false, true, true, true>(p, A5, bl, 0.f, tid, 0, cur.n, cur.oy0, cur.ox0);
                     } else {
                         auto epi14 = [&](f32x16 (&A)[1][NT]) {
-                            if constexpr (BWD) conv_epilogue<false, 1, NT, 1, 68, F16 ? 1 : 0, true, true, true, true>(p, A, bl, 0.f, tid, 0, cur.n, cur.oy0, cur.ox0, &mpre);
-                            else conv_epilogue<false, 1, NT, 1, 67, F16 ? 1 : 0, false, true, true, true>(p, A, bl, 0.f, tid, 0, cur.n, cur.oy0, cur.ox0);
+                            if constexpr (BWD) conv_epilogue<false, 1, NT, 1, 68, F16 ? 1 : 0, true, true, true, true>(p, A, bl, 0.f, tid, 0, cur.n, cur.oy0, cur.ox0, &mpre, p.mask_bits);
+                            else conv_epilogue<false, 1, NT, 1, 67, F16 ? 1 : 0, false, true, true, true>(p, A, bl, 0.f, tid, 0, cur.n, cur.oy0, cur.ox0, nullptr, p.sign_out);
                         };
                         if constexpr (EU == 0) epi14(A0);
                         else if constexpr (EU == 1) epi14(A1);
diff --git a/dasr_amd/dist.py b/dasr_amd/dist.py
--- a/dasr_amd/dist.py
+++ b/dasr_amd/dist.py
@@ -5,7 +5,7 @@
 
 
 RANK_CONSISTENT_ENV = ('DASR_HR_PREC', 'DASR_RDB_PREC', 'DASR_VGG_PREC', 'DASR_VGG_BWD_PREC', 'DASR_VGG_NOGRAD_PREC', 'DASR_D_PREC', 'DASR_DSN_BWD16', 'DASR_DSN_FWD16', 'DASR_DSN_PRELU_FUSED',
-                       'DASR_STREAMS', 'DASR_ENQ', 'DASR_CHAIN', 'DASR_CHAIN_FORM', 'DASR_CHAIN_SPLIT', 'DASR_TUNE', 'DASR_HIP_LIB', 'DASR_RCCL_NATIVE', 'DASR_DP_BACKEND', 'DASR_ALLOW_NONFINITE')
+                       'DASR_STREAMS', 'DASR_ENQ', 'DASR_CHAIN', 'DASR_CHAIN_FORM', 'DASR_CHAIN_SPLIT', 'DASR_SIGN_PLANES', 'DASR_TUNE', 'DASR_HIP_LIB', 'DASR_RCCL_NATIVE', 'DASR_DP_BACKEND', 'DASR_ALLOW_NONFINITE')
 
 
 SHARED_DEVICE = False
diff --git a/dasr_amd/engine.py b/dasr_amd/engine.py
--- a/dasr_amd/engine.py
+++ b/dasr_amd/engine.py
@@ -292,7 +292,7 @@
 def conv_op(pack, ref, inp, in_f32, cin, Hin, Win, Hout, Wout, N, bias=None, kh=3, stride=1, pad=1, ups=0, act=0, slope=SLOPE,
             mask=None, mask_f32=0, alpha=1.0, res1=None, beta1=0.0, res2=None, beta2=0.0, out_f32=None, out_bf16=None, gamma=1.0,
             pad_x=-1, out_stride=1, out_oy=0, out_ox=0, out_W=0, slope_ptr=None, in_stride=1, in_oy=0, in_ox=0, in_W=0, flops=None, in_scale=0.0, out16_f16=0,
-            in_wrap=0, out16_lo=0, res1_lo=0):
+            in_wrap=0, out16_lo=0, res1_lo=0, sign_out=None, mask_bits=None):
     assert cin == ref.cin_pad, (cin, ref.cin_pad)
     o = Op()
     o.op = _lib.OP_CONV
@@ -317,6 +317,7 @@
     p.out16_f16 = int(out16_f16)
     p.res1_lo = int(res1_lo)
     p.in_wrap, p.out16_lo = int(in_wrap), int(out16_lo)
+    p.sign_out, p.mask_bits = sign_out, mask_bits
     return o
 
 
diff --git a/dasr_amd/rrdbnet.py b/dasr_amd/rrdbnet.py
--- a/dasr_amd/rrdbnet.py
+++ b/dasr_amd/rrdbnet.py
@@ -45,6 +45,7 @@
         self.rdb_prec, self.stream_prec = rdb_prec, stream_prec
         self.rdb_f16 = rdb_prec == 2
         self.chain = os.environ.get('DASR_CHAIN', '1') == '1' and not self.rdb_f16
+        self.sign_planes = os.environ.get('DASR_SIGN_PLANES', '1') == '1'
         self.chain_form = os.environ.get('DASR_CHAIN_FORM', 'auto')
         assert self.chain_form in ('auto', 'is', 'layer')
         self.chain_err = torch.zeros(1, dtype=torch.int32, device=self.device)
@@ -234,6 +235,9 @@
         t = getattr(c, name)
         if t.p:
             t.p = t.p + n0 * t.n_stride * esz
+    for name in ('sign_out', 'mask_bits'):
+        if getattr(c, name):
+            setattr(c, name, getattr(c, name) + n0 * 4 * c.Hout * c.Wout * 4)
     c.N = n
     q.flops = o.flops * n / N
     return q
@@ -273,6 +277,7 @@
         super().__init__(net.rdb_f16, headroom=0.04)
         self.slab_t = [mk() for _ in range(3 * nb)]
         self.gslab_t = [mk() for _ in range(3 * nb)]
+        self.sign_t = [torch.zeros((N, 4, h, w), dtype=torch.int32, device=dev) for _ in range(3 * nb)] if getattr(net, 'sign_planes', False) else None
         self.sc = sc
         self.ws = Workspace(dev)
         self._build_phase()
@@ -285,6 +290,11 @@
     def gslab(self, ridx, n0=0, N=None):
         N = self.N if N is None else N
         return BTensor.wrap(self.gslab_t[ridx][n0:n0 + N], self.sc, False)
+
+    def sign_plane(self, ridx, k, n0=0):
+        if self.sign_t is None:
+            return None
+        return self.sign_t[ridx].data_ptr() + ((n0 * 4 + (k - 1)) * self.h * self.w) * 4
 
     def _build_phase(self):
         net, N, h, w = self.net, self.N, self.h, self.w
@@ -453,7 +463,7 @@
                 for j in range(1, 5):
                     cin = nf + (j - 1) * GC
                     ops.add(conv_op(pack, pk[(i, r, j)], S.view(0), False, cin, h, w, h, w, N, bias=P.ptr('%s%d.0.bias' % (pre, j)),
-                                    act=1, out_bf16=S.view(cin), out16_f16=f16))
+                                    act=1, out_bf16=S.view(cin), out16_f16=f16, sign_out=None if self.inference else self.store.sign_plane(ridx, j, self.n0)))
                 last = (ridx == 3 * nb - 1)
                 Y = next(b for b in free if b is not X and b is not Xrrdb)
                 nxt = None if last else self.slabs[ridx + 1].view(0)
@@ -685,8 +695,9 @@
                 S, Gs = self.slabs[ridx], self.gslab[gs_cur]
                 for k in range(4, 0, -1):
                     cin_b = nf + (4 - k) * GC
+                    bits = self.store.sign_plane(ridx, k, self.n0)
                     ops.add(conv_op(pack, pk[(i, r, 'b', k)], Gs.view(0), False, cin_b, h, w, h, w, N,
-                                    mask=S.view(nf + (k - 1) * GC), mask_f32=0, out_bf16=Gs.view(cin_b), out16_f16=f16))
+                                    mask=None if bits else S.view(nf + (k - 1) * GC), mask_f32=0, mask_bits=bits, out_bf16=Gs.view(cin_b), out16_f16=f16))
                 Gin = next(b for b in free if b is not Grr and b is not Gout)
                 first = (ridx == 0)
                 nxt = None if first else self.gslab[gs_cur + 1].view(0)
diff --git a/include/dasr_hip.h b/include/dasr_hip.h
--- a/include/dasr_hip.h
+++ b/include/dasr_hip.h
@@ -36,6 +36,9 @@
     int32_t out16_f16;
     int32_t in_wrap, out16_lo, res1_lo;
     float* prelu_part;
+    int32_t* sign_out;
+    const int32_t* mask_bits;
+    int64_t reserved_[2];
 } dasr_conv_params;
 
 int dasr_conv(const dasr_conv_params* p, void* stream);
```

Result: no change. 555.7 (-0.0%).
